# lez-s/Materialist

Hardware: AMD Instinct MI355X
Metric: opt_iterations_per_sec_512x512 (higher is better)
Workload: dtype f32; 1 GPU; BASELINE configs[1] synthetic: 1x512x512/GPU, --model_name pos_mlp --opt_order 'rm a' part rm, spp 64; mode=pos_mlp, height=512, width=512, spp=64, images_per_gpu=1, light=SH25, parallelism=dp1 (independent images, no data-path collective)

## Files before the change

include/matpbr_mlp.h:

```cpp
#ifndef MATPBR_MLP_H
#define MATPBR_MLP_H
#include <stddef.h>
#include <stdint.h>

#ifdef __cplusplus
extern "C" {
#endif

int matpbr_mlp_small_bwd_step(const float* g, int ldg, const float* w, int ldw, const float* c_prev, float* g_prev, int ldo, float* colsum_out,
                              int n_prev, const float* x, int ldx, float* d_w, int ldw_out, int K, const float* colsum_in, int colsum_stride,
                              int groups_in, float* d_bias, long M, int n_red, void* stream);

int matpbr_sin_bwd(const float* d_y, long ld_d, const float* pre, long ld_p, float* out, long M, int n, void* stream);
size_t matpbr_column_sum_workspace_bytes(int N);
int matpbr_column_sum(const float* x, float* out, long M, int N, void* workspace, size_t workspace_bytes, void* stream);

int matpbr_mlp_layer_fwd(const float* x, int ldx, const float* w, int ldw, const float* bias, float* s_out, float* c_out, int ldo, long M,
                         int N, int K, void* stream);
size_t matpbr_mlp_bwd_input_workspace_bytes(long M);
int matpbr_mlp_layer_bwd_input(const float* g, int ldg, const float* wt, int ldwt, const float* c_prev, float* g_prev, int ldo,
                               float* d_bias_prev, void* workspace, size_t workspace_bytes, long M, int n_prev, int n_red, void* stream);
size_t matpbr_mlp_bwd_weight_workspace_bytes(long M);
int matpbr_mlp_layer_bwd_weight(const float* g, int ldg, const float* x, int ldx, float* d_w, int ldw, void* workspace,
                                size_t workspace_bytes, long M, int N, int K, void* stream);

size_t matpbr_mlp_wsplit_bytes(int K);
int matpbr_mlp_split_weights(const float* w, int ldw, int N, int K, void* wsplit, void* stream);
int matpbr_mlp_layer_fwd_bx(const float* x, int ldx, const void* wsplit, const float* bias, float* s_out, float* c_out, int ldo, long M,
                            int N, int K, int nprod, void* stream);
int matpbr_mlp_first_layer_bwd_bx(const float* g, int ldg, const void* wtsplit, const float* c_prev, int ldc, int sgn, const float* x0, int ldx0,
                                  float* d_w0, long ld_j, long ld_c, int d0, float* d_bias0, void* workspace, size_t workspace_bytes, void* workspace2,
                                  size_t workspace2_bytes, long M, int n0, int n_red, int nprod, void* stream);
int matpbr_mlp_layer_bwd_input_bx(const float* g, int ldg, const void* wtsplit, const float* c_prev, float* g_prev, int ldo,
                                  float* d_bias_prev, void* workspace, size_t workspace_bytes, long M, int n_prev, int n_red,
                                  int nprod, void* stream);
int matpbr_mlp_layer_fwd_tail(const float* x, int ldx, const float* w, int ldw, const float* bias, float* s_out, float* c_out, int ldo,
                              const float* tail, int ldt, long M, int N, int K, void* stream);
int matpbr_mlp_layer_fwd_bx_tail(const float* x, int ldx, const void* wsplit, const float* bias, float* s_out, float* c_out, int ldo,
                                 const float* tail, int ldt, long M, int N, int K, int nprod, void* stream);
int matpbr_mlp_layer_fwd_bx_head(const float* x, int ldx, const void* wsplit, const float* bias, float* s_out, float* c_out, int ldo,
                                 const float* w_out, int ldw_out, const float* bias_out, const float* start, int lds, float* th,
                                 float* map_a, float* map_r, float* map_m, long M, int K, int nprod, void* stream);
int matpbr_mlp_layer_fwd_sgn(const float* x, int ldx, const float* w, int ldw, const float* bias, float* s_out, int ldo, const float* tail, int ldt,
                             long M, int N, int K, void* stream);
int matpbr_mlp_layer_bwd_input_sgn(const float* g, int ldg, const float* wt, int ldwt, const float* s_prev, float* g_prev, int ldo,
                                   float* d_bias_prev, void* workspace, size_t workspace_bytes, long M, int n_prev, int n_red, void* stream);
int matpbr_mlp_layer_bwd_input_bx_sgn(const float* g, int ldg, const void* wtsplit, const float* s_prev, float* g_prev, int ldo,
                                      float* d_bias_prev, void* workspace, size_t workspace_bytes, long M, int n_prev, int n_red,
                                      int nprod, void* stream);
int matpbr_mlp_layer_bwd_weight_bx(const float* g, int ldg, const float* x, int ldx, float* d_w, int ldw, void* workspace,
                                   size_t workspace_bytes, long M, int N, int K, int nprod, void* stream);

#define MATPBR_WSPLIT_TRANSPOSED 1
#define MATPBR_WSPLIT_F16X2 2
int matpbr_mlp_split_weights_fmt(const float* w, int ldw, int N, int K, int flags, void* wsplit, void* stream);
size_t matpbr_mlp_chain_images_bytes(void);
int matpbr_mlp_chain_prep(const float* const* w, const int* ldw, const int* n, const float* const* bias, int d0, void* images, void* const* bwd_images,
                          void* zero, long zero_words, void* stream);
int matpbr_mlp_chain_fwd(const float* x0, int ldx0, const void* images, float* const* s_out, int ldo, const int* n, const float* start, int lds, float* th,
                         float* map_a, float* map_r, float* map_m, int n_head, long M, void* stream);
#define MATPBR_REDUCE_NONE (-1)
#define MATPBR_REDUCE_WGRAD 0
#define MATPBR_REDUCE_COLSUM 1
#define MATPBR_REDUCE_SKINNY 2
typedef struct MatpbrReduceJob {
    int kind, groups;
    const float *src, *src_b, *src_g;
    float *dst, *dst_b, *dst_g;
    int n0, n1, n2, n3;
    long ld_j, ld_c;
} MatpbrReduceJob;
int matpbr_mlp_reduce_jobs(const MatpbrReduceJob* jobs, int n_jobs, void* stream);
int matpbr_mlp_out_layer_bwd_tmax(const float* d_x, int ldd, const float* s_prev, const float* c_prev, int lds, const float* w_out, int ldw, float* g_prev,
                                  int ldg, void* g_tile_max, float* d_w, long ld_j, long ld_c, float* d_bias, float* d_bias_prev, void* workspace,
                                  size_t workspace_bytes, long M, int J, int n_prev, MatpbrReduceJob* defer, void* stream);
int matpbr_mlp_layer_bwd_input_blk(const float* g, int ldg, const void* g_tile_max, const void* wtsplit, const float* s_prev, float* g_prev, int ldo,
                                   void* out_tile_max, float* d_bias_prev, void* workspace, size_t workspace_bytes, long M, int n_prev, int n_red,
                                   MatpbrReduceJob* defer, void* stream);
int matpbr_mlp_first_layer_bwd_blk(const float* g, int ldg, const void* g_tile_max, const void* wtsplit, const float* s_prev, int lds, const float* x0,
                                   int ldx0, float* d_w0, long ld_j, long ld_c, int d0, float* d_bias0, void* workspace, size_t workspace_bytes,
                                   void* workspace2, size_t workspace2_bytes, long M, int n0, int n_red, MatpbrReduceJob* defer2, void* stream);
int matpbr_mlp_layer_bwd_weight_blk(const float* g, int ldg, const void* g_tile_max, const float* x, int ldx, float* d_w, int ldw, void* workspace,
                                    size_t workspace_bytes, long M, int N, int K, MatpbrReduceJob* defer, void* stream);
int matpbr_mlp_set_wgrad_kernel(int kernel);
int matpbr_mlp_split_weights_multi(const float* const* w, const int* ldw, const int* N, const int* K, const int* transposed,
                                   void* const* wsplit, int n_jobs, void* stream);
int matpbr_mlp_skinny_fwd(const float* x, int ldx, const float* w, int ldw, const float* bias, float* out, int ldo, long M, int J, int K,
                          void* stream);
int matpbr_mlp_arm_head_fwd(const float* x, int ldx, const float* w, int ldw, const float* bias, const float* start, int lds, float* th,
                            float* map_a, float* map_r, float* map_m, long M, int K, void* stream);
int matpbr_mlp_arm_head_bwd(const float* g_a, const float* g_r, const float* g_m, const float* th, float* d_x, long M, void* stream);
size_t matpbr_mlp_skinny_workspace_bytes(int J);
int matpbr_mlp_out_layer_bwd(const float* d_x, int ldd, const float* s_prev, const float* c_prev, int lds, const float* w_out, int ldw, float* g_prev,
                             int ldg, float* d_w, long ld_j, long ld_c, float* d_bias, float* d_bias_prev, void* workspace, size_t workspace_bytes,
                             long M, int J, int n_prev, void* stream);
int matpbr_mlp_skinny_bwd_weight(const float* s, int lds, const float* b, int ldb, float* d_w, long ld_j, long ld_c, float* d_bias,
                                 void* workspace, size_t workspace_bytes, long M, int J, int C, void* stream);
int matpbr_adamw_step_dev(float* p, const float* g, float* m, float* v, long n, float* hyper, float beta1, float beta2, float eps,
                          float weight_decay, void* stream);
int matpbr_adamw_step_snapshot_dev(float* p, const float* g, float* m, float* v, long n, float* hyper, float beta1, float beta2,
                                   float eps, float weight_decay, float* best, const float* stats, void* stream);

#ifdef __cplusplus
}
#endif
#endif
```

materialist_amd/_lib.py:

```python
from __future__ import annotations

import ctypes
import os
import threading

from . import build as _build

_c_f = ctypes.c_void_p


class MatpbrCamera(ctypes.Structure):
    _fields_ = [("fov_x_deg", ctypes.c_float)]


class MatpbrBrdfPhase(ctypes.Structure):
    _fields_ = ([(k, ctypes.c_void_p) for k in ("pa", "pr", "pm", "n", "light", "gt_srgb", "a0", "r0", "m0", "dcache", "pred", "jac", "d_a",
                                                "d_r", "d_m")] +
                [("adam_m", ctypes.c_void_p * 3), ("adam_v", ctypes.c_void_p * 3)] +
                [(k, ctypes.c_void_p) for k in ("best_a", "best_r", "best_m", "best_img", "stats", "history", "workspace")] +
                [("workspace_bytes", ctypes.c_size_t), ("H", ctypes.c_int), ("W", ctypes.c_int), ("batch", ctypes.c_int), ("spp", ctypes.c_int),
                 ("fov_x_deg", ctypes.c_float), ("scale_delta", ctypes.c_float), ("part_mask", ctypes.c_uint32), ("es_patience", ctypes.c_int),
                 ("es_min_delta", ctypes.c_float), ("hist_len", ctypes.c_int), ("s1cache", ctypes.c_void_p), ("lazy_state", ctypes.c_void_p),
                 ("lazy_tol", ctypes.c_float), ("pred_next", ctypes.c_void_p), ("flags", ctypes.c_uint32), ("lazy_fold", ctypes.c_void_p)])


class MatpbrNormalStep(ctypes.Structure):
    _fields_ = ([(k, ctypes.c_void_p) for k in ("pa", "pr", "pm", "pn", "ca", "cr", "cm", "cn", "d_a", "d_r", "d_m", "d_n", "a0", "r0", "m0", "n0")] +
                [("adam_m", ctypes.c_void_p * 4), ("adam_v", ctypes.c_void_p * 4)] +
                [(k, ctypes.c_void_p) for k in ("best_a", "best_r", "best_m", "best_n", "best_img", "pred", "stats", "ln_part")] +
                [("H", ctypes.c_int), ("W", ctypes.c_int), ("batch", ctypes.c_int), ("part_mask", ctypes.c_uint32), ("scale_delta", ctypes.c_float)])


class MatpbrError(RuntimeError):
    pass


class ReduceJob(ctypes.Structure):
    _fields_ = [("kind", ctypes.c_int), ("groups", ctypes.c_int), ("src", ctypes.c_void_p), ("src_b", ctypes.c_void_p), ("src_g", ctypes.c_void_p),
                ("dst", ctypes.c_void_p), ("dst_b", ctypes.c_void_p), ("dst_g", ctypes.c_void_p), ("n0", ctypes.c_int), ("n1", ctypes.c_int),
                ("n2", ctypes.c_int), ("n3", ctypes.c_int), ("ld_j", ctypes.c_long), ("ld_c", ctypes.c_long)]


SIGNATURES = {
    "matpbr_version": (ctypes.c_int, []),
    "matpbr_strerror": (ctypes.c_char_p, [ctypes.c_int]),
    "matpbr_shade_fwd": (ctypes.c_int, [_c_f] * 5 + [ctypes.c_int, ctypes.c_int, _c_f, ctypes.c_int, ctypes.c_int, ctypes.c_int,
                                       ctypes.c_int, ctypes.POINTER(MatpbrCamera), ctypes.c_uint32, ctypes.c_void_p]),
    "matpbr_shade_bwd": (ctypes.c_int, [_c_f] * 5 + [ctypes.c_int, ctypes.c_int] + [_c_f] * 6 + [ctypes.c_void_p, ctypes.c_size_t,
                                       ctypes.c_int, ctypes.c_int, ctypes.c_int, ctypes.c_int, ctypes.POINTER(MatpbrCamera),
                                       ctypes.c_uint32, ctypes.c_void_p]),
    "matpbr_shade_bwd_workspace_bytes": (ctypes.c_size_t, [ctypes.c_int] * 4),
    "matpbr_plane9_bytes": (ctypes.c_size_t, [ctypes.c_int] * 3),
    "matpbr_shade_fwd_ex": (ctypes.c_int, [_c_f] * 5 + [ctypes.c_int, ctypes.c_int, _c_f, _c_f, _c_f, ctypes.c_int, ctypes.c_int, ctypes.c_int,
                                          ctypes.c_int, ctypes.POINTER(MatpbrCamera), ctypes.c_uint32, ctypes.c_void_p]),
    "matpbr_shade_fwd_keep": (ctypes.c_int, [_c_f] * 5 + [ctypes.c_int, ctypes.c_int, _c_f, _c_f, _c_f, _c_f, ctypes.c_int, ctypes.c_int, ctypes.c_int,
                                            ctypes.c_int, ctypes.POINTER(MatpbrCamera), ctypes.c_uint32, ctypes.c_void_p]),
    "matpbr_shade_fwd_cached": (ctypes.c_int, [_c_f] * 5 + [ctypes.c_int, ctypes.c_int, ctypes.c_int, ctypes.c_uint32, ctypes.c_void_p]),
    "matpbr_diffuse_cache": (ctypes.c_int, [_c_f, _c_f, ctypes.c_int, ctypes.c_int, _c_f, ctypes.c_int, ctypes.c_int, ctypes.c_int, ctypes.c_int,
                                           ctypes.POINTER(MatpbrCamera), ctypes.c_void_p]),
    "matpbr_lazy_state_bytes": (ctypes.c_size_t, [ctypes.c_int] * 3),
    "matpbr_lazy_fold_bytes": (ctypes.c_size_t, [ctypes.c_int] * 3),
    "matpbr_env_texel_phase_step": (ctypes.c_int, [_c_f] * 6 + [ctypes.c_int, ctypes.c_int, ctypes.c_float, ctypes.c_void_p, ctypes.c_size_t, ctypes.c_int,
                                                   ctypes.c_int, _c_f, ctypes.c_int] + [_c_f] * 8 + [ctypes.c_float] * 3 + [ctypes.c_int, ctypes.c_int,
                                                                                                                          ctypes.c_void_p]),
    "matpbr_brdf_loss_dpred": (ctypes.c_int, [_c_f] * 4 + [ctypes.c_int, ctypes.c_int, ctypes.c_int, ctypes.c_void_p]),
    "matpbr_brdf_normal_step": (ctypes.c_int, [ctypes.POINTER(MatpbrNormalStep), ctypes.c_int, ctypes.c_float, ctypes.c_void_p]),
    "matpbr_env_mlp_phase_step": (ctypes.c_int, [_c_f] * 7 + [ctypes.c_int, ctypes.c_int, ctypes.c_float, ctypes.c_void_p, ctypes.c_size_t, ctypes.c_int,
                                                 ctypes.c_int, _c_f, ctypes.c_int] + [_c_f] * 4 + [ctypes.c_int, ctypes.c_int, ctypes.c_void_p]),
    "matpbr_brdf_phase_stages_timed": (ctypes.c_int, [ctypes.POINTER(MatpbrBrdfPhase), ctypes.c_int, ctypes.c_float, ctypes.c_uint32, ctypes.c_void_p,
                                                      ctypes.c_void_p, ctypes.c_void_p]),
    "matpbr_lazy_sums_count": (ctypes.c_int, [ctypes.c_int] * 2),
    "matpbr_shade_fwd_lazy": (ctypes.c_int, [_c_f] * 5 + [ctypes.c_int, ctypes.c_int] + [_c_f] * 6 + [ctypes.c_int, ctypes.c_int, ctypes.c_int, ctypes.c_int,
                                            ctypes.POINTER(MatpbrCamera), ctypes.c_uint32, ctypes.c_float, ctypes.c_float, ctypes.c_void_p]),
    "matpbr_lazy_state_unpack": (ctypes.c_int, [_c_f, _c_f, _c_f, ctypes.c_int, ctypes.c_int, ctypes.c_int, ctypes.c_void_p]),
    "matpbr_jac16_unpack": (ctypes.c_int, [_c_f, _c_f, ctypes.c_int, ctypes.c_int, ctypes.c_int, ctypes.c_void_p]),
    "matpbr_shade_bwd_jac": (ctypes.c_int, [_c_f] * 8 + [ctypes.c_int, ctypes.c_int, ctypes.c_int, ctypes.c_void_p]),
    "matpbr_brdf_loss_workspace_bytes": (ctypes.c_size_t, [ctypes.c_int]),
    "matpbr_brdf_loss_stats": (ctypes.c_int, [_c_f] * 9 + [ctypes.c_float, _c_f, ctypes.c_void_p, ctypes.c_size_t, ctypes.c_int, ctypes.c_int,
                                             ctypes.c_int, ctypes.c_uint32, ctypes.c_void_p]),
    "matpbr_brdf_loss_stats_es": (ctypes.c_int, [_c_f] * 9 + [ctypes.c_float, _c_f, ctypes.c_void_p, ctypes.c_size_t, ctypes.c_int, ctypes.c_int,
                                                ctypes.c_int, ctypes.c_uint32, ctypes.c_int, ctypes.c_float, _c_f, ctypes.c_int, ctypes.c_void_p]),
    "matpbr_brdf_loss_bwd_jac": (ctypes.c_int, [_c_f] * 10 + [ctypes.c_float] + [_c_f] * 7 + [ctypes.c_int, ctypes.c_int, ctypes.c_int,
                                                                                              ctypes.c_uint32, ctypes.c_void_p]),
    "matpbr_brdf_phase_workspace_bytes": (ctypes.c_size_t, [ctypes.c_int] * 3),
    "matpbr_brdf_phase_step": (ctypes.c_int, [ctypes.POINTER(MatpbrBrdfPhase), ctypes.c_int, ctypes.c_float, ctypes.c_void_p]),
    "matpbr_brdf_phase_stages": (ctypes.c_int, [ctypes.POINTER(MatpbrBrdfPhase), ctypes.c_int, ctypes.c_float, ctypes.c_uint32, ctypes.c_void_p]),
    "matpbr_brdf_phase_resolve": (ctypes.c_int, [ctypes.POINTER(MatpbrBrdfPhase), ctypes.c_int, ctypes.c_void_p]),
    "matpbr_env_phase_workspace_bytes": (ctypes.c_size_t, [ctypes.c_int] * 3),
    "matpbr_env_phase_step": (ctypes.c_int, [_c_f] * 7 + [ctypes.c_int, ctypes.c_int, ctypes.c_float, ctypes.c_void_p, ctypes.c_size_t,
                                            ctypes.c_int, ctypes.c_int, ctypes.c_int, ctypes.c_void_p]),
    "matpbr_env_project": (ctypes.c_int, [_c_f, ctypes.c_int, _c_f, _c_f, _c_f, ctypes.c_int, ctypes.c_void_p]),
    "matpbr_env_project_bwd": (ctypes.c_int, [_c_f, ctypes.c_int, _c_f, _c_f, _c_f, ctypes.c_int, ctypes.c_int, ctypes.c_void_p]),
    "matpbr_select_improved": (ctypes.c_int, [_c_f, _c_f, _c_f, ctypes.c_int, ctypes.c_long, ctypes.c_void_p]),
    "matpbr_mlp_wsplit_bytes": (ctypes.c_size_t, [ctypes.c_int]),
    "matpbr_mlp_split_weights": (ctypes.c_int, [_c_f, ctypes.c_int, ctypes.c_int, ctypes.c_int, _c_f, ctypes.c_void_p]),
    "matpbr_mlp_layer_fwd_bx": (ctypes.c_int, [_c_f, ctypes.c_int, _c_f, _c_f, _c_f, _c_f, ctypes.c_int, ctypes.c_long, ctypes.c_int, ctypes.c_int,
                                              ctypes.c_int, ctypes.c_void_p]),
    "matpbr_mlp_layer_bwd_input_bx": (ctypes.c_int, [_c_f, ctypes.c_int, _c_f, _c_f, _c_f, ctypes.c_int, _c_f, ctypes.c_void_p, ctypes.c_size_t,
                                                    ctypes.c_long, ctypes.c_int, ctypes.c_int, ctypes.c_int, ctypes.c_void_p]),
    "matpbr_sin_bwd": (ctypes.c_int, [_c_f, ctypes.c_long, _c_f, ctypes.c_long, _c_f, ctypes.c_long, ctypes.c_int, ctypes.c_void_p]),
    "matpbr_mlp_layer_fwd": (ctypes.c_int, [_c_f, ctypes.c_int, _c_f, ctypes.c_int, _c_f, _c_f, _c_f, ctypes.c_int, ctypes.c_long, ctypes.c_int,
                                           ctypes.c_int, ctypes.c_void_p]),
    "matpbr_mlp_bwd_input_workspace_bytes": (ctypes.c_size_t, [ctypes.c_long]),
    "matpbr_mlp_layer_bwd_input": (ctypes.c_int, [_c_f, ctypes.c_int, _c_f, ctypes.c_int, _c_f, _c_f, ctypes.c_int, _c_f, ctypes.c_void_p,
                                                 ctypes.c_size_t, ctypes.c_long, ctypes.c_int, ctypes.c_int, ctypes.c_void_p]),
    "matpbr_mlp_bwd_weight_workspace_bytes": (ctypes.c_size_t, [ctypes.c_long]),
    "matpbr_mlp_layer_bwd_weight": (ctypes.c_int, [_c_f, ctypes.c_int, _c_f, ctypes.c_int, _c_f, ctypes.c_int, ctypes.c_void_p, ctypes.c_size_t,
                                                  ctypes.c_long, ctypes.c_int, ctypes.c_int, ctypes.c_void_p]),
    "matpbr_mlp_layer_fwd_sgn": (ctypes.c_int, [_c_f, ctypes.c_int, _c_f, ctypes.c_int, _c_f, _c_f, ctypes.c_int, _c_f, ctypes.c_int, ctypes.c_long,
                                               ctypes.c_int, ctypes.c_int, ctypes.c_void_p]),
    "matpbr_mlp_layer_bwd_input_sgn": (ctypes.c_int, [_c_f, ctypes.c_int, _c_f, ctypes.c_int, _c_f, _c_f, ctypes.c_int, _c_f, ctypes.c_void_p,
                                                     ctypes.c_size_t, ctypes.c_long, ctypes.c_int, ctypes.c_int, ctypes.c_void_p]),
    "matpbr_mlp_layer_bwd_input_bx_sgn": (ctypes.c_int, [_c_f, ctypes.c_int, _c_f, _c_f, _c_f, ctypes.c_int, _c_f, ctypes.c_void_p, ctypes.c_size_t,
                                                        ctypes.c_long, ctypes.c_int, ctypes.c_int, ctypes.c_int, ctypes.c_void_p]),
    "matpbr_mlp_layer_bwd_weight_bx": (ctypes.c_int, [_c_f, ctypes.c_int, _c_f, ctypes.c_int, _c_f, ctypes.c_int, ctypes.c_void_p, ctypes.c_size_t,
                                                     ctypes.c_long, ctypes.c_int, ctypes.c_int, ctypes.c_int, ctypes.c_void_p]),
    "matpbr_mlp_out_layer_bwd_tmax": (ctypes.c_int, [_c_f, ctypes.c_int, _c_f, _c_f, ctypes.c_int, _c_f, ctypes.c_int, _c_f, ctypes.c_int, ctypes.c_void_p, _c_f,
                                                     ctypes.c_long, ctypes.c_long, _c_f, _c_f, ctypes.c_void_p, ctypes.c_size_t, ctypes.c_long, ctypes.c_int,
                                                     ctypes.c_int, ctypes.c_void_p, ctypes.c_void_p]),
    "matpbr_mlp_reduce_jobs": (ctypes.c_int, [ctypes.c_void_p, ctypes.c_int, ctypes.c_void_p]),
    "matpbr_mlp_layer_bwd_input_blk": (ctypes.c_int, [_c_f, ctypes.c_int, ctypes.c_void_p, ctypes.c_void_p, _c_f, _c_f, ctypes.c_int, ctypes.c_void_p, _c_f,
                                                      ctypes.c_void_p, ctypes.c_size_t, ctypes.c_long, ctypes.c_int, ctypes.c_int, ctypes.c_void_p, ctypes.c_void_p]),
    "matpbr_mlp_first_layer_bwd_blk": (ctypes.c_int, [_c_f, ctypes.c_int, ctypes.c_void_p, ctypes.c_void_p, _c_f, ctypes.c_int, _c_f, ctypes.c_int, _c_f,
                                                      ctypes.c_long, ctypes.c_long, ctypes.c_int, _c_f, ctypes.c_void_p, ctypes.c_size_t, ctypes.c_void_p,
                                                      ctypes.c_size_t, ctypes.c_long, ctypes.c_int, ctypes.c_int, ctypes.c_void_p, ctypes.c_void_p]),
    "matpbr_mlp_layer_bwd_weight_blk": (ctypes.c_int, [_c_f, ctypes.c_int, ctypes.c_void_p, _c_f, ctypes.c_int, _c_f, ctypes.c_int, ctypes.c_void_p,
                                                       ctypes.c_size_t, ctypes.c_long, ctypes.c_int, ctypes.c_int, ctypes.c_void_p, ctypes.c_void_p]),
    "matpbr_mlp_set_wgrad_kernel": (ctypes.c_int, [ctypes.c_int]),
    "matpbr_mlp_chain_images_bytes": (ctypes.c_size_t, []),
    "matpbr_mlp_chain_prep": (ctypes.c_int, [ctypes.c_void_p, ctypes.c_void_p, ctypes.c_void_p, ctypes.c_void_p, ctypes.c_int, ctypes.c_void_p, ctypes.c_void_p,
                                             ctypes.c_void_p, ctypes.c_long, ctypes.c_void_p]),
    "matpbr_mlp_chain_fwd": (ctypes.c_int, [_c_f, ctypes.c_int, ctypes.c_void_p, ctypes.c_void_p, ctypes.c_int, ctypes.c_void_p, _c_f, ctypes.c_int, _c_f, _c_f, _c_f,
                                            _c_f, ctypes.c_int, ctypes.c_long, ctypes.c_void_p]),
    "matpbr_mlp_split_weights_fmt": (ctypes.c_int, [_c_f, ctypes.c_int, ctypes.c_int, ctypes.c_int, ctypes.c_int, ctypes.c_void_p, ctypes.c_void_p]),
    "matpbr_mlp_skinny_fwd": (ctypes.c_int, [_c_f, ctypes.c_int, _c_f, ctypes.c_int, _c_f, _c_f, ctypes.c_int, ctypes.c_long, ctypes.c_int, ctypes.c_int,
                                            ctypes.c_void_p]),
    "matpbr_mlp_arm_head_fwd": (ctypes.c_int, [_c_f, ctypes.c_int, _c_f, ctypes.c_int, _c_f, _c_f, ctypes.c_int, _c_f, _c_f, _c_f, _c_f, ctypes.c_long,
                                              ctypes.c_int, ctypes.c_void_p]),
    "matpbr_mlp_arm_head_bwd": (ctypes.c_int, [_c_f, _c_f, _c_f, _c_f, _c_f, ctypes.c_long, ctypes.c_void_p]),
    "matpbr_mlp_skinny_workspace_bytes": (ctypes.c_size_t, [ctypes.c_int]),
    "matpbr_mlp_set_lds_dma": (ctypes.c_int, [ctypes.c_int]),
    "matpbr_mlp_skinny_bwd_weight": (ctypes.c_int, [_c_f, ctypes.c_int, _c_f, ctypes.c_int, _c_f, ctypes.c_long, ctypes.c_long, _c_f, ctypes.c_void_p,
                                                   ctypes.c_size_t, ctypes.c_long, ctypes.c_int, ctypes.c_int, ctypes.c_void_p]),
    "matpbr_adamw_step_dev": (ctypes.c_int, [_c_f] * 4 + [ctypes.c_long, _c_f, ctypes.c_float, ctypes.c_float, ctypes.c_float, ctypes.c_float,
                                                         ctypes.c_void_p]),
    "matpbr_light_to_sh25": (ctypes.c_int, [_c_f, ctypes.c_int, ctypes.c_int, _c_f, ctypes.c_int, ctypes.c_void_p]),
    "matpbr_light_to_sh25_bwd": (ctypes.c_int, [_c_f, ctypes.c_int, ctypes.c_int, _c_f, ctypes.c_int, ctypes.c_void_p]),
    "matpbr_mlp_split_weights_multi": (ctypes.c_int, [ctypes.c_void_p] * 6 + [ctypes.c_int, ctypes.c_void_p]),
    "matpbr_adamw_step_snapshot_dev": (ctypes.c_int, [_c_f] * 4 + [ctypes.c_long, _c_f, ctypes.c_float, ctypes.c_float, ctypes.c_float, ctypes.c_float,
                                                                  _c_f, _c_f, ctypes.c_void_p]),
    "matpbr_mlp_layer_fwd_tail": (ctypes.c_int, [_c_f, ctypes.c_int, _c_f, ctypes.c_int, _c_f, _c_f, _c_f, ctypes.c_int, _c_f, ctypes.c_int, ctypes.c_long,
                                                ctypes.c_int, ctypes.c_int, ctypes.c_void_p]),
    "matpbr_mlp_layer_fwd_bx_tail": (ctypes.c_int, [_c_f, ctypes.c_int, _c_f, _c_f, _c_f, _c_f, ctypes.c_int, _c_f, ctypes.c_int, ctypes.c_long,
                                                   ctypes.c_int, ctypes.c_int, ctypes.c_int, ctypes.c_void_p]),
    "matpbr_sample_brdf_dr": (ctypes.c_int, [_c_f] * 10 + [ctypes.c_long, ctypes.c_void_p]),
    "matpbr_mlp_layer_fwd_bx_head": (ctypes.c_int, [_c_f, ctypes.c_int, _c_f, _c_f, _c_f, _c_f, ctypes.c_int, _c_f, ctypes.c_int, _c_f, _c_f, ctypes.c_int,
                                                   _c_f, _c_f, _c_f, _c_f, ctypes.c_long, ctypes.c_int, ctypes.c_int, ctypes.c_void_p]),
    "matpbr_column_sum_workspace_bytes": (ctypes.c_size_t, [ctypes.c_int]),
    "matpbr_column_sum": (ctypes.c_int, [_c_f, _c_f, ctypes.c_long, ctypes.c_int, ctypes.c_void_p, ctypes.c_size_t, ctypes.c_void_p]),
    "matpbr_shade_transfer": (ctypes.c_int, [_c_f] * 5 + [ctypes.c_int, ctypes.c_int, ctypes.c_int, ctypes.c_int, ctypes.POINTER(MatpbrCamera),
                                            ctypes.c_uint32, ctypes.c_void_p]),
    "matpbr_transfer_bytes": (ctypes.c_size_t, [ctypes.c_int] * 3),
    "matpbr_relight": (ctypes.c_int, [_c_f] * 3 + [ctypes.c_int, ctypes.c_int, ctypes.c_int, ctypes.c_void_p]),
    "matpbr_adam_step": (ctypes.c_int, [_c_f] * 4 + [ctypes.c_long, ctypes.c_float, ctypes.c_float, ctypes.c_float, ctypes.c_float, ctypes.c_int,
                                       ctypes.c_void_p]),
    "matpbr_eval_brdf": (ctypes.c_int, [_c_f] * 8 + [ctypes.c_long, ctypes.c_void_p]),
    "matpbr_eval_brdf_bwd": (ctypes.c_int, [_c_f] * 11 + [ctypes.c_long, ctypes.c_void_p]),
    "matpbr_brdf_terms": (ctypes.c_int, [_c_f] * 5 + [ctypes.c_long, ctypes.c_void_p]),
    "matpbr_sample_brdf": (ctypes.c_int, [_c_f] * 10 + [ctypes.c_long, ctypes.c_void_p]),
    "matpbr_sh_eval": (ctypes.c_int, [_c_f] * 3 + [ctypes.c_long, ctypes.c_void_p]),
    "matpbr_depth_to_mesh_host": (ctypes.c_int, [ctypes.c_void_p, ctypes.c_int, ctypes.c_int, ctypes.c_float, ctypes.c_float] + [ctypes.c_void_p] * 6),
    "matpbr_mlp_small_bwd_step": (ctypes.c_int, [_c_f, ctypes.c_int, _c_f, ctypes.c_int, _c_f, _c_f, ctypes.c_int, _c_f, ctypes.c_int, _c_f, ctypes.c_int,
                                                 _c_f, ctypes.c_int, ctypes.c_int, _c_f, ctypes.c_int, ctypes.c_int, _c_f, ctypes.c_long, ctypes.c_int,
                                                 ctypes.c_void_p]),
    "matpbr_mlp_out_layer_bwd": (ctypes.c_int, [_c_f, ctypes.c_int, _c_f, _c_f, ctypes.c_int, _c_f, ctypes.c_int, _c_f, ctypes.c_int, _c_f, ctypes.c_long,
                                                ctypes.c_long, _c_f, _c_f, ctypes.c_void_p, ctypes.c_size_t, ctypes.c_long, ctypes.c_int, ctypes.c_int,
                                                ctypes.c_void_p]),
    "matpbr_mlp_first_layer_bwd_bx": (ctypes.c_int, [_c_f, ctypes.c_int, ctypes.c_void_p, _c_f, ctypes.c_int, ctypes.c_int, _c_f, ctypes.c_int, _c_f, ctypes.c_long,
                                                     ctypes.c_long, ctypes.c_int, _c_f, ctypes.c_void_p, ctypes.c_size_t, ctypes.c_void_p, ctypes.c_size_t,
                                                     ctypes.c_long, ctypes.c_int, ctypes.c_int, ctypes.c_int, ctypes.c_void_p]),
    "matpbr_masked_mean_fill": (ctypes.c_int, [_c_f, ctypes.c_void_p, _c_f, ctypes.c_float, ctypes.c_float, _c_f, ctypes.c_long, ctypes.c_int,
                                               ctypes.c_void_p]),
    "matpbr_normals_from_depth": (ctypes.c_int, [_c_f, _c_f, ctypes.c_int, ctypes.c_int, ctypes.c_int, ctypes.POINTER(MatpbrCamera),
                                                 ctypes.c_void_p]),
}

_lock = threading.Lock()
_lib = None


def library_path() -> str:
    return os.environ.get("MATPBR_LIB") or _build.LIB_PATH


def load(build_if_missing: bool = False) -> ctypes.CDLL:
    global _lib
    with _lock:
        if _lib is not None:
            return _lib
        path = library_path()
        if not os.path.exists(path):
            if build_if_missing:
                _build.build_library()
            else:
                raise MatpbrError(
                    f"{path} is missing: build it with `python -c 'import __graft_entry__ as g; g.build()'` "
                    "(hipcc --offload-arch=gfx950). matpbr has no CPU or PyTorch fallback.")
        try:
            lib = ctypes.CDLL(path)
        except OSError as e:
            raise MatpbrError(f"cannot load {path}: {e}") from e
        for name, (res, args) in SIGNATURES.items():
            try:
                fn = getattr(lib, name)
            except AttributeError as e:
                raise MatpbrError(f"{path} does not export {name}") from e
            fn.restype = res
            fn.argtypes = args
        _lib = lib
        return lib


def check(code: int, what: str) -> None:
    if code != 0:
        msg = load().matpbr_strerror(code)
        raise MatpbrError(f"{what} failed: {msg.decode() if msg else code} ({code})")
```

materialist_amd/csrc/posmlp_kernels.hip:

```cpp
#include <hip/hip_runtime.h>
#include <stdint.h>
#include <atomic>
#include <type_traits>

#include "../../include/matpbr.h"
#include "../../include/matpbr_experimental.h"
#include "posmlp_device.hpp"

namespace {


constexpr int kBM = 128, kBN = 128, kBK = 32;
constexpr int kPersistent = 512;
constexpr int EPI_SINCOS = 0, EPI_MULC = 1, EPI_BIAS = 2;

struct HeadArgs {
  const float* w;
  int ldw;
  const float* bias;
  ArmHead h;
};

__global__ __launch_bounds__(256) void mlp_tail_copy_kernel(float* __restrict__ out, int ldo, const float* __restrict__ tail, int ldt, long M, int N) {
  const int w = 256 - N;
  const long total = M * w;
  for (long i = (long)blockIdx.x * 256 + threadIdx.x; i < total; i += (long)gridDim.x * 256) {
    const long m = i / w;
    const int j = (int)(i - m * w);
    out[m * ldo + N + j] = tail[m * ldt + j];
  }
}
__device__ __forceinline__ void store4_upto(float* dst, float4 v, int valid, bool all) {
  if (all) {
    *reinterpret_cast<float4*>(dst) = v;
    return;
  }
  if (valid >= 4) {
    *reinterpret_cast<float4*>(dst) = v;
  } else {
    if (valid > 0) dst[0] = v.x;
    if (valid > 1) dst[1] = v.y;
    if (valid > 2) dst[2] = v.z;
  }
}

struct NtArgs {
  const float* A;
  const float* B;
  const float* bias;
  const float* cmul;
  float* out0;
  float* out1;
  float* colsum;
  int M;
  int N, K, lda, ldb, ldo;
  const float* tail;
  int ldt;
  int cmul_sin;
  const float* x0;
  int ldx0;
  float* w0_part;
  const unsigned* a_tmax;
  unsigned* o_tmax;
};

constexpr int kLd = 36;
constexpr int kTileFloats = kBM * kLd;

__device__ __forceinline__ void fetch_a(const NtArgs& p, float4 (&ra)[4], int row0, int kslot, int crow, int ck) {
  int k = kslot * kBK + ck;
  const int kmax = ((p.K + 3) & ~3) - 4;
  k = k < kmax ? k : kmax;
#pragma unroll
  for (int q = 0; q < 4; ++q) {
    int m = row0 + crow + 32 * q;
    m = m < p.M ? m : p.M - 1;
    ra[q] = *reinterpret_cast<const float4*>(p.A + (size_t)m * p.lda + k);
  }
}

__device__ __forceinline__ void fetch_b(const NtArgs& p, float4 (&rb)[4], int col0, int kslot, int crow, int ck) {
  int k = kslot * kBK + ck;
  const int kmax = ((p.K + 3) & ~3) - 4;
  k = k < kmax ? k : kmax;
#pragma unroll
  for (int q = 0; q < 4; ++q) {
    int n = col0 + crow + 32 * q;
    n = n < p.N ? n : p.N - 1;
    rb[q] = *reinterpret_cast<const float4*>(p.B + (size_t)n * p.ldb + k);
  }
}

__device__ __forceinline__ float4 kmask(float4 v, int k, int K, bool keep) {
  v.x = (keep && k < K) ? v.x : 0.f;
  v.y = (keep && k + 1 < K) ? v.y : 0.f;
  v.z = (keep && k + 2 < K) ? v.z : 0.f;
  v.w = (keep && k + 3 < K) ? v.w : 0.f;
  return v;
}

template <bool ROWS_FULL>
__device__ __forceinline__ void stash(const NtArgs& p, const float4 (&ra)[4], const float4 (&rb)[4], float* sA, float* sB, int row0, int col0,
                                      int kslot, int crow, int ck) {
  const int k = kslot * kBK + ck;
#pragma unroll
  for (int q = 0; q < 4; ++q) {
    const bool mrow = ROWS_FULL || (row0 + crow + 32 * q < p.M);
    *reinterpret_cast<float4*>(sA + (crow + 32 * q) * kLd + ck) = kmask(ra[q], k, p.K, mrow);
    *reinterpret_cast<float4*>(sB + (crow + 32 * q) * kLd + ck) = kmask(rb[q], k, p.K, col0 + crow + 32 * q < p.N);
  }
}

template <class Mid>
__device__ __forceinline__ void nt_tile_mma(f32x16 (&acc)[2][2], const float* pa, const float* pb, Mid&& mid) {
#pragma unroll
  for (int j = 0; j < 4; ++j) {
    float4 a4[2], b4[2];
#pragma unroll
    for (int mi = 0; mi < 2; ++mi) a4[mi] = *reinterpret_cast<const float4*>(pa + mi * 32 * kLd + 4 * j);
#pragma unroll
    for (int ni = 0; ni < 2; ++ni) b4[ni] = *reinterpret_cast<const float4*>(pb + ni * 32 * kLd + 4 * j);
#pragma unroll
    for (int e = 0; e < 4; ++e)
#pragma unroll
      for (int mi = 0; mi < 2; ++mi)
#pragma unroll
        for (int ni = 0; ni < 2; ++ni) {
          const float av = e == 0 ? a4[mi].x : e == 1 ? a4[mi].y : e == 2 ? a4[mi].z : a4[mi].w;
          const float bv = e == 0 ? b4[ni].x : e == 1 ? b4[ni].y : e == 2 ? b4[ni].z : b4[ni].w;
          acc[mi][ni] = __builtin_amdgcn_mfma_f32_32x32x2f32(av, bv, acc[mi][ni], 0, 0, 0);
        }
    mid(j);
  }
}

struct TileMap {
  int halves, half, col0, my_count;
  __device__ TileMap(int rtiles, int N) {
    halves = (N + kBN - 1) / kBN;
    const int ntiles = (halves == 2) ? ((rtiles + 7) / 8) * 16 : rtiles;
    half = (halves == 2) ? (int)((blockIdx.x >> 3) & 1) : 0;
    col0 = half * kBN;
    my_count = ((int)blockIdx.x < ntiles) ? (ntiles - (int)blockIdx.x + (int)gridDim.x - 1) / (int)gridDim.x : 0;
    while (my_count > 0 && row_of(my_count - 1) >= rtiles * kBM) --my_count;
  }
  __device__ int row_of(int j) const {
    const int id = (int)blockIdx.x + j * (int)gridDim.x;
    return ((halves == 2) ? (id >> 4) * 8 + (id & 7) : id) * kBM;
  }
};

template <int EPI>
__global__ __launch_bounds__(256, 2) void mlp_gemm_nt(NtArgs p) {
  __shared__ __attribute__((aligned(16))) float sA[2][kTileFloats];
  __shared__ __attribute__((aligned(16))) float sB[2][kTileFloats];
  const int tid = threadIdx.x, lane = tid & 63, wave = tid >> 6;
  const int wm = wave >> 1, wn = wave & 1;
  const int li = lane & 31, lh = lane >> 5;
  const int crow = tid >> 3, ck = (tid & 7) * 4;
  const int nk = (p.K + kBK - 1) / kBK;
  const int aoff = (wm * 64 + li) * kLd + 16 * lh, boff = (wn * 64 + li) * kLd + 16 * lh;
  const TileMap tm((p.M + kBM - 1) / kBM, p.N);
  const int col0 = tm.col0;
  float csum[2] = {0.f, 0.f};

  for (int j = 0; j < tm.my_count; ++j) {
    const int row0 = tm.row_of(j);
    f32x16 acc[2][2];
#pragma unroll
    for (int mi = 0; mi < 2; ++mi)
#pragma unroll
      for (int ni = 0; ni < 2; ++ni)
#pragma unroll
        for (int r = 0; r < 16; ++r) acc[mi][ni][r] = 0.f;

    float4 ra[4], rb[4];
    __syncthreads();
    fetch_a(p, ra, row0, 0, crow, ck);
    fetch_b(p, rb, col0, 0, crow, ck);
    stash<false>(p, ra, rb, sA[0], sB[0], row0, col0, 0, crow, ck);
    fetch_a(p, ra, row0, nk > 1 ? 1 : 0, crow, ck);
    fetch_b(p, rb, col0, nk > 1 ? 1 : 0, crow, ck);
    __syncthreads();
    for (int kt = 0; kt < nk; ++kt) {
      const int cur = kt & 1;
      nt_tile_mma(acc, sA[cur] + aoff, sB[cur] + boff, [](int) {});
      const int k1 = kt + 1 < nk ? kt + 1 : kt, k2 = kt + 2 < nk ? kt + 2 : nk - 1;
      stash<false>(p, ra, rb, sA[cur ^ 1], sB[cur ^ 1], row0, col0, k1, crow, ck);
      fetch_a(p, ra, row0, k2, crow, ck);
      fetch_b(p, rb, col0, k2, crow, ck);
      __syncthreads();
    }

    int ncol[2];
    bool nok[2];
    float bn[2];
#pragma unroll
    for (int ni = 0; ni < 2; ++ni) {
      const int n = col0 + wn * 64 + ni * 32 + li;
      nok[ni] = n < p.N;
      ncol[ni] = nok[ni] ? n : p.N - 1;
      bn[ni] = (EPI != EPI_MULC) ? p.bias[ncol[ni]] : 0.f;
    }
    if (row0 + kBM <= p.M && p.ldo >= col0 + kBN) {
      float* scr = sA[0] + wave * (32 * kLd);
      const int t_row = lane >> 3, t_col = (lane & 7) * 4;
      float4 cs4[2] = {make_float4(0.f, 0.f, 0.f, 0.f), make_float4(0.f, 0.f, 0.f, 0.f)};
#pragma unroll
      for (int mi = 0; mi < 2; ++mi) {
        const size_t tile_row = (size_t)(row0 + wm * 64 + mi * 32 + t_row) * p.ldo;
        float4 cv4[2][4];
        if (EPI == EPI_MULC) {
#pragma unroll
          for (int ni = 0; ni < 2; ++ni)
#pragma unroll
            for (int ps = 0; ps < 4; ++ps)
// ... 653 lines not shown
  const int tn = block / tiles_k, tk = block - tn * tiles_k;
  const int n = tn * 32 + li, k = tk * 32 + li;
  const bool nok = n < N, kok = k < K;
  const float* pg = G + (nok ? n : N - 1);
  const float* px = X + (kok ? k : K - 1);
  const int quarter = ((M + 3) / 4 + 1) & ~1;
  const int m_begin = wave * quarter, m_end = min(M, m_begin + quarter);
  f32x16 acc;
#pragma unroll
  for (int r = 0; r < 16; ++r) acc[r] = 0.f;
  for (int m0 = m_begin; m0 < m_end; m0 += 128) {
    float a[64], b[64];
#pragma unroll
    for (int j = 0; j < 64; ++j) {
      const int m = m0 + 2 * j + lh;
      const int mc = m < M ? m : M - 1;
      const float av = pg[(size_t)mc * ldg], bv = px[(size_t)mc * ldx];
      a[j] = (m < m_end && nok) ? av : 0.f;
      b[j] = (m < m_end && kok) ? bv : 0.f;
    }
#pragma unroll
    for (int j = 0; j < 64; ++j)
      if (m0 + 2 * j < m_end) acc = __builtin_amdgcn_mfma_f32_32x32x2f32(a[j], b[j], acc, 0, 0, 0);
  }
  if (wave > 0) {
#pragma unroll
    for (int r = 0; r < 16; ++r) s_part[wave - 1][r * 64 + lane] = acc[r];
  }
  __syncthreads();
  if (wave == 0) {
#pragma unroll
    for (int r = 0; r < 16; ++r) {
      const float v = ((acc[r] + s_part[0][r * 64 + lane]) + s_part[1][r * 64 + lane]) + s_part[2][r * 64 + lane];
      const int nn = tn * 32 + (r & 3) + 8 * (r >> 2) + 4 * lh;
      if (nn < N && kok) dW[(size_t)nn * ldw + k] = v;
    }
  }
}

__global__ __launch_bounds__(256) void mlp_small_tn(const float* __restrict__ G, int ldg, const float* __restrict__ X, int ldx,
                                                    float* __restrict__ dW, int ldw, int M, int N, int K) {
  small_tn_body(G, ldg, X, ldx, dW, ldw, M, N, K, (int)blockIdx.x);
}

struct SmallBwdStep {
  NtArgs d;
  int nD;
  const float* G; int ldg; const float* X; int ldx; float* dW; int ldw; int M, N, K;
  int nW;
  const float* part_in; int part_stride, groups_in; float* d_bias; int n_bias;
};
__global__ __launch_bounds__(256) void mlp_small_bwd_step_kernel(const SmallBwdStep a) {
  int b = (int)blockIdx.x;
  if (b < a.nD) {
    small_nt_body<EPI_MULC, true>(a.d, b);
    return;
  }
  b -= a.nD;
  if (b < a.nW) {
    small_tn_body(a.G, a.ldg, a.X, a.ldx, a.dW, a.ldw, a.M, a.N, a.K, b);
    return;
  }
  if (a.n_bias <= 4 && a.groups_in > 64) {
    __shared__ float s_b[256][4];
    float v[4] = {0.f, 0.f, 0.f, 0.f};
    for (int g = (int)threadIdx.x; g < a.groups_in; g += 256) {
#pragma unroll
      for (int c = 0; c < 4; ++c)
        if (c < a.n_bias) v[c] += a.part_in[(long)g * a.part_stride + c];
    }
#pragma unroll
    for (int c = 0; c < 4; ++c) s_b[threadIdx.x][c] = v[c];
    __syncthreads();
    for (int half = 128; half > 0; half >>= 1) {
      if ((int)threadIdx.x < half) {
#pragma unroll
        for (int c = 0; c < 4; ++c) s_b[threadIdx.x][c] += s_b[threadIdx.x + half][c];
      }
      __syncthreads();
    }
    if ((int)threadIdx.x < a.n_bias) a.d_bias[threadIdx.x] = s_b[0][threadIdx.x];
    return;
  }
  const int c = (b - a.nW) * 256 + (int)threadIdx.x;
  if (c < a.n_bias) {
    float s = 0.f;
    int g = 0;
    for (; g + 8 <= a.groups_in; g += 8) {
      float t[8];
#pragma unroll
      for (int j = 0; j < 8; ++j) t[j] = a.part_in[(long)(g + j) * a.part_stride + c];
#pragma unroll
      for (int j = 0; j < 8; ++j) s += t[j];
    }
    for (; g < a.groups_in; ++g) s += a.part_in[(long)g * a.part_stride + c];
    a.d_bias[c] = s;
  }
}

template <int EPI, bool BKN = false>
int launch_small_nt(NtArgs p, long M, hipStream_t stream) {
  p.M = (int)M;
  const int tiles = (int)((M + 31) / 32) * ((p.N + 31) / 32);
  hipLaunchKernelGGL((mlp_small_nt<EPI, BKN>), dim3((unsigned)tiles), dim3(256), 0, stream, p);
  return (int)((M + 31) / 32);
}


constexpr int kBxStage = 2 * 3 * 2 * 256;
__host__ __device__ inline size_t wsplit_index(int ks, int s, int piece, int n, int g) {
  return ((((size_t)ks * 2 + s) * 3 + piece) * 2 + g) * 256 + n;
}
__device__ __forceinline__ void split_weights_item(const float* __restrict__ B, int ldb, int N, int K, bool tr, bool f16, uint4* __restrict__ out, int idx) {
  const int nks = (K + 31) / 32;
  if (idx >= nks * 2 * 256 * 2) return;
  const int g = idx & 1, n = (idx >> 1) & 255, s = (idx >> 9) & 1, ks = idx >> 10;
  float v[8];
#pragma unroll
  for (int q = 0; q < 8; ++q) {
    const int k = 32 * ks + 16 * g + 8 * s + q;
    v[q] = (n < N && k < K) ? (tr ? B[(size_t)k * ldb + n] : B[(size_t)n * ldb + k]) : 0.f;
  }
  if (f16) {
    unsigned p[2][4];
#pragma unroll
    for (int q = 0; q < 4; ++q) split2h(v[2 * q] * kF16WScale, v[2 * q + 1] * kF16WScale, p[0][q], p[1][q]);
#pragma unroll
    for (int piece = 0; piece < 2; ++piece)
      out[((((size_t)ks * 2 + s) * 2 + piece) * 2 + g) * 256 + n] = make_uint4(p[piece][0], p[piece][1], p[piece][2], p[piece][3]);
    return;
  }
  unsigned p[3][4];
#pragma unroll
  for (int q = 0; q < 4; ++q) split3(v[2 * q], v[2 * q + 1], p[0][q], p[1][q], p[2][q]);
#pragma unroll
  for (int piece = 0; piece < 3; ++piece) out[wsplit_index(ks, s, piece, n, g)] = make_uint4(p[piece][0], p[piece][1], p[piece][2], p[piece][3]);
}
__global__ __launch_bounds__(256) void mlp_split_weights_kernel(const float* __restrict__ B, int ldb, int N, int K, int flags, uint4* __restrict__ out) {
  split_weights_item(B, ldb, N, K, (flags & 1) != 0, (flags & 2) != 0, out, blockIdx.x * 256 + threadIdx.x);
}

struct SplitJobs {
  const float* w[8];
  uint4* out[8];
  int ldw[8], N[8], K[8], transposed[8];
};
__global__ __launch_bounds__(256) void mlp_split_weights_multi_kernel(const SplitJobs jobs) {
  const int j = blockIdx.y;
  split_weights_item(jobs.w[j], jobs.ldw[j], jobs.N[j], jobs.K[j], (jobs.transposed[j] & 1) != 0, (jobs.transposed[j] & 2) != 0, jobs.out[j],
                     blockIdx.x * 256 + threadIdx.x);
}

constexpr int kBxThreads = 512;
typedef float f32x4v __attribute__((ext_vector_type(4)));
constexpr int kGlRows = 128 * 32 * 4;
constexpr size_t kGlSmem = 2 * kBxStage * sizeof(uint4) + 3 * kGlRows;
template <int EPI, int NPROD, bool FULL, bool HEAD = false, bool W0 = false, bool GL = false>
__global__ __launch_bounds__(kBxThreads, 1) void mlp_nt_bx(const NtArgs p, const uint4* __restrict__ wsplit, const HeadArgs hd) {
  extern __shared__ __align__(16) unsigned char bx_smem[];
  uint4* sB = reinterpret_cast<uint4*>(bx_smem);
  float* sScr = reinterpret_cast<float*>(bx_smem + 2 * kBxStage * sizeof(uint4));
  float* sRed = reinterpret_cast<float*>(bx_smem);
  float* sExtra = GL ? reinterpret_cast<float*>(bx_smem + kGlSmem) : sScr + 8 * 32 * kLd;
  float* sW4 = sExtra;
  float* sComb = sW4 + 5 * 256;
  float* sX0 = sExtra;
  const int tid = threadIdx.x, lane = tid & 63, wave = tid >> 6;
  const int wm = wave >> 1, wn = wave & 1, li = lane & 31, lh = lane >> 5;
  const int nks = (p.K + 31) / 32;
  const int tiles = p.M / kBM;
  constexpr int kCopy = kBxStage / kBxThreads;
  float bn[4];
  float4 csum4[4];
  f32x4v acc0[4][2];
  if (W0) {
#pragma unroll
    for (int ni = 0; ni < 4; ++ni)
#pragma unroll
      for (int ct = 0; ct < 2; ++ct) acc0[ni][ct] = f32x4v{0.f, 0.f, 0.f, 0.f};
  }
#pragma unroll
  for (int ni = 0; ni < 4; ++ni) {
    const int n = wn * 128 + ni * 32 + li;
    bn[ni] = (EPI != EPI_MULC) ? p.bias[n < p.N ? n : p.N - 1] : 0.f;
    csum4[ni] = make_float4(0.f, 0.f, 0.f, 0.f);
  }
  const int b_lane = lh * 256 + wn * 128 + li;
  uint4 bnext[kCopy];
  if (!GL) {
#pragma unroll
    for (int q = 0; q < kCopy; ++q) sB[tid + kBxThreads * q] = wsplit[tid + kBxThreads * q];
  }
  if (HEAD) {
    for (int i = tid; i < 5 * 256; i += kBxThreads) sW4[i] = hd.w[(size_t)(i >> 8) * hd.ldw + (i & 255)];
  }
  __syncthreads();
  int buf = 0;
  const int wave_u = __builtin_amdgcn_readfirstlane(wave);
  const unsigned lds0 = GL ? lds_byte_address(bx_smem) : 0u;
  const bool issuer = wave_u >= 4;
  const unsigned gl_w_dst = lds0, gl_a_dst = lds0 + 2u * kBxStage * 16u;
  unsigned gl_w_voff[2], gl_a_voff[2][2], gl_rd[4];
#pragma unroll
  for (int v = 0; v < 2; ++v) {
    const int vw = (wave & 3) + 4 * v;
    gl_w_voff[v] = (unsigned)(384 * vw + lane) * 16u;
#pragma unroll
    for (int j = 0; j < 2; ++j) {
      const int row = 16 * vw + 8 * j + (lane >> 3);
      gl_a_voff[v][j] = (unsigned)(row * p.lda + 4 * ((lane & 7) ^ ((row >> 1) & 7))) * 4u;
    }
  }
#pragma unroll
  for (int q = 0; q < 4; ++q) {
    const int row = wm * 32 + li;
    gl_rd[q] = (unsigned)(2 * kBxStage * 16 + row * 128 + (((4 * lh + q) ^ ((row >> 1) & 7)) * 16));
  }
  int a_slot = 0;
  auto gl_issue_w = [&](int ks_w, int wb) {
    const char* src = reinterpret_cast<const char*>(wsplit) + (size_t)ks_w * (kBxStage * 16);
#pragma unroll
    for (int v = 0; v < 2; ++v)
#pragma unroll
      for (int j = 0; j < 6; ++j)
        glds16(src + 1024 * j, gl_w_voff[v], gl_w_dst + (unsigned)wb * (kBxStage * 16u) + (unsigned)((wave_u & 3) + 4 * v) * 6144u + 1024u * j);
  };
  auto gl_issue_a = [&](int tile_a, int ks_a, int slot) {
    const float* src = p.A + (size_t)tile_a * kBM * p.lda + 32 * ks_a;
#pragma unroll
    for (int v = 0; v < 2; ++v)
#pragma unroll
      for (int j = 0; j < 2; ++j)
        glds16(src, gl_a_voff[v][j], gl_a_dst + (unsigned)slot * (unsigned)kGlRows + (unsigned)((wave_u & 3) + 4 * v) * 2048u + 1024u * j);
  };
  if (GL) {
    const int t0 = blockIdx.x;
    if (issuer) {
      gl_issue_w(0, 0);
      gl_issue_a(t0, 0, 0);
      gl_issue_a(nks > 1 ? t0 : (t0 + (int)gridDim.x < tiles ? t0 + (int)gridDim.x : t0), nks > 1 ? 1 : 0, 1);
      asm volatile("s_waitcnt vmcnt(4)" ::: "memory");
    }
    asm volatile("s_barrier" ::: "memory");
  }

  for (int tile = blockIdx.x; tile < tiles; tile += gridDim.x) {
    const int row0 = tile * kBM;
    const float* pa0 = p.A + (size_t)(row0 + wm * 32 + li) * p.lda + 16 * lh;
    f32x16 acc[4];
#pragma unroll
    for (int ni = 0; ni < 4; ++ni)
#pragma unroll
      for (int r = 0; r < 16; ++r) acc[ni][r] = 0.f;

    float4 raw[4];
    if (!GL) {
#pragma unroll
      for (int q = 0; q < 4; ++q) raw[q] = *reinterpret_cast<const float4*>(pa0 + 4 * q);
    }
    for (int ks = 0; ks < nks; ++ks) {
      const int ksn = ks + 1 < nks ? ks + 1 : 0;
      float4 cur[4];
      const int ks_stamp = ks & 7; (void)ks_stamp;
      if (GL) {
        int t2 = tile, k2 = ks + 2;
        if (k2 >= nks) { k2 -= nks; t2 = tile + (int)gridDim.x < tiles ? tile + (int)gridDim.x : tile; }
        if (k2 >= nks) k2 = 0;
        if (issuer) {
          gl_issue_w(ksn, buf ^ 1);
          gl_issue_a(t2, k2, a_slot >= 1 ? a_slot - 1 : 2);
        }
#pragma unroll
        for (int q = 0; q < 4; ++q) cur[q] = *reinterpret_cast<const float4*>(bx_smem + gl_rd[q] + a_slot * kGlRows);
      } else {
#pragma unroll
      for (int q = 0; q < 4; ++q) cur[q] = raw[q];
      const uint4* wsrc = wsplit + (size_t)ksn * kBxStage + tid;
#pragma unroll
      for (int q = 0; q < kCopy; ++q) bnext[q] = wsrc[kBxThreads * q];
      if (ks + 1 < nks) {
#pragma unroll
        for (int q = 0; q < 4; ++q) raw[q] = *reinterpret_cast<const float4*>(pa0 + 32 * (ks + 1) + 4 * q);
      }
      }
      if (32 * (ks + 1) > p.K) {
#pragma unroll
        for (int q = 0; q < 4; ++q) {
          const int k = 32 * ks + 16 * lh + 4 * q;
          cur[q].x = k < p.K ? cur[q].x : 0.f;
          cur[q].y = k + 1 < p.K ? cur[q].y : 0.f;
          cur[q].z = k + 2 < p.K ? cur[q].z : 0.f;
          cur[q].w = k + 3 < p.K ? cur[q].w : 0.f;
        }
      }
      const uint4* sb = sB + buf * kBxStage + b_lane;
#pragma unroll
      for (int s = 0; s < 2; ++s) {
        uint4 bq[3][4];
#pragma unroll
        for (int piece = 0; piece < 3; ++piece)
#pragma unroll
          for (int ni = 0; ni < 4; ++ni) bq[piece][ni] = sb[((s * 3 + piece) * 2) * 256 + ni * 32];
        uint4 aq[3];
        {
          const float4 u = cur[2 * s], v = cur[2 * s + 1];
          split3(u.x, u.y, aq[0].x, aq[1].x, aq[2].x);
          split3(u.z, u.w, aq[0].y, aq[1].y, aq[2].y);
// ... 7 lines not shown
#pragma unroll
          for (int ni = 0; ni < 4; ++ni)
            acc[ni] = __builtin_amdgcn_mfma_f32_32x32x16_bf16(__builtin_bit_cast(bf16x8, aq[ia[t]]), __builtin_bit_cast(bf16x8, bq[ib[t]][ni]),
                                                              acc[ni], 0, 0, 0);
        }
      }
      if (GL) {
        if (issuer) asm volatile("s_waitcnt vmcnt(4)" ::: "memory");
        asm volatile("s_waitcnt lgkmcnt(0)\n\ts_barrier" ::: "memory");
        a_slot = a_slot == 2 ? 0 : a_slot + 1;
      } else {
      uint4* sdst = sB + (buf ^ 1) * kBxStage + tid;
#pragma unroll
      for (int q = 0; q < kCopy; ++q) sdst[kBxThreads * q] = bnext[q];
      __syncthreads();
      }
      buf ^= 1;
    }
    float* scr = GL ? reinterpret_cast<float*>(bx_smem + (size_t)(buf ^ 1) * (kBxStage * 16) + wave * 6144) : sScr + wave * (32 * kLd);
    const int t_row = lane >> 3, t_col = (lane & 7) * 4;
    const size_t tile_row = (size_t)(row0 + wm * 32 + t_row) * p.ldo;
    float* sx = sX0 + wave * (32 * 16);
    if (W0) {
      const float* xs = p.x0 + (size_t)(row0 + wm * 32 + (lane >> 1)) * p.ldx0 + 8 * (lane & 1);
      const float4 xa = *reinterpret_cast<const float4*>(xs), xb = *reinterpret_cast<const float4*>(xs + 4);
      *reinterpret_cast<float4*>(sx + (lane >> 1) * 16 + 8 * (lane & 1)) = xa;
      *reinterpret_cast<float4*>(sx + (lane >> 1) * 16 + 8 * (lane & 1) + 4) = xb;
    }
    float hacc[4][5];
    if (HEAD) {
#pragma unroll
      for (int ps = 0; ps < 4; ++ps)
#pragma unroll
        for (int j = 0; j < 5; ++j) hacc[ps][j] = 0.f;
    }
#pragma unroll
    for (int nh = 0; nh < 2; ++nh) {
      float4 cv[2][4];
      if (EPI == EPI_MULC) {
#pragma unroll
        for (int n2 = 0; n2 < 2; ++n2)
#pragma unroll
          for (int ps = 0; ps < 4; ++ps)
            cv[n2][ps] = *reinterpret_cast<const float4*>(p.cmul + tile_row + (size_t)(8 * ps) * p.ldo + wn * 128 + (nh * 2 + n2) * 32 + t_col);
      }
#pragma unroll
      for (int n2 = 0; n2 < 2; ++n2) {
        const int ni = nh * 2 + n2;
        const size_t o0 = tile_row + wn * 128 + ni * 32 + t_col;
        float second[16];
#pragma unroll
        for (int r = 0; r < 16; ++r) {
          float v = acc[ni][r];
          if (EPI == EPI_SINCOS) {
            if (p.out1 == nullptr) v = sin_packed(v + bn[ni]);
            else sincos_cw(v + bn[ni], v, second[r]);
          } else if (EPI == EPI_BIAS) {
            v += bn[ni];
          }
          scr[((r & 3) + 8 * (r >> 2) + 4 * lh) * kLd + li] = v;
        }
#pragma unroll
        for (int ps = 0; ps < 4; ++ps) {
          float4 v = *reinterpret_cast<const float4*>(scr + (t_row + 8 * ps) * kLd + t_col);
          if (EPI == EPI_MULC) {
            if (p.cmul_sin) cv[n2][ps] = cos_from_packed_sin(cv[n2][ps]);
            v.x *= cv[n2][ps].x; v.y *= cv[n2][ps].y; v.z *= cv[n2][ps].z; v.w *= cv[n2][ps].w;
            csum4[ni].x += v.x; csum4[ni].y += v.y; csum4[ni].z += v.z; csum4[ni].w += v.w;
          }
          if (W0) *reinterpret_cast<float4*>(scr + (t_row + 8 * ps) * kLd + t_col) = v;
          if (HEAD) {
#pragma unroll
            for (int j = 0; j < 5; ++j) {
              const float4 w4 = *reinterpret_cast<const float4*>(sW4 + j * 256 + wn * 128 + ni * 32 + t_col);
              hacc[ps][j] = __builtin_fmaf(v.x, w4.x, __builtin_fmaf(v.y, w4.y, __builtin_fmaf(v.z, w4.z, __builtin_fmaf(v.w, w4.w, hacc[ps][j]))));
            }
          }
          if (!W0) store4_upto(p.out0 + o0 + (size_t)(8 * ps) * p.ldo, v, p.N - (wn * 128 + ni * 32 + t_col), FULL || wn * 128 + ni * 32 + 32 <= p.N);
        }
        if (W0) {
#pragma unroll
          for (int ct = 0; ct < 2; ++ct)
#pragma unroll
            for (int kk = 0; kk < 8; ++kk)
              acc0[ni][ct] = __builtin_amdgcn_mfma_f32_16x16x4f32(scr[(4 * kk + (lane >> 4)) * kLd + 16 * ct + (lane & 15)],
                                                                  sx[(4 * kk + (lane >> 4)) * 16 + (lane & 15)], acc0[ni][ct], 0, 0, 0);
        }
        if (EPI == EPI_SINCOS && p.out1 != nullptr) {
#pragma unroll
          for (int r = 0; r < 16; ++r) scr[((r & 3) + 8 * (r >> 2) + 4 * lh) * kLd + li] = second[r];
#pragma unroll
          for (int ps = 0; ps < 4; ++ps)
            store4_upto(p.out1 + o0 + (size_t)(8 * ps) * p.ldo, *reinterpret_cast<const float4*>(scr + (t_row + 8 * ps) * kLd + t_col),
                        p.N - (wn * 128 + ni * 32 + t_col), FULL || wn * 128 + ni * 32 + 32 <= p.N);
        }
      }
    }
    if (HEAD) {
#pragma unroll
      for (int ps = 0; ps < 4; ++ps)
#pragma unroll
        for (int j = 0; j < 5; ++j) {
          float v = hacc[ps][j];
          v = dpp_add_f<0x111>(v);
          v = dpp_add_f<0x112>(v);
          v = dpp_add_f<0x114>(v);
          if ((lane & 7) == 7) sComb[((wm * 32 + t_row + 8 * ps) * 2 + wn) * 8 + j] = v;
        }
      __syncthreads();
      if (tid < kBM) {
        float v5[5];
#pragma unroll
        for (int j = 0; j < 5; ++j) v5[j] = (sComb[(tid * 2) * 8 + j] + sComb[(tid * 2 + 1) * 8 + j]) + hd.bias[j];
        arm_head_store(hd.h, (long)row0 + tid, v5);
      }
    }
    if (GL) asm volatile("s_waitcnt lgkmcnt(0)\n\ts_barrier" ::: "memory");
  }
  if (GL) asm volatile("s_waitcnt vmcnt(0)" ::: "memory");
  if (W0) {
    const size_t slab = (size_t)blockIdx.x * 4 + wm;
#pragma unroll
    for (int ni = 0; ni < 4; ++ni)
#pragma unroll
      for (int ct = 0; ct < 2; ++ct)
#pragma unroll
        for (int r = 0; r < 4; ++r)
          p.w0_part[(slab * 16 + (lane & 15)) * 256 + wn * 128 + ni * 32 + 16 * ct + 4 * (lane >> 4) + r] = acc0[ni][ct][r];
  }
  if (EPI == EPI_MULC && p.colsum != nullptr) {
    const int t_row = lane >> 3, t_col = (lane & 7) * 4;
    __syncthreads();
#pragma unroll
    for (int ni = 0; ni < 4; ++ni)
      *reinterpret_cast<float4*>(sRed + (wm * 8 + t_row) * 256 + wn * 128 + ni * 32 + t_col) = csum4[ni];
    __syncthreads();
    if (tid < 256) {
      float t = 0.f;
#pragma unroll
      for (int sl = 0; sl < 32; ++sl) t += sRed[sl * 256 + tid];
      p.colsum[(size_t)blockIdx.x * 256 + tid] = t;
    }
  }
}

constexpr int kGxThreads = 256;
constexpr int kGxW = kBxStage / 2 * 16;
constexpr size_t kGxSmem = 2 * kGxW + 2 * kGlRows;
template <int EPI, int NPROD, bool HEAD, bool PK, bool W0 = false>
__global__ __launch_bounds__(kGxThreads, 2) void mlp_nt_gx(const NtArgs p, const uint4* __restrict__ wsplit, const HeadArgs hd) {
  extern __shared__ __align__(16) unsigned char gx_smem[];
  constexpr bool F16 = NPROD == 3;
  constexpr bool BLK = F16 && EPI == EPI_MULC;
  static_assert(!F16 || EPI != EPI_BIAS, "the two-piece f16 form: sine layers forward (sines in, unit scale) and input gradients (block-scaled rows)");
  constexpr int kSlicePitch = F16 ? 384 : 256;
  constexpr size_t kStepBytes = F16 ? 16384 : (size_t)kGxW;
  const int tid = threadIdx.x, lane = tid & 63, wave = tid >> 6;
  const int wm = wave >> 1, wn = wave & 1, li = lane & 31, lh = lane >> 5;
  const int ng = (p.K + 31) / 32;
  const int tiles = p.M / kBM;
  const int wave_u = __builtin_amdgcn_readfirstlane(wave);
  const unsigned lds0 = lds_byte_address(gx_smem);
  const unsigned w_dst = lds0 + (unsigned)wave_u * 6144u, a_dst = lds0 + 2u * kGxW + (unsigned)wave_u * 4096u;
  const unsigned w_voff = (unsigned)((F16 ? 256 : 384) * wave + lane) * 16u;
  unsigned a_voff[4], a_rd[4];
#pragma unroll
  for (int j = 0; j < 4; ++j) {
    const int row = 32 * wave + 8 * j + (lane >> 3);
    a_voff[j] = (unsigned)(row * p.lda + 4 * ((lane & 7) ^ ((row >> 1) & 7))) * 4u;
  }
#pragma unroll
  for (int q = 0; q < 4; ++q) a_rd[q] = (unsigned)(2 * kGxW + (wm * 64 + li) * 128 + (((4 * lh + q) ^ ((li >> 1) & 7)) * 16));
  float bn[4];
  float4 csum4[4];
#pragma unroll
  for (int ni = 0; ni < 4; ++ni) {
    bn[ni] = (EPI != EPI_MULC) ? p.bias[wn * 128 + ni * 32 + li] : 0.f;
    csum4[ni] = make_float4(0.f, 0.f, 0.f, 0.f);
  }
  f32x4v acc0[4][2];
  if (W0) {
#pragma unroll
    for (int ni = 0; ni < 4; ++ni)
#pragma unroll
      for (int ct = 0; ct < 2; ++ct) acc0[ni][ct] = f32x4v{0.f, 0.f, 0.f, 0.f};
  }
  const int b_lane = lh * kSlicePitch + wn * 128 + li;
  auto issue_w = [&](int step_w, int wb) {
    const char* src = reinterpret_cast<const char*>(wsplit) + (size_t)step_w * kStepBytes;
    if (F16) {
      glds16_x4(src, w_voff, w_dst + (unsigned)wb * (unsigned)kGxW);
    } else {
      glds16_x3(src, w_voff, w_dst + (unsigned)wb * (unsigned)kGxW);
      glds16_x3(src + 3072, w_voff, w_dst + (unsigned)wb * (unsigned)kGxW + 3072u);
    }
  };
  auto issue_a = [&](int tile_a, int g_a, int ab) {
    const float* src = p.A + (size_t)tile_a * kBM * p.lda + 32 * g_a;
    glds16_x4v(src, a_voff[0], a_voff[1] - 1024u, a_voff[2] - 2048u, a_voff[3] - 3072u, a_dst + (unsigned)ab * (unsigned)kGlRows);
  };
  issue_w(0, 0);
  issue_a(blockIdx.x, 0, 0);
  asm volatile("s_waitcnt vmcnt(0)\n\ts_barrier" ::: "memory");
  int wb = 0, ab = 0;

  for (int tile = blockIdx.x; tile < tiles; tile += gridDim.x) {
    const int row0 = tile * kBM;
    float a_scale = 1.0f, a_unscale = kF16WUnscale, omax = 0.f;
    if (BLK) {
      block_scale(p.a_tmax[tile], a_scale, a_unscale);
      a_unscale *= kF16WUnscale;
    }
    f32x16 acc[2][4];
#pragma unroll
    for (int mi = 0; mi < 2; ++mi)
#pragma unroll
      for (int ni = 0; ni < 4; ++ni)
#pragma unroll
        for (int r = 0; r < 16; ++r) acc[mi][ni][r] = 0.f;
    for (int g = 0; g < ng; ++g) {
      int t2 = tile, g2 = g + 1;
      if (g2 >= ng) { g2 = 0; t2 = tile + (int)gridDim.x < tiles ? tile + (int)gridDim.x : tile; }
#pragma unroll
      for (int s = 0; s < 2; ++s) {
        const int step_n = s == 0 ? 2 * g + 1 : (g + 1 < ng ? 2 * g + 2 : 0);
        issue_w(step_n, wb ^ 1);
        if (s == 0) issue_a(t2, g2, ab ^ 1);
        uint4 aq[2][3];
#pragma unroll
        for (int mi = 0; mi < 2; ++mi) {
          float4 u = *reinterpret_cast<const float4*>(gx_smem + a_rd[2 * s] + ab * kGlRows + mi * 4096);
          float4 v = *reinterpret_cast<const float4*>(gx_smem + a_rd[2 * s + 1] + ab * kGlRows + mi * 4096);
          if (32 * (g + 1) > p.K) {
            const int k = 32 * g + 16 * lh + 8 * s;
            u.x = k < p.K ? u.x : 0.f; u.y = k + 1 < p.K ? u.y : 0.f; u.z = k + 2 < p.K ? u.z : 0.f; u.w = k + 3 < p.K ? u.w : 0.f;
            v.x = k + 4 < p.K ? v.x : 0.f; v.y = k + 5 < p.K ? v.y : 0.f; v.z = k + 6 < p.K ? v.z : 0.f; v.w = k + 7 < p.K ? v.w : 0.f;
          }
          if (BLK) {
            u.x *= a_scale; u.y *= a_scale; u.z *= a_scale; u.w *= a_scale;
            v.x *= a_scale; v.y *= a_scale; v.z *= a_scale; v.w *= a_scale;
          }
          if (F16) {
            split2h(u.x, u.y, aq[mi][0].x, aq[mi][1].x);
            split2h(u.z, u.w, aq[mi][0].y, aq[mi][1].y);
            split2h(v.x, v.y, aq[mi][0].z, aq[mi][1].z);
            split2h(v.z, v.w, aq[mi][0].w, aq[mi][1].w);
          } else {
            split3(u.x, u.y, aq[mi][0].x, aq[mi][1].x, aq[mi][2].x);
            split3(u.z, u.w, aq[mi][0].y, aq[mi][1].y, aq[mi][2].y);
            split3(v.x, v.y, aq[mi][0].z, aq[mi][1].z, aq[mi][2].z);
            split3(v.z, v.w, aq[mi][0].w, aq[mi][1].w, aq[mi][2].w);
          }
        }
        const uint4* sb = reinterpret_cast<const uint4*>(gx_smem + wb * kGxW) + b_lane;
#pragma unroll
        for (int ni = 0; ni < 4; ++ni) {
          uint4 bq[3];
#pragma unroll
          for (int piece = 0; piece < (F16 ? 2 : 3); ++piece) bq[piece] = sb[(piece * 2) * kSlicePitch + ni * 32];
          if constexpr (F16) {
#pragma unroll
            for (int t = 0; t < 3; ++t) {
              constexpr int ia[3] = {1, 0, 0}, ib[3] = {0, 1, 0};
#pragma unroll
              for (int mi = 0; mi < 2; ++mi)
                acc[mi][ni] = __builtin_amdgcn_mfma_f32_32x32x16_f16(__builtin_bit_cast(f16x8, aq[mi][ia[t]]), __builtin_bit_cast(f16x8, bq[ib[t]]),
                                                                     acc[mi][ni], 0, 0, 0);
            }
          }
#pragma unroll
          for (int t = 0; t < (F16 ? 0 : 9); ++t) {
            constexpr int ia[9] = {2, 1, 2, 2, 0, 1, 1, 0, 0}, ib[9] = {2, 2, 1, 0, 2, 1, 0, 1, 0};
            if (NPROD == 6 && t < 3) continue;
#pragma unroll
            for (int mi = 0; mi < 2; ++mi)
              acc[mi][ni] = __builtin_amdgcn_mfma_f32_32x32x16_bf16(__builtin_bit_cast(bf16x8, aq[mi][ia[t]]), __builtin_bit_cast(bf16x8, bq[ib[t]]),
                                                                    acc[mi][ni], 0, 0, 0);
          }
        }
        if (s == 0) asm volatile("s_waitcnt vmcnt(4) lgkmcnt(0)\n\ts_barrier" ::: "memory");
        else asm volatile("s_waitcnt vmcnt(0) lgkmcnt(0)\n\ts_barrier" ::: "memory");
        wb ^= 1;
      }
      ab ^= 1;
    }
    float* scr = reinterpret_cast<float*>(gx_smem + (size_t)(wb ^ 1) * kGxW + wave * 6144);
    float* sW4 = reinterpret_cast<float*>(gx_smem + 2 * kGxW + (size_t)(ab ^ 1) * kGlRows);
    float* sComb = sW4 + 5 * 256;
    const int t_row = lane >> 3, t_col = (lane & 7) * 4;
    if (HEAD) {
      for (int i = tid; i < 5 * 256; i += kGxThreads) sW4[i] = hd.w[(size_t)(i >> 8) * hd.ldw + (i & 255)];
      __syncthreads();
    }
    float* sx = reinterpret_cast<float*>(gx_smem + 2 * kGxW + (size_t)(ab ^ 1) * kGlRows + wave * 4096);
    if (W0) {
      const float* xs = p.x0 + (size_t)(row0 + wm * 64 + lane) * p.ldx0;
#pragma unroll
      for (int q = 0; q < 4; ++q) *reinterpret_cast<float4*>(sx + lane * 16 + 4 * ((q + lane) & 3)) = *reinterpret_cast<const float4*>(xs + 4 * ((q + lane) & 3));
    }
    constexpr int kCvSets = W0 ? 1 : 2;
    float4 cvb[kCvSets][4];
    auto cv_load = [&](int b, float4 (&dst)[4]) {
      const float* src = p.cmul + (size_t)(row0 + wm * 64 + (b >> 2) * 32 + t_row) * p.ldo + wn * 128 + (b & 3) * 32 + t_col;
#pragma unroll
      for (int ps = 0; ps < 4; ++ps) dst[ps] = *reinterpret_cast<const float4*>(src + (size_t)(8 * ps) * p.ldo);
    };
    if (EPI == EPI_MULC) cv_load(0, cvb[0]);
    float hacc[4][5];
#pragma unroll
    for (int b = 0; b < 8; ++b) {
      const int mi = b >> 2, ni = b & 3;
      const size_t o0 = (size_t)(row0 + wm * 64 + mi * 32 + t_row) * p.ldo + wn * 128 + ni * 32 + t_col;
      if (EPI == EPI_MULC && !W0 && b + 1 < 8) cv_load(b + 1, cvb[(b + 1) & (kCvSets - 1)]);
      if (HEAD && ni == 0) {
#pragma unroll
        for (int ps = 0; ps < 4; ++ps)
#pragma unroll
          for (int j = 0; j < 5; ++j) hacc[ps][j] = 0.f;
      }
      float second[16];
#pragma unroll
      for (int r = 0; r < 16; ++r) {
        float v = acc[mi][ni][r];
        if (BLK) v *= a_unscale;
        if (EPI == EPI_SINCOS) {
          const float pre = F16 ? __builtin_fmaf(v, kF16WUnscale, bn[ni]) : v + bn[ni];
          if (PK) v = sin_packed(pre);
          else sincos_cw(pre, v, second[r]);
        }
        scr[((r & 3) + 8 * (r >> 2) + 4 * lh) * kLd + li] = v;
      }
      float4 vrow[4];
#pragma unroll
      for (int ps = 0; ps < 4; ++ps) {
        float4 v = *reinterpret_cast<const float4*>(scr + (t_row + 8 * ps) * kLd + t_col);
        if (EPI == EPI_MULC) {
          float4 c4 = cvb[b & (kCvSets - 1)][ps];
          if (p.cmul_sin) c4 = cos_from_packed_sin(c4);
          v.x *= c4.x; v.y *= c4.y; v.z *= c4.z; v.w *= c4.w;
          csum4[ni].x += v.x; csum4[ni].y += v.y; csum4[ni].z += v.z; csum4[ni].w += v.w;
          if (BLK && !W0) omax = __builtin_fmaxf(__builtin_fmaxf(omax, __builtin_fmaxf(__builtin_fabsf(v.x), __builtin_fabsf(v.y))),
                                                   __builtin_fmaxf(__builtin_fabsf(v.z), __builtin_fabsf(v.w)));
        }
        if (EPI == EPI_SINCOS && !HEAD && ni == 3 && p.tail != nullptr && wn == 1) {
            const int col = 224 + t_col;
            const float* tl = p.tail + (size_t)(row0 + wm * 64 + mi * 32 + t_row + 8 * ps) * p.ldt - p.N;
            if (col >= p.N) v.x = tl[col];
            if (col + 1 >= p.N) v.y = tl[col + 1];
            if (col + 2 >= p.N) v.z = tl[col + 2];
            if (col + 3 >= p.N) v.w = tl[col + 3];
        }
        if (W0) *reinterpret_cast<float4*>(scr + (t_row + 8 * ps) * kLd + t_col) = v;
        else *reinterpret_cast<float4*>(p.out0 + o0 + (size_t)(8 * ps) * p.ldo) = v;
        vrow[ps] = v;
      }
      if (W0) {
        if (EPI == EPI_MULC && b + 1 < 8) cv_load(b + 1, cvb[0]);
#pragma unroll
        for (int ct = 0; ct < 2; ++ct) {
#pragma unroll
          for (int kk = 0; kk < 8; ++kk)
            acc0[ni][ct] = __builtin_amdgcn_mfma_f32_16x16x4f32(scr[(4 * kk + (lane >> 4)) * kLd + 16 * ct + (lane & 15)],
                                                                sx[(mi * 32 + 4 * kk + (lane >> 4)) * 16 + (lane & 15)], acc0[ni][ct], 0, 0, 0);
          __builtin_amdgcn_sched_barrier(0);
        }
      }
      if (HEAD) {
#pragma unroll
        for (int j = 0; j < 5; ++j) {
          const float4 w4 = *reinterpret_cast<const float4*>(sW4 + j * 256 + wn * 128 + ni * 32 + t_col);
#pragma unroll
          for (int ps = 0; ps < 4; ++ps)
            hacc[ps][j] = __builtin_fmaf(vrow[ps].x, w4.x, __builtin_fmaf(vrow[ps].y, w4.y, __builtin_fmaf(vrow[ps].z, w4.z, __builtin_fmaf(vrow[ps].w, w4.w, hacc[ps][j]))));
        }
      }
      if (EPI == EPI_SINCOS && !PK) {
#pragma unroll
        for (int r = 0; r < 16; ++r) scr[((r & 3) + 8 * (r >> 2) + 4 * lh) * kLd + li] = second[r];
#pragma unroll
        for (int ps = 0; ps < 4; ++ps)
          *reinterpret_cast<float4*>(p.out1 + o0 + (size_t)(8 * ps) * p.ldo) = *reinterpret_cast<const float4*>(scr + (t_row + 8 * ps) * kLd + t_col);
      }
      if (HEAD && ni == 3) {
#pragma unroll
        for (int ps = 0; ps < 4; ++ps)
#pragma unroll
          for (int j = 0; j < 5; ++j) {
            float v = hacc[ps][j];
            v = dpp_add_f<0x111>(v);
            v = dpp_add_f<0x112>(v);
            v = dpp_add_f<0x114>(v);
            if ((lane & 7) == 7) sComb[((wm * 64 + mi * 32 + t_row + 8 * ps) * 2 + wn) * 8 + j] = v;
          }
      }
    }
    if (HEAD) {
      __syncthreads();
      if (tid < kBM) {
        float v5[5];
#pragma unroll
        for (int j = 0; j < 5; ++j) v5[j] = (sComb[(tid * 2) * 8 + j] + sComb[(tid * 2 + 1) * 8 + j]) + hd.bias[j];
        arm_head_store(hd.h, (long)row0 + tid, v5);
      }
      __syncthreads();
    }
    if (BLK && !W0 && p.o_tmax != nullptr) {
      const float wmx = wave_max_lane63(omax);
      if (lane == 63) atomicMax(p.o_tmax + tile, __float_as_uint(wmx));
    }
    asm volatile("s_waitcnt lgkmcnt(0)" ::: "memory");
  }
  asm volatile("s_waitcnt vmcnt(0)" ::: "memory");
  if (W0) {
    const size_t slab = (size_t)blockIdx.x * 2 + wm;
#pragma unroll
    for (int ni = 0; ni < 4; ++ni)
#pragma unroll
      for (int ct = 0; ct < 2; ++ct)
#pragma unroll
        for (int r = 0; r < 4; ++r)
          p.w0_part[(slab * 16 + (lane & 15)) * 256 + wn * 128 + ni * 32 + 16 * ct + 4 * (lane >> 4) + r] = acc0[ni][ct][r];
  }
  if (EPI == EPI_MULC && p.colsum != nullptr) {
    float* sRed = reinterpret_cast<float*>(gx_smem);
    const int t_row = lane >> 3, t_col = (lane & 7) * 4;
    __syncthreads();
#pragma unroll
    for (int ni = 0; ni < 4; ++ni)
      *reinterpret_cast<float4*>(sRed + (wm * 8 + t_row) * 256 + wn * 128 + ni * 32 + t_col) = csum4[ni];
    __syncthreads();
    float t = 0.f;
#pragma unroll
    for (int sl = 0; sl < 16; ++sl) t += sRed[sl * 256 + tid];
    p.colsum[(size_t)blockIdx.x * 256 + tid] = t;
  }
}

constexpr int kWgStage = 2 * 3 * 2 * 256;
constexpr size_t kWgSmem = 2 * kWgStage * sizeof(uint4);
#ifndef MATPBR_WG_DEPTH
#define MATPBR_WG_DEPTH 2
#endif
constexpr int kWgDepth = MATPBR_WG_DEPTH;
constexpr int kWgThreads = 512;
__device__ __forceinline__ int wg_perm(int i) { return (i & 16) + 2 * (i & 7) + ((i >> 3) & 1); }
template <int NPROD, bool EARLY>
__device__ __forceinline__ void wgrad_bx_body(const float* __restrict__ G, int ldg, const float* __restrict__ X, int ldx,
                                              float* __restrict__ partial, long M, long rows_per_slab, uint4* sW, const unsigned* __restrict__ g_tmax) {
  constexpr bool F16 = NPROD == 3;
  constexpr int NP = F16 ? 2 : 3;
  const int tid = threadIdx.x, lane = tid & 63, wave = tid >> 6;
  const int nq = wave >> 1, kq = wave & 1, li = lane & 31, lh = lane >> 5;
  const long m_begin = (long)blockIdx.x * rows_per_slab;
  const long m_end = (m_begin + rows_per_slab < M) ? m_begin + rows_per_slab : M;
  const int t_first = F16 ? (int)(M / kBM) - 1 - (int)blockIdx.x : 0;
  const int steps = F16 ? (t_first >= 0 ? (t_first / (int)gridDim.x + 1) * (kBM / 16) : 0) : (m_begin < m_end ? (int)((m_end - m_begin) / 16) : 0);
  auto step_row = [&](int step) -> long {
    return F16 ? ((long)t_first - (long)(step >> 3) * gridDim.x) * kBM + 16 * (7 - (step & 7)) : m_begin + 16L * step;
  };
  float g_scale = 1.0f, g_unscale = 1.0f;
  if (F16 && steps > 0) {
    unsigned mb = 0;
    for (int t = t_first; t >= 0; t -= (int)gridDim.x) mb = g_tmax[t] > mb ? g_tmax[t] : mb;
    block_scale(mb, g_scale, g_unscale);
  }

  f32x16 acc[2][4];
#pragma unroll
  for (int ni = 0; ni < 2; ++ni)
#pragma unroll
    for (int ki = 0; ki < 4; ++ki)
#pragma unroll
      for (int r = 0; r < 16; ++r) acc[ni][ki][r] = 0.f;

  const int cp = tid & 255, sh = tid >> 8;
  const float* src = (cp >> 7) ? X + (8 * sh) * (long)ldx + 2 * (cp & 127) : G + (8 * sh) * (long)ldg + 2 * (cp & 127);
  const long ld = (cp >> 7) ? ldx : ldg;
  const float my_scale = (F16 && !(cp >> 7)) ? g_scale : 1.0f;
  uint4* sdst = sW + (((cp >> 7) * NP) * 2 + sh) * 256 + ((cp & 127) >> 3) * 16 + (cp & 7);
  float2 raw[kWgDepth][8];
  auto load_stage = [&](int slot, int step) {
#pragma unroll
    for (int j = 0; j < 8; ++j) raw[slot][j] = *reinterpret_cast<const float2*>(src + (step_row(step) + j) * ld);
  };
  auto split_store = [&](int slot, int buf) {
#pragma unroll
    for (int c = 0; c < 2; ++c) {
      uint4 pc[3];
      const float2* r = raw[slot];
#define MATPBR_COMP(v) (c == 0 ? (v).x : (v).y)
      if (F16) {
        split2h(MATPBR_COMP(r[0]) * my_scale, MATPBR_COMP(r[1]) * my_scale, pc[0].x, pc[1].x);
        split2h(MATPBR_COMP(r[2]) * my_scale, MATPBR_COMP(r[3]) * my_scale, pc[0].y, pc[1].y);
        split2h(MATPBR_COMP(r[4]) * my_scale, MATPBR_COMP(r[5]) * my_scale, pc[0].z, pc[1].z);
        split2h(MATPBR_COMP(r[6]) * my_scale, MATPBR_COMP(r[7]) * my_scale, pc[0].w, pc[1].w);
      } else {
        split3(MATPBR_COMP(r[0]), MATPBR_COMP(r[1]), pc[0].x, pc[1].x, pc[2].x);
        split3(MATPBR_COMP(r[2]), MATPBR_COMP(r[3]), pc[0].y, pc[1].y, pc[2].y);
        split3(MATPBR_COMP(r[4]), MATPBR_COMP(r[5]), pc[0].z, pc[1].z, pc[2].z);
        split3(MATPBR_COMP(r[6]), MATPBR_COMP(r[7]), pc[0].w, pc[1].w, pc[2].w);
      }
#undef MATPBR_COMP
#pragma unroll
      for (int piece = 0; piece < NP; ++piece) sdst[buf * kWgStage + (piece * 2) * 256 + 8 * c] = pc[piece];
    }
  };
  auto stage = [&](int slot, int buf, int next_stage) {
    __builtin_amdgcn_sched_barrier(0);
    split_store(slot, buf);
    __builtin_amdgcn_sched_barrier(0);
    load_stage(slot, next_stage < steps ? next_stage : steps - 1);
    __builtin_amdgcn_sched_barrier(0);
  };

  if (steps > 0) {
    load_stage(0, 0);
    split_store(0, 0);
#pragma unroll
    for (int d = 0; d < kWgDepth; ++d) {
      __builtin_amdgcn_sched_barrier(0);
      load_stage((1 + d) % kWgDepth, 1 + d < steps ? 1 + d : steps - 1);
    }
    __builtin_amdgcn_sched_barrier(0);
    __syncthreads();
    auto step = [&](auto u_tag, int st) {
        constexpr int u = decltype(u_tag)::value;
        const int cur = st & 1;
        if (EARLY) stage((u + 1) % kWgDepth, cur ^ 1, st + 1 + kWgDepth);
        const uint4* sa = sW + cur * kWgStage + lh * 256 + nq * 64 + li;
        const uint4* sb = sW + cur * kWgStage + (NP * 2 + lh) * 256 + kq * 128 + li;
        uint4 a[3][2];
#pragma unroll
        for (int piece = 0; piece < NP; ++piece)
#pragma unroll
          for (int ni = 0; ni < 2; ++ni) a[piece][ni] = sa[(piece * 2) * 256 + ni * 32];
#pragma unroll
        for (int kh = 0; kh < 2; ++kh) {
          uint4 b[3][2];
#pragma unroll
          for (int piece = 0; piece < NP; ++piece)
#pragma unroll
            for (int k2 = 0; k2 < 2; ++k2) b[piece][k2] = sb[(piece * 2) * 256 + (kh * 2 + k2) * 32];
          if constexpr (F16) {
#pragma unroll
            for (int t = 0; t < 3; ++t) {
              constexpr int ia[3] = {1, 0, 0}, ib[3] = {0, 1, 0};
#pragma unroll
              for (int k2 = 0; k2 < 2; ++k2)
#pragma unroll
                for (int ni = 0; ni < 2; ++ni)
                  acc[ni][kh * 2 + k2] = __builtin_amdgcn_mfma_f32_32x32x16_f16(__builtin_bit_cast(f16x8, a[ia[t]][ni]),
                                                                               __builtin_bit_cast(f16x8, b[ib[t]][k2]), acc[ni][kh * 2 + k2], 0, 0, 0);
            }
          }
#pragma unroll
          for (int t = 0; t < (F16 ? 0 : 9); ++t) {
            constexpr int ia[9] = {2, 1, 2, 2, 0, 1, 1, 0, 0}, ib[9] = {2, 2, 1, 0, 2, 1, 0, 1, 0};
            if (NPROD == 6 && t < 3) continue;
#pragma unroll
            for (int k2 = 0; k2 < 2; ++k2)
#pragma unroll
              for (int ni = 0; ni < 2; ++ni)
                acc[ni][kh * 2 + k2] = __builtin_amdgcn_mfma_f32_32x32x16_bf16(__builtin_bit_cast(bf16x8, a[ia[t]][ni]),
                                                                              __builtin_bit_cast(bf16x8, b[ib[t]][k2]), acc[ni][kh * 2 + k2], 0, 0, 0);
          }
        }
        if (!EARLY) stage((u + 1) % kWgDepth, cur ^ 1, st + 1 + kWgDepth);
        __syncthreads();
    };
    int st0 = 0;
    for (; st0 + kWgDepth <= steps; st0 += kWgDepth) {
      step(std::integral_constant<int, 0>{}, st0);
      if constexpr (kWgDepth > 1) step(std::integral_constant<int, 1>{}, st0 + 1);
      if constexpr (kWgDepth > 2) step(std::integral_constant<int, 2>{}, st0 + 2);
      if constexpr (kWgDepth > 3) step(std::integral_constant<int, 3>{}, st0 + 3);
    }
    if (st0 < steps) step(std::integral_constant<int, 0>{}, st0);
    if constexpr (kWgDepth > 2) if (st0 + 1 < steps) step(std::integral_constant<int, 1>{}, st0 + 1);
    if constexpr (kWgDepth > 3) if (st0 + 2 < steps) step(std::integral_constant<int, 2>{}, st0 + 2);
  }
  float* out = partial + (long)blockIdx.x * 256 * 256;
#pragma unroll
  for (int ni = 0; ni < 2; ++ni)
#pragma unroll
    for (int ki = 0; ki < 4; ++ki)
#pragma unroll
      for (int r = 0; r < 16; ++r) {
        const int n = nq * 64 + ni * 32 + wg_perm((r & 3) + 8 * (r >> 2) + 4 * lh);
        const int k = kq * 128 + ki * 32 + wg_perm(li);
        out[n * 256 + k] = F16 ? acc[ni][ki][r] * g_unscale : acc[ni][ki][r];
      }
}

template <int NPROD>
__global__ __launch_bounds__(kWgThreads, 1) void mlp_wgrad_bx(const float* __restrict__ G, int ldg, const float* __restrict__ X, int ldx,
                                                              float* __restrict__ partial, long M, long rows_per_slab, const unsigned* __restrict__ g_tmax) {
  extern __shared__ __align__(16) unsigned char wg_smem[];
  uint4* sW = reinterpret_cast<uint4*>(wg_smem);
  if (threadIdx.x >> 8)
    wgrad_bx_body<NPROD, true>(G, ldg, X, ldx, partial, M, rows_per_slab, sW, g_tmax);
  else
    wgrad_bx_body<NPROD, false>(G, ldg, X, ldx, partial, M, rows_per_slab, sW, g_tmax);
}

#ifndef MATPBR_WG_HX
#define MATPBR_WG_HX 1
#endif
constexpr int kHxRaw = 16 * 2 * 1024;
constexpr int kHxPieces = 2 * 2 * 2 * 256;
constexpr size_t kHxSmem = 3 * kHxRaw + 2 * kHxPieces * sizeof(uint4);
static_assert(kHxSmem <= 160 * 1024, "mlp_wgrad_hx: the LDS of a CU");
__global__ __launch_bounds__(kWgThreads, 1) void mlp_wgrad_hx(const float* __restrict__ G, int ldg, const float* __restrict__ X, int ldx,
                                                              float* __restrict__ partial, long M, long rows_per_slab, const unsigned* __restrict__ g_tmax) {
  extern __shared__ __align__(16) unsigned char hx_smem[];
  uint4* sP = reinterpret_cast<uint4*>(hx_smem + 3 * kHxRaw);
  const int tid = threadIdx.x, lane = tid & 63, wave = tid >> 6;
  const int nq = wave >> 1, kq = wave & 1, li = lane & 31, lh = lane >> 5;
  (void)rows_per_slab;
  const int tiles = (int)(M / kBM);
  const int t_first = tiles - 1 - (int)blockIdx.x;
  const int my_tiles = t_first >= 0 ? t_first / (int)gridDim.x + 1 : 0;
  const int steps = my_tiles * (kBM / 16);
  float g_scale = 1.0f, g_unscale = 1.0f;
  if (steps > 0) {
    unsigned mb = 0;
    for (int t = t_first; t >= 0; t -= (int)gridDim.x) mb = g_tmax[t] > mb ? g_tmax[t] : mb;
    block_scale(mb, g_scale, g_unscale);
  }
  f32x16 acc[2][4];
#pragma unroll
  for (int ni = 0; ni < 2; ++ni)
#pragma unroll
    for (int ki = 0; ki < 4; ++ki)
#pragma unroll
      for (int r = 0; r < 16; ++r) acc[ni][ki][r] = 0.f;
  if (steps > 0) {
    const int wave_u = __builtin_amdgcn_readfirstlane(wave);
    const bool loader = wave_u < 4;
    const unsigned lds0 = lds_byte_address(hx_smem);
    unsigned vg[4], vx[4];
#pragma unroll
    for (int j = 0; j < 4; ++j) {
      vg[j] = (unsigned)(j * ldg) * 4u + (unsigned)lane * 16u - 1024u * j;
      vx[j] = (unsigned)(j * ldx) * 4u + (unsigned)lane * 16u - 1024u * j;
    }
    auto issue = [&](int step, int buf) {
      const int sc = step < steps ? step : steps - 1;
      const long row = ((long)t_first - (long)(sc >> 3) * gridDim.x) * kBM + 16 * (7 - (sc & 7)) + 4 * wave_u;
      const unsigned dst = lds0 + (unsigned)buf * (unsigned)kHxRaw + (unsigned)wave_u * 4096u;
      glds16_x4v(G + row * ldg, vg[0], vg[1], vg[2], vg[3], dst);
      glds16_x4v(X + row * ldx, vx[0], vx[1], vx[2], vx[3], dst + 16u * 1024u);
    };
    const int cp = tid & 255, sh = tid >> 8;
    const float my_scale = (cp >> 7) ? 1.0f : g_scale;
    const unsigned raw_off = (unsigned)((cp >> 7) * 16 * 1024 + (8 * sh) * 1024 + (cp & 127) * 8);
    uint4* sdst = sP + (((cp >> 7) * 2) * 2 + sh) * 256 + ((cp & 127) >> 3) * 16 + (cp & 7);
    float2 raw[8];
    auto read_raw = [&](int buf) {
#pragma unroll
      for (int j = 0; j < 8; ++j) raw[j] = *reinterpret_cast<const float2*>(hx_smem + buf * kHxRaw + raw_off + j * 1024);
    };
    auto cut_store = [&](int pb) {
#pragma unroll
      for (int c = 0; c < 2; ++c) {
        uint4 pc[2];
#define MATPBR_COMP(v) (c == 0 ? (v).x : (v).y)
        split2h(MATPBR_COMP(raw[0]) * my_scale, MATPBR_COMP(raw[1]) * my_scale, pc[0].x, pc[1].x);
        split2h(MATPBR_COMP(raw[2]) * my_scale, MATPBR_COMP(raw[3]) * my_scale, pc[0].y, pc[1].y);
        split2h(MATPBR_COMP(raw[4]) * my_scale, MATPBR_COMP(raw[5]) * my_scale, pc[0].z, pc[1].z);
        split2h(MATPBR_COMP(raw[6]) * my_scale, MATPBR_COMP(raw[7]) * my_scale, pc[0].w, pc[1].w);
#undef MATPBR_COMP
#pragma unroll
        for (int piece = 0; piece < 2; ++piece) sdst[pb * kHxPieces + (piece * 2) * 256 + 8 * c] = pc[piece];
      }
    };
    const uint4* sa = sP + lh * 256 + nq * 64 + li;
    const uint4* sb = sP + (2 * 2 + lh) * 256 + kq * 128 + li;
    auto read_frags = [&](int pb, uint4 (&a)[2][2], uint4 (&b)[2][4]) {
#pragma unroll
      for (int piece = 0; piece < 2; ++piece) {
#pragma unroll
        for (int ni = 0; ni < 2; ++ni) a[piece][ni] = sa[pb * kHxPieces + (piece * 2) * 256 + ni * 32];
#pragma unroll
        for (int ki = 0; ki < 4; ++ki) b[piece][ki] = sb[pb * kHxPieces + (piece * 2) * 256 + ki * 32];
      }
    };
    auto products = [&](const uint4 (&a)[2][2], const uint4 (&b)[2][4]) {
#pragma unroll
      for (int ki = 0; ki < 4; ++ki)
#pragma unroll
        for (int t = 0; t < 3; ++t) {
          constexpr int ia[3] = {1, 0, 0}, ib[3] = {0, 1, 0};
#pragma unroll
          for (int ni = 0; ni < 2; ++ni)
            acc[ni][ki] = __builtin_amdgcn_mfma_f32_32x32x16_f16(__builtin_bit_cast(f16x8, a[ia[t]][ni]), __builtin_bit_cast(f16x8, b[ib[t]][ki]), acc[ni][ki], 0, 0, 0);
        }
    };
#define MATPBR_HX_BARRIER() do { __builtin_amdgcn_sched_barrier(0); asm volatile("s_waitcnt lgkmcnt(0)\n\ts_barrier" ::: "memory"); __builtin_amdgcn_sched_barrier(0); } while (0)
    if (loader) { issue(0, 0); issue(1, 1); issue(2, 2); }
    if (loader) asm volatile("s_waitcnt vmcnt(16)" ::: "memory");
    asm volatile("s_barrier" ::: "memory");
    read_raw(0);
    cut_store(0);
    uint4 a[2][2], b[2][4];
    int nxt = 1;
    if (loader) {
      for (int st = 0; st < steps; ++st) {
        asm volatile("s_waitcnt vmcnt(8)" ::: "memory");
        MATPBR_HX_BARRIER();
        issue(st + 3, nxt == 0 ? 2 : nxt - 1);
        __builtin_amdgcn_sched_barrier(0);
        read_frags(st & 1, a, b);
        read_raw(nxt);
        cut_store((st + 1) & 1);
        MATPBR_HX_BARRIER();
        products(a, b);
        nxt = nxt == 2 ? 0 : nxt + 1;
      }
    } else {
      MATPBR_HX_BARRIER();
      MATPBR_HX_BARRIER();
      read_frags(0, a, b);
      read_raw(1);
      cut_store(1);
      nxt = 2;
      for (int st = 1; st < steps; ++st) {
        MATPBR_HX_BARRIER();
        products(a, b);
        MATPBR_HX_BARRIER();
        read_frags(st & 1, a, b);
        read_raw(nxt);
        cut_store((st + 1) & 1);
        nxt = nxt == 2 ? 0 : nxt + 1;
      }
      products(a, b);
    }
#undef MATPBR_HX_BARRIER
    asm volatile("s_waitcnt vmcnt(0)" ::: "memory");
  }
  float* out = partial + (long)blockIdx.x * 256 * 256;
#pragma unroll
  for (int ni = 0; ni < 2; ++ni)
#pragma unroll
    for (int ki = 0; ki < 4; ++ki)
#pragma unroll
      for (int r = 0; r < 16; ++r) {
        const int n = nq * 64 + ni * 32 + wg_perm((r & 3) + 8 * (r >> 2) + 4 * lh);
        const int k = kq * 128 + ki * 32 + wg_perm(li);
        out[n * 256 + k] = acc[ni][ki][r] * g_unscale;
      }
}

constexpr size_t kBxSmem = 2 * kBxStage * sizeof(uint4) + 8 * 32 * kLd * sizeof(float);
constexpr size_t kBxSmemHead = kBxSmem + (5 * 256 + 128 * 2 * 8) * sizeof(float);
std::atomic<int> g_nt_gl{2};
std::atomic<int> g_nt_w0_gx{0};
std::atomic<int> g_wg_hx{MATPBR_WG_HX};
inline bool gl_ok(const NtArgs& p) {
  return g_nt_gl.load(std::memory_order_relaxed) != 0 && p.K > 32 && (long)kBM * p.lda * 4 < (1l << 31);
}
template <auto Kernel>
bool lds_opt_in(size_t bytes) {
  static std::atomic<unsigned long long> done{0};
  int dev = 0;
  if (hipGetDevice(&dev) != hipSuccess) return false;
  const unsigned long long bit = 1ull << (dev & 63);
  if (done.load(std::memory_order_acquire) & bit) return true;
  if (hipFuncSetAttribute(reinterpret_cast<const void*>(Kernel), hipFuncAttributeMaxDynamicSharedMemorySize, (int)bytes) != hipSuccess) return false;
  done.fetch_or(bit, std::memory_order_release);
  return true;
}
template <int EPI, int NPROD, bool FULL>
bool launch_nt_bx_full(const NtArgs& p, const uint4* wsplit, unsigned grid, hipStream_t stream) {
  if constexpr (FULL) if (gl_ok(p)) {
    if (!lds_opt_in<&mlp_nt_bx<EPI, NPROD, true, false, false, true>>(kGlSmem)) return false;
    hipLaunchKernelGGL((mlp_nt_bx<EPI, NPROD, true, false, false, true>), dim3(grid), dim3(kBxThreads), kGlSmem, stream, p, wsplit, HeadArgs{});
    return true;
  }
  if (!lds_opt_in<&mlp_nt_bx<EPI, NPROD, FULL>>(kBxSmem)) return false;
  hipLaunchKernelGGL((mlp_nt_bx<EPI, NPROD, FULL>), dim3(grid), dim3(kBxThreads), kBxSmem, stream, p, wsplit, HeadArgs{});
  return true;
}
constexpr size_t kBxSmemW0 = kBxSmem + 8 * 32 * 16 * sizeof(float);
template <int NPROD>
bool launch_nt_bx_w0(const NtArgs& p, const uint4* wsplit, unsigned grid, hipStream_t stream) {
  if (gl_ok(p)) {
    constexpr size_t bytes = kGlSmem + 8 * 32 * 16 * sizeof(float);
    if (!lds_opt_in<&mlp_nt_bx<EPI_MULC, NPROD, true, false, true, true>>(bytes)) return false;
    hipLaunchKernelGGL((mlp_nt_bx<EPI_MULC, NPROD, true, false, true, true>), dim3(grid), dim3(kBxThreads), bytes, stream, p, wsplit, HeadArgs{});
    return true;
  }
  if (!lds_opt_in<&mlp_nt_bx<EPI_MULC, NPROD, true, false, true>>(kBxSmemW0)) return false;
  hipLaunchKernelGGL((mlp_nt_bx<EPI_MULC, NPROD, true, false, true>), dim3(grid), dim3(kBxThreads), kBxSmemW0, stream, p, wsplit, HeadArgs{});
  return true;
}
template <int NPROD>
bool launch_nt_bx_head(const NtArgs& p, const uint4* wsplit, const HeadArgs& hd, unsigned grid, hipStream_t stream) {
  if (gl_ok(p)) {
    constexpr size_t bytes = kGlSmem + (5 * 256 + 128 * 2 * 8) * sizeof(float);
    if (!lds_opt_in<&mlp_nt_bx<EPI_SINCOS, NPROD, true, true, false, true>>(bytes)) return false;
    hipLaunchKernelGGL((mlp_nt_bx<EPI_SINCOS, NPROD, true, true, false, true>), dim3(grid), dim3(kBxThreads), bytes, stream, p, wsplit, hd);
    return true;
  }
  if (!lds_opt_in<&mlp_nt_bx<EPI_SINCOS, NPROD, true, true>>(kBxSmemHead)) return false;
  hipLaunchKernelGGL((mlp_nt_bx<EPI_SINCOS, NPROD, true, true>), dim3(grid), dim3(kBxThreads), kBxSmemHead, stream, p, wsplit, hd);
  return true;
}
template <int EPI, int NPROD>
bool launch_nt_bx_one(const NtArgs& p, const uint4* wsplit, unsigned grid, hipStream_t stream) {
  if (p.N >= 256 || EPI == EPI_MULC || p.tail != nullptr) return launch_nt_bx_full<EPI, NPROD, true>(p, wsplit, grid, stream);
  return launch_nt_bx_full<EPI, NPROD, false>(p, wsplit, grid, stream);
}
template <int EPI, int NPROD, bool HEAD, bool PK>
bool launch_nt_gx_pk(const NtArgs& p, const uint4* wsplit, const HeadArgs& hd, unsigned grid, hipStream_t stream) {
  if (!lds_opt_in<&mlp_nt_gx<EPI, NPROD, HEAD, PK>>(kGxSmem)) return false;
  hipLaunchKernelGGL((mlp_nt_gx<EPI, NPROD, HEAD, PK>), dim3(grid), dim3(kGxThreads), kGxSmem, stream, p, wsplit, hd);
  return true;
}
template <int EPI, int NPROD, bool HEAD>
bool launch_nt_gx(const NtArgs& p, const uint4* wsplit, const HeadArgs& hd, unsigned grid, hipStream_t stream) {
  if constexpr (EPI == EPI_SINCOS) {
    if (p.out1 == nullptr) return launch_nt_gx_pk<EPI, NPROD, HEAD, true>(p, wsplit, hd, grid, stream);
  }
  return launch_nt_gx_pk<EPI, NPROD, HEAD, false>(p, wsplit, hd, grid, stream);
}
inline bool gx_ok(const NtArgs& p) { return g_nt_gl.load(std::memory_order_relaxed) == 2 && gl_ok(p); }
template <int EPI>
int launch_nt_bx(NtArgs p, const uint4* wsplit, int nprod, hipStream_t stream) {
  const int tiles = p.M / kBM;
  if (nprod == 3) {
    if constexpr (EPI != EPI_BIAS) {
      if (p.K > 32 && (long)kBM * p.lda * 4 < (1l << 31) && (p.N >= 256 || EPI == EPI_MULC || p.tail != nullptr) && (EPI != EPI_MULC || p.a_tmax != nullptr)) {
        const unsigned grid2 = (unsigned)(tiles < 512 ? tiles : 512);
        return launch_nt_gx<EPI, 3, false>(p, wsplit, HeadArgs{}, grid2, stream) ? (int)grid2 : -1;
      }
    }
    return -1;
  }
  if constexpr (EPI != EPI_BIAS) {
    if (gx_ok(p) && (p.N >= 256 || EPI == EPI_MULC || p.tail != nullptr)) {
      const unsigned grid2 = (unsigned)(tiles < 512 ? tiles : 512);
      const bool ok2 = nprod == 9 ? launch_nt_gx<EPI, 9, false>(p, wsplit, HeadArgs{}, grid2, stream) : launch_nt_gx<EPI, 6, false>(p, wsplit, HeadArgs{}, grid2, stream);
      return ok2 ? (int)grid2 : -1;
    }
  }
  const unsigned grid = (unsigned)(tiles < 256 ? tiles : 256);
  const bool ok = nprod == 9 ? launch_nt_bx_one<EPI, 9>(p, wsplit, grid, stream) : launch_nt_bx_one<EPI, 6>(p, wsplit, grid, stream);
  return ok ? (int)grid : -1;
}

inline unsigned nt_grid(long M, int N) {
  const long rt = (M + kBM - 1) / kBM;
  const long items = N > kBN ? ((rt + 7) / 8) * 16 : rt;
  return (unsigned)(items < kPersistent ? items : kPersistent);
}

inline bool aligned16(const void* p) { return (reinterpret_cast<uintptr_t>(p) & 15u) == 0; }

template <int EPI>
int launch_nt(NtArgs p, long M, hipStream_t stream) {
  const int halves = (p.N + kBN - 1) / kBN;
  const bool pipe = p.K > 224 && p.ldo >= halves * kBN && p.lda >= 256 && p.ldb >= 256 && M >= kBM;
  int groups = 0;
  long done = 0;
  if (pipe && halves == 2) {
    done = M / kBM * kBM;
    p.M = (int)done;
    const long rt = done / kBM;
    const unsigned grid = (unsigned)(rt < kPersistent ? rt : kPersistent);
    hipLaunchKernelGGL(mlp_gemm_nt_wide<EPI>, dim3(grid), dim3(256), 0, stream, p);
    groups += (int)grid;
  } else if (pipe) {
    done = M / kBM * kBM;
    p.M = (int)done;
    const unsigned grid = nt_grid(done, p.N);
    hipLaunchKernelGGL(mlp_gemm_nt_pipe<EPI>, dim3(grid), dim3(256), 0, stream, p);
    groups += (int)grid;
  }
  if (done < M) {
    NtArgs q = p;
    q.A = p.A + (size_t)done * p.lda;
    q.out0 = p.out0 + (size_t)done * p.ldo;
    if (p.out1) q.out1 = p.out1 + (size_t)done * p.ldo;
    if (p.cmul) q.cmul = p.cmul + (size_t)done * p.ldo;
    if (p.tail) q.tail = p.tail + (size_t)done * p.ldt;
    if (p.colsum) q.colsum = p.colsum + (size_t)groups * 256;
    q.M = (int)(M - done);
    const unsigned grid = nt_grid(M - done, p.N);
    hipLaunchKernelGGL(mlp_gemm_nt<EPI>, dim3(grid), dim3(256), 0, stream, q);
    groups += (int)grid;
  }
  return groups;
}

template <int EPI, int KP>
__global__ __launch_bounds__(256) void mlp_thin_k_kernel(const NtArgs p, int tiles) {
  __shared__ __align__(16) float scr_all[4][32 * kLd];
  __shared__ __align__(16) float sWt[256 * KP];
  const int lane = threadIdx.x & 63, wave = threadIdx.x >> 6, li = lane & 31, lh = lane >> 5;
  float* scr = scr_all[wave];
  constexpr int KS = KP / 2;
  for (int i = threadIdx.x; i < 256 * KP; i += 256) {
    const int nn = i / KP, k = i - nn * KP;
    sWt[i] = (nn < p.N && k < p.K) ? p.B[(size_t)nn * p.ldb + k] : 0.f;
  }
  float bn[8];
#pragma unroll
  for (int ni = 0; ni < 8; ++ni) bn[ni] = (EPI != EPI_MULC && ni * 32 + li < p.N) ? p.bias[ni * 32 + li] : 0.f;
  __syncthreads();
  const int t_row = lane >> 3, t_col = (lane & 7) * 4;
// ... 40 lines not shown
      float second[16];
#pragma unroll
      for (int r = 0; r < 16; ++r) {
        float v = acc[r];
        if (EPI == EPI_SINCOS) {
          if (p.out1 == nullptr) v = sin_packed<true>(v + bn[ni]);
          else sincos_cw(v + bn[ni], v, second[r]);
        } else if (EPI == EPI_BIAS) v += bn[ni];
        scr[((r & 3) + 8 * (r >> 2) + 4 * lh) * kLd + li] = v;
      }
      const bool all_cols = ni * 32 + 32 <= p.N || p.tail != nullptr;
#pragma unroll
      for (int ps = 0; ps < 4; ++ps) {
        float4 v = *reinterpret_cast<const float4*>(scr + (t_row + 8 * ps) * kLd + t_col);
        const bool row_ok = full_rows || row0 + t_row + 8 * ps < p.M;
        if (EPI == EPI_MULC) {
          if (p.cmul_sin) cv[ps] = cos_from_packed_sin(cv[ps]);
          v.x *= cv[ps].x; v.y *= cv[ps].y; v.z *= cv[ps].z; v.w *= cv[ps].w;
          if (!row_ok) v = make_float4(0.f, 0.f, 0.f, 0.f);
          csum[ni].x += v.x; csum[ni].y += v.y; csum[ni].z += v.z; csum[ni].w += v.w;
        }
        if (row_ok)
          store4_upto(p.out0 + o0 + (size_t)(8 * ps) * p.ldo, v, p.N - (ni * 32 + t_col), all_cols);
      }
      if (EPI == EPI_SINCOS && p.out1 != nullptr) {
#pragma unroll
        for (int r = 0; r < 16; ++r) scr[((r & 3) + 8 * (r >> 2) + 4 * lh) * kLd + li] = second[r];
#pragma unroll
        for (int ps = 0; ps < 4; ++ps)
          if (full_rows || row0 + t_row + 8 * ps < p.M)
            store4_upto(p.out1 + o0 + (size_t)(8 * ps) * p.ldo, *reinterpret_cast<const float4*>(scr + (t_row + 8 * ps) * kLd + t_col),
                        p.N - (ni * 32 + t_col), all_cols);
      }
    }
  }
  if (EPI == EPI_MULC && p.colsum != nullptr) {
    __shared__ float red[32][256];
    __syncthreads();
#pragma unroll
    for (int ni = 0; ni < 8; ++ni) *reinterpret_cast<float4*>(&red[wave * 8 + t_row][ni * 32 + t_col]) = csum[ni];
    __syncthreads();
    float t = 0.f;
#pragma unroll
    for (int sl = 0; sl < 32; ++sl) t += red[sl][threadIdx.x];
    p.colsum[(size_t)blockIdx.x * 256 + threadIdx.x] = t;
  }
}
constexpr int kThinBlocks = 1024;
inline int thin_pad(int K) { return K <= 8 ? 8 : 16; }
template <int EPI>
int launch_thin_k(const NtArgs& p, hipStream_t stream) {
  const int tiles = (p.M + 31) / 32;
  const int grid = (tiles + 3) / 4 < kThinBlocks ? (tiles + 3) / 4 : kThinBlocks;
  if (p.K <= 8) hipLaunchKernelGGL((mlp_thin_k_kernel<EPI, 8>), dim3(grid), dim3(256), 0, stream, p, tiles);
  else hipLaunchKernelGGL((mlp_thin_k_kernel<EPI, 16>), dim3(grid), dim3(256), 0, stream, p, tiles);
  return grid;
}

template <int J, bool HEAD>
__global__ __launch_bounds__(256) void mlp_skinny_nt_kernel(const float* __restrict__ X, int ldx, const float* __restrict__ W, int ldw,
                                                            const float* __restrict__ bias, float* __restrict__ out, int ldo, long M, int K,
                                                            const ArmHead h) {
  const int lane = threadIdx.x & 63;
  const long wave = (long)blockIdx.x * 4 + (threadIdx.x >> 6), waves = (long)gridDim.x * 4;
  const int k0 = 4 * lane;
  const bool in = k0 < K;
  float4 w[J];
#pragma unroll
  for (int j = 0; j < J; ++j) w[j] = in ? *reinterpret_cast<const float4*>(W + (size_t)j * ldw + k0) : make_float4(0.f, 0.f, 0.f, 0.f);
  const long tiles = (M + 63) / 64;
  constexpr int R = 4;
  for (long tile = wave; tile < tiles; tile += waves) {
    const long row0 = tile * 64;
    float mine[J];
#pragma unroll
    for (int j = 0; j < J; ++j) mine[j] = 0.f;
    float4 x[R];
    auto load_rows = [&](int g) {
#pragma unroll
      for (int r = 0; r < R; ++r) {
        long m = row0 + g * R + r;
        m = m < M ? m : M - 1;
        x[r] = in ? *reinterpret_cast<const float4*>(X + m * ldx + k0) : make_float4(0.f, 0.f, 0.f, 0.f);
      }
    };
    load_rows(0);
    for (int g = 0; g < 64 / R; ++g) {
      float4 cur[R];
#pragma unroll
      for (int r = 0; r < R; ++r) cur[r] = x[r];
      if (g + 1 < 64 / R) load_rows(g + 1);
#pragma unroll
      for (int r = 0; r < R; ++r) {
        const int row = g * R + r;
#pragma unroll
        for (int j = 0; j < J; ++j) {
          const float t = wave_sum_lane63(fmaf(cur[r].x, w[j].x, fmaf(cur[r].y, w[j].y, fmaf(cur[r].z, w[j].z, cur[r].w * w[j].w))));
          const float total = __builtin_bit_cast(float, __builtin_amdgcn_readlane(__builtin_bit_cast(int, t), 63));
          mine[j] = lane == row ? total : mine[j];
        }
      }
    }
    const long m = row0 + lane;
    if (m < M) {
      float v[J];
#pragma unroll
      for (int j = 0; j < J; ++j) v[j] = mine[j] + bias[j];
      if (out != nullptr) {
#pragma unroll
        for (int j = 0; j < J; ++j) out[m * ldo + j] = v[j];
      }
      if (HEAD) arm_head_store(h, m, v);
    }
  }
}

template <int J, bool HEAD>
void launch_skinny_nt(const float* x, int ldx, const float* w, int ldw, const float* bias, float* out, int ldo, long M, int K, const ArmHead& h,
                      hipStream_t stream) {
  const long tiles = (M + 63) / 64;
  const unsigned grid = (unsigned)((tiles + 3) / 4 < 2048 ? (tiles + 3) / 4 : 2048);
  hipLaunchKernelGGL((mlp_skinny_nt_kernel<J, HEAD>), dim3(grid), dim3(256), 0, stream, x, ldx, w, ldw, bias, out, ldo, M, K, h);
}

__global__ __launch_bounds__(256) void arm_head_bwd_kernel(const float* __restrict__ g_a, const float* __restrict__ g_r, const float* __restrict__ g_m,
                                                           const float* __restrict__ th, float* __restrict__ d_x, long M) {
  for (long m = (long)blockIdx.x * 256 + threadIdx.x; m < M; m += (long)gridDim.x * 256) {
    const float4 t0 = *reinterpret_cast<const float4*>(th + m * 8);
    const float t4 = th[m * 8 + 4];
    float4 o = make_float4(0.f, 0.f, 0.f, 0.f);
    float o4 = 0.f;
    if (g_a) {
      o.x = (g_a[m * 3 + 0] * 1.3f) * (1.f - t0.x * t0.x);
      o.y = (g_a[m * 3 + 1] * 1.3f) * (1.f - t0.y * t0.y);
      o.z = (g_a[m * 3 + 2] * 1.3f) * (1.f - t0.z * t0.z);
    }
    if (g_r) o.w = ((g_r[m] * 0.93f) * 1.3f) * (1.f - t0.w * t0.w);
    if (g_m) o4 = (g_m[m] * 1.3f) * (1.f - t4 * t4);
    *reinterpret_cast<float4*>(d_x + m * 8) = o;
    *reinterpret_cast<float4*>(d_x + m * 8 + 4) = make_float4(o4, 0.f, 0.f, 0.f);
  }
}

constexpr int kSkinnySlabs = 1024;
constexpr int kOutJ = 5;
struct SkinnyDgrad {
  const float* W;
  int ldw, Jv;
  const float* cmul;
  float* G;
  int ldg;
  float* gsum_part;
  unsigned* tmax;
};
template <int J, bool DGRAD = false, int JV = kOutJ>
__global__ __launch_bounds__(256) void mlp_skinny_tn_kernel(const float* __restrict__ S, int lds, const float* __restrict__ B, int ldb,
                                                            float* __restrict__ partial, float* __restrict__ bpart, long M, long rows_per_slab,
                                                            const SkinnyDgrad dg) {
  __shared__ float red[3][8][256];
  __shared__ float bred[4][J];
  const int cq = threadIdx.x & 63, rs = __builtin_amdgcn_readfirstlane(threadIdx.x >> 6);
  const long m_begin = (long)blockIdx.x * rows_per_slab;
  const long m_end = (m_begin + rows_per_slab < M) ? m_begin + rows_per_slab : M;
  float4 acc[J];
  float bs[J];
#pragma unroll
  for (int j = 0; j < J; ++j) { acc[j] = make_float4(0.f, 0.f, 0.f, 0.f); bs[j] = 0.f; }
  float4 wv[DGRAD ? JV : 1], gsum = make_float4(0.f, 0.f, 0.f, 0.f);
  if (DGRAD) {
#pragma unroll
    for (int j = 0; j < JV; ++j) wv[j] = j < dg.Jv ? *reinterpret_cast<const float4*>(dg.W + (size_t)j * dg.ldw + 4 * cq) : make_float4(0.f, 0.f, 0.f, 0.f);
  }
  constexpr int U = 4;
  float tmx = 0.f;
  long tmx_tile = m_begin / kBM;
  auto tmx_flush = [&]() {
    if (DGRAD && dg.tmax != nullptr) {
      const float wmx = wave_max_lane63(tmx);
      if (cq == 63) atomicMax(dg.tmax + tmx_tile, __float_as_uint(wmx));
    }
    tmx = 0.f;
  };
  for (long m0 = m_begin + rs; m0 < m_end; m0 += 4 * U) {
    float4 b[U];
#pragma unroll
    for (int u = 0; u < U; ++u) {
      const long m = m0 + 4 * u;
      b[u] = m < m_end ? *reinterpret_cast<const float4*>(B + m * ldb + 4 * cq) : make_float4(0.f, 0.f, 0.f, 0.f);
    }
#pragma unroll
    for (int u = 0; u < U; ++u) {
      const long m = m0 + 4 * u < m_end ? m0 + 4 * u : m_end - 1;
      const float* srow = S + m * lds;
      const bool live = m0 + 4 * u < m_end;
      float4 dot = make_float4(0.f, 0.f, 0.f, 0.f);
      constexpr int JA = DGRAD ? JV : J;
#pragma unroll
      for (int j = 0; j < JA; ++j) {
        const float sv = srow[j];
        acc[j].x = fmaf(sv, b[u].x, acc[j].x);
        acc[j].y = fmaf(sv, b[u].y, acc[j].y);
        acc[j].z = fmaf(sv, b[u].z, acc[j].z);
        acc[j].w = fmaf(sv, b[u].w, acc[j].w);
        bs[j] += live ? sv : 0.f;
        if (DGRAD && j < JV) {
          dot.x = fmaf(sv, wv[j].x, dot.x); dot.y = fmaf(sv, wv[j].y, dot.y); dot.z = fmaf(sv, wv[j].z, dot.z); dot.w = fmaf(sv, wv[j].w, dot.w);
        }
      }
      if (DGRAD && live) {
        const float4 c = dg.cmul ? *reinterpret_cast<const float4*>(dg.cmul + m * ldb + 4 * cq) : cos_from_packed_sin(b[u]);
        const float4 gv = make_float4(dot.x * c.x, dot.y * c.y, dot.z * c.z, dot.w * c.w);
        *reinterpret_cast<float4*>(dg.G + m * dg.ldg + 4 * cq) = gv;
        gsum.x += gv.x; gsum.y += gv.y; gsum.z += gv.z; gsum.w += gv.w;
        if (m / kBM != tmx_tile) {
          tmx_flush();
          tmx_tile = m / kBM;
        }
        tmx = __builtin_fmaxf(__builtin_fmaxf(tmx, __builtin_fmaxf(__builtin_fabsf(gv.x), __builtin_fabsf(gv.y))), __builtin_fmaxf(__builtin_fabsf(gv.z), __builtin_fabsf(gv.w)));
      }
    }
  }
  if (DGRAD) tmx_flush();
  if (DGRAD) {
    if (rs > 0) *reinterpret_cast<float4*>(&red[rs - 1][0][4 * cq]) = gsum;
    __syncthreads();
    if (rs == 0) {
#pragma unroll
      for (int q = 0; q < 3; ++q) {
        const float4 o = *reinterpret_cast<const float4*>(&red[q][0][4 * cq]);
        gsum.x += o.x; gsum.y += o.y; gsum.z += o.z; gsum.w += o.w;
      }
      *reinterpret_cast<float4*>(dg.gsum_part + (size_t)blockIdx.x * 256 + 4 * cq) = gsum;
    }
    __syncthreads();
  }
  if (cq == 0) {
#pragma unroll
    for (int j = 0; j < J; ++j) bred[rs][j] = bs[j];
  }
#pragma unroll
  for (int j0 = 0; j0 < J; j0 += 8) {
    if (j0 > 0) __syncthreads();
    if (rs > 0) {
#pragma unroll
      for (int j = 0; j < 8; ++j) *reinterpret_cast<float4*>(&red[rs - 1][j][4 * cq]) = acc[j0 + j];
    }
    __syncthreads();
    if (rs == 0) {
#pragma unroll
      for (int j = 0; j < 8; ++j) {
        float4 t = acc[j0 + j];
#pragma unroll
        for (int q = 0; q < 3; ++q) {
          const float4 o = *reinterpret_cast<const float4*>(&red[q][j][4 * cq]);
          t.x += o.x; t.y += o.y; t.z += o.z; t.w += o.w;
        }
        *reinterpret_cast<float4*>(partial + ((size_t)blockIdx.x * J + j0 + j) * 256 + 4 * cq) = t;
      }
    }
  }
  if (rs == 0 && bpart != nullptr && threadIdx.x < J)
    bpart[(size_t)blockIdx.x * J + threadIdx.x] = (bred[0][threadIdx.x] + bred[1][threadIdx.x]) + (bred[2][threadIdx.x] + bred[3][threadIdx.x]);
}

__device__ __forceinline__ void skinny_reduce_body(float* red_, int block, const float* __restrict__ partial, const float* __restrict__ bpart, int slabs, int J, int Jv,
                                                             int C, float* __restrict__ out, long ld_j, long ld_c, float* __restrict__ d_b,
                                                             const float* __restrict__ gsum_part, int C2, float* __restrict__ d_b2) {
  float (*red)[64] = reinterpret_cast<float (*)[64]>(red_);
  int j = block >> 2;
  const int cl = threadIdx.x & 63, c = (block & 3) * 64 + cl, sl = threadIdx.x >> 6;
  if (j == J) {
    partial = gsum_part; J = 1; j = 0; Jv = 1; C = C2; out = d_b2; ld_j = 0; ld_c = 1; d_b = nullptr;
  }
  if (j >= Jv) return;
  float a0 = 0.f, a1 = 0.f, a2 = 0.f, a3 = 0.f;
  int q = sl;
  for (; q + 48 < slabs; q += 64) {
    a0 += partial[((size_t)q * J + j) * 256 + c];
    a1 += partial[((size_t)(q + 16) * J + j) * 256 + c];
    a2 += partial[((size_t)(q + 32) * J + j) * 256 + c];
    a3 += partial[((size_t)(q + 48) * J + j) * 256 + c];
  }
  for (; q < slabs; q += 16) a0 += partial[((size_t)q * J + j) * 256 + c];
  red[sl][cl] = (a0 + a1) + (a2 + a3);
  __syncthreads();
  if (sl == 0 && c < C) {
    float t = 0.f;
#pragma unroll
    for (int u = 0; u < 16; ++u) t += red[u][cl];
    out[j * ld_j + c * ld_c] = t;
  }
  if (d_b != nullptr && bpart != nullptr && (block & 3) == 0) {
    __syncthreads();
    float t = 0.f;
    for (int q2 = threadIdx.x; q2 < slabs; q2 += 1024) t += bpart[(size_t)q2 * J + j];
    red[sl][cl] = t;
    __syncthreads();
    if (sl == 0) {
      float u = 0.f;
#pragma unroll
      for (int r = 0; r < 16; ++r) u += red[r][cl];
      red[0][cl] = u;
    }
    __syncthreads();
    if (threadIdx.x == 0) {
      float u = 0.f;
      for (int r = 0; r < 64; ++r) u += red[0][r];
      d_b[j] = u;
    }
  }
}
__global__ __launch_bounds__(1024) void mlp_skinny_tn_reduce(const float* __restrict__ partial, const float* __restrict__ bpart, int slabs, int J, int Jv,
                                                             int C, float* __restrict__ out, long ld_j, long ld_c, float* __restrict__ d_b,
                                                             const float* __restrict__ gsum_part, int C2, float* __restrict__ d_b2) {
  __shared__ float red[1024];
  skinny_reduce_body(red, (int)blockIdx.x, partial, bpart, slabs, J, Jv, C, out, ld_j, ld_c, d_b, gsum_part, C2, d_b2);
}

constexpr int kMaxReduceJobs = 16;
struct ReduceJobs {
  MatpbrReduceJob j[kMaxReduceJobs];
  int first[kMaxReduceJobs + 1];
  int n;
};
__global__ __launch_bounds__(1024) void mlp_reduce_jobs_kernel(const ReduceJobs js) {
  __shared__ float red[1024];
  int k = 0;
  while (k + 1 < js.n && (int)blockIdx.x >= js.first[k + 1]) ++k;
  const MatpbrReduceJob& q = js.j[k];
  const int block = (int)blockIdx.x - js.first[k];
  if (q.kind == MATPBR_REDUCE_WGRAD) wgrad_reduce_body(red, q.src, q.groups, q.dst, q.n0, q.n1, q.n2, block);
  else if (q.kind == MATPBR_REDUCE_COLSUM) colsum_reduce_body(red, q.src, q.groups, q.dst, block);
  else skinny_reduce_body(red, block, q.src, q.src_b, q.groups, q.n0, q.n1, q.n2, q.dst, q.ld_j, q.ld_c, q.dst_b, q.src_g, q.n3, q.dst_g);
}
inline int reduce_job_blocks(const MatpbrReduceJob& q) {
  if (q.kind == MATPBR_REDUCE_WGRAD) return 256;
  if (q.kind == MATPBR_REDUCE_COLSUM) return q.n0;
  return q.n0 * 4 + (q.dst_g ? 4 : 0);
}
inline void launch_reduce_job(const MatpbrReduceJob& q, hipStream_t st) {
  if (q.kind == MATPBR_REDUCE_WGRAD) hipLaunchKernelGGL(mlp_wgrad_reduce, dim3(256), dim3(1024), 0, st, q.src, q.groups, q.dst, q.n0, q.n1, q.n2);
  else if (q.kind == MATPBR_REDUCE_COLSUM) hipLaunchKernelGGL(mlp_colsum_reduce, dim3(q.n0), dim3(256), 0, st, q.src, q.groups, q.dst);
  else hipLaunchKernelGGL(mlp_skinny_tn_reduce, dim3(reduce_job_blocks(q)), dim3(1024), 0, st, q.src, q.src_b, q.groups, q.n0, q.n1, q.n2, q.dst, q.ld_j, q.ld_c,
                          q.dst_b, q.src_g, q.n3, q.dst_g);
}
inline void reduce_or_defer(const MatpbrReduceJob& q, MatpbrReduceJob* defer, hipStream_t st) {
  if (defer) *defer = q;
  else launch_reduce_job(q, st);
}

}

extern "C" {

int matpbr_mlp_set_wgrad_kernel(int kernel) { return g_wg_hx.exchange(kernel != 0 ? 1 : 0, std::memory_order_relaxed); }

int matpbr_mlp_set_lds_dma(int mode) {
  g_nt_w0_gx.store(mode == 3 ? 1 : 0, std::memory_order_relaxed);
  const int was = g_nt_gl.exchange(mode < 0 ? 0 : (mode > 2 ? 2 : mode), std::memory_order_relaxed);
  return was;
}

int matpbr_mlp_layer_fwd_tail(const float* x, int ldx, const float* w, int ldw, const float* bias, float* s_out, float* c_out, int ldo,
                              const float* tail, int ldt, long M, int N, int K, void* stream) {
  if (!x || !w || !bias || !s_out || M <= 0 || M > 0x7fffff00L || N <= 0 || N > 256 || K <= 0 || K > 256) return MATPBR_ERR_INVALID_ARG;
  if ((ldx & 3) || (ldw & 3) || ldx < ((K + 3) & ~3) || ldw < ((K + 3) & ~3) || ldo < N || !aligned16(x) || !aligned16(w))
    return MATPBR_ERR_INVALID_ARG;
  if (tail && (ldo < 256 || ldt < 256 - N || !c_out)) return MATPBR_ERR_INVALID_ARG;
  NtArgs p{x, w, bias, nullptr, s_out, c_out, nullptr, 0, N, K, ldx, ldw, ldo};
  p.tail = tail; p.ldt = ldt;
  const bool thin = M > kSmallM && K <= 16 && ldx >= thin_pad(K) && ldw >= ((K + 3) & ~3) && ldo >= 256 && !(ldo & 3) && aligned16(s_out) &&
                    (!c_out || aligned16(c_out));
  if (M <= kSmallM) {
    if (c_out) launch_small_nt<EPI_SINCOS>(p, M, (hipStream_t)stream);
    else launch_small_nt<EPI_BIAS>(p, M, (hipStream_t)stream);
  } else if (thin) {
    p.M = (int)M;
    if (c_out) launch_thin_k<EPI_SINCOS>(p, (hipStream_t)stream);
    else launch_thin_k<EPI_BIAS>(p, (hipStream_t)stream);
  } else if (c_out)
    launch_nt<EPI_SINCOS>(p, M, (hipStream_t)stream);
  else
    launch_nt<EPI_BIAS>(p, M, (hipStream_t)stream);
  if (tail && N < 256)
    hipLaunchKernelGGL(mlp_tail_copy_kernel, dim3((unsigned)((M * (256 - N) + 255) / 256 < 2048 ? (M * (256 - N) + 255) / 256 : 2048)), dim3(256), 0,
                       (hipStream_t)stream, s_out, ldo, tail, ldt, M, N);
  return hipGetLastError() == hipSuccess ? MATPBR_OK : MATPBR_ERR_LAUNCH;
}

int matpbr_mlp_layer_fwd_sgn(const float* x, int ldx, const float* w, int ldw, const float* bias, float* s_out, int ldo, const float* tail, int ldt,
                             long M, int N, int K, void* stream) {
  if (!x || !w || !bias || !s_out || M <= 0 || M > 0x7fffff00L || N <= 0 || N > 256 || K <= 0 || K > 16) return MATPBR_ERR_INVALID_ARG;
  if (M <= kSmallM || (ldx & 3) || (ldw & 3) || ldx < thin_pad(K) || ldw < ((K + 3) & ~3) || ldo < 256 || (ldo & 3) || !aligned16(x) || !aligned16(w) ||
      !aligned16(s_out))
    return MATPBR_ERR_UNSUPPORTED;
  if (tail && ldt < 256 - N) return MATPBR_ERR_INVALID_ARG;
  NtArgs p{x, w, bias, nullptr, s_out, nullptr, nullptr, (int)M, N, K, ldx, ldw, ldo};
  p.tail = tail; p.ldt = ldt;
  launch_thin_k<EPI_SINCOS>(p, (hipStream_t)stream);
  if (tail && N < 256)
    hipLaunchKernelGGL(mlp_tail_copy_kernel, dim3((unsigned)((M * (256 - N) + 255) / 256 < 2048 ? (M * (256 - N) + 255) / 256 : 2048)), dim3(256), 0,
                       (hipStream_t)stream, s_out, ldo, tail, ldt, M, N);
  return hipGetLastError() == hipSuccess ? MATPBR_OK : MATPBR_ERR_LAUNCH;
}

int matpbr_mlp_layer_fwd(const float* x, int ldx, const float* w, int ldw, const float* bias, float* s_out, float* c_out, int ldo, long M,
                         int N, int K, void* stream) {
  return matpbr_mlp_layer_fwd_tail(x, ldx, w, ldw, bias, s_out, c_out, ldo, nullptr, 0, M, N, K, stream);
}

size_t matpbr_mlp_bwd_input_workspace_bytes(long M) {
  (void)M;
  return (size_t)((kPersistent + 16) > kThinBlocks ? (kPersistent + 16) : kThinBlocks) * 256 * sizeof(float);
}

static int mlp_layer_bwd_input_impl(const float* g, int ldg, const float* wt, int ldwt, const float* c_prev, float* g_prev, int ldo,
                                    float* d_bias_prev, void* workspace, size_t workspace_bytes, long M, int n_prev, int n_red, int sgn, void* stream) {
  if (!g || !wt || !c_prev || !g_prev || M <= 0 || M > 0x7fffff00L || n_prev <= 0 || n_prev > 256 || n_red <= 0 || n_red > 256)
    return MATPBR_ERR_INVALID_ARG;
  if ((ldg & 3) || (ldwt & 3) || ldg < ((n_red + 3) & ~3) || ldwt < ((n_red + 3) & ~3) || ldo < n_prev || !aligned16(g) || !aligned16(wt))
    return MATPBR_ERR_INVALID_ARG;
  if (d_bias_prev && (!workspace || workspace_bytes < matpbr_mlp_bwd_input_workspace_bytes(M))) return MATPBR_ERR_WORKSPACE;
  NtArgs p{g, wt, nullptr, c_prev, g_prev, nullptr, d_bias_prev ? (float*)workspace : nullptr, 0, n_prev, n_red, ldg, ldwt, ldo};
  p.cmul_sin = sgn;
  const bool thin = M > kSmallM && n_red <= 16 && ldg >= (n_red <= 8 ? 8 : 16) && ldo >= 256 && !(ldo & 3) && aligned16(c_prev) && aligned16(g_prev);
  if (sgn && !thin) return MATPBR_ERR_UNSUPPORTED;
  int groups;
  if (thin) {
    p.M = (int)M;
    groups = launch_thin_k<EPI_MULC>(p, (hipStream_t)stream);
  } else {
    groups = M <= kSmallM ? launch_small_nt<EPI_MULC>(p, M, (hipStream_t)stream) : launch_nt<EPI_MULC>(p, M, (hipStream_t)stream);
  }
  if (d_bias_prev)
    hipLaunchKernelGGL(mlp_colsum_reduce, dim3(n_prev), dim3(256), 0, (hipStream_t)stream, (const float*)workspace, groups, d_bias_prev);
  return hipGetLastError() == hipSuccess ? MATPBR_OK : MATPBR_ERR_LAUNCH;
}

int matpbr_mlp_layer_bwd_input(const float* g, int ldg, const float* wt, int ldwt, const float* c_prev, float* g_prev, int ldo,
                               float* d_bias_prev, void* workspace, size_t workspace_bytes, long M, int n_prev, int n_red, void* stream) {
  return mlp_layer_bwd_input_impl(g, ldg, wt, ldwt, c_prev, g_prev, ldo, d_bias_prev, workspace, workspace_bytes, M, n_prev, n_red, 0, stream);
}
int matpbr_mlp_layer_bwd_input_sgn(const float* g, int ldg, const float* wt, int ldwt, const float* s_prev, float* g_prev, int ldo,
                                   float* d_bias_prev, void* workspace, size_t workspace_bytes, long M, int n_prev, int n_red, void* stream) {
  return mlp_layer_bwd_input_impl(g, ldg, wt, ldwt, s_prev, g_prev, ldo, d_bias_prev, workspace, workspace_bytes, M, n_prev, n_red, 1, stream);
}

int matpbr_mlp_small_bwd_step(const float* g, int ldg, const float* w, int ldw, const float* c_prev, float* g_prev, int ldo, float* colsum_out,
                              int n_prev, const float* x, int ldx, float* d_w, int ldw_out, int K, const float* colsum_in, int colsum_stride,
                              int groups_in, float* d_bias, long M, int n_red, void* stream) {
  if (!g || !x || !d_w || M <= 0 || M > kSmallM || n_red <= 0 || n_red > 256 || K <= 0 || K > 256) return MATPBR_ERR_INVALID_ARG;
  if ((ldg & 3) || (ldx & 3) || ldg < ((n_red + 3) & ~3) || ldx < ((K + 3) & ~3) || ldw_out < K || !aligned16(g) || !aligned16(x)) return MATPBR_ERR_INVALID_ARG;
  SmallBwdStep a{};
  if (w) {
    if (!c_prev || !g_prev || n_prev <= 0 || n_prev > 256 || ldw < n_prev || ldo < n_prev) return MATPBR_ERR_INVALID_ARG;
    a.d = NtArgs{g, w, nullptr, c_prev, g_prev, nullptr, colsum_out, (int)M, n_prev, n_red, ldg, ldw, ldo};
    a.nD = (int)((M + 31) / 32) * ((n_prev + 31) / 32);
  }
  a.G = g; a.ldg = ldg; a.X = x; a.ldx = ldx; a.dW = d_w; a.ldw = ldw_out; a.M = (int)M; a.N = n_red; a.K = K;
  a.nW = ((n_red + 31) / 32) * ((K + 31) / 32);
  int nB = 0;
  if (d_bias) {
    if (!colsum_in || groups_in <= 0 || colsum_stride < n_red) return MATPBR_ERR_INVALID_ARG;
    a.part_in = colsum_in; a.part_stride = colsum_stride; a.groups_in = groups_in; a.d_bias = d_bias; a.n_bias = n_red;
    nB = (n_red + 255) / 256;
  }
  hipLaunchKernelGGL(mlp_small_bwd_step_kernel, dim3((unsigned)(a.nD + a.nW + nB)), dim3(256), 0, (hipStream_t)stream, a);
  return hipGetLastError() == hipSuccess ? MATPBR_OK : MATPBR_ERR_LAUNCH;
}

size_t matpbr_mlp_wsplit_bytes(int K) { return K > 0 ? (size_t)((K + 31) / 32) * 2 * 3 * 256 * 2 * sizeof(uint4) : 0; }

static int split_weights_one(const float* w, int ldw, int N, int K, int flags, void* wsplit, void* stream) {
  if (!w || !wsplit || N <= 0 || N > 256 || K <= 0 || K > 256 || ldw < ((flags & 1) ? N : K)) return MATPBR_ERR_INVALID_ARG;
  const int n = ((K + 31) / 32) * 2 * 256 * 2;
  hipLaunchKernelGGL(mlp_split_weights_kernel, dim3((unsigned)((n + 255) / 256)), dim3(256), 0, (hipStream_t)stream, w, ldw, N, K, flags, (uint4*)wsplit);
  return hipGetLastError() == hipSuccess ? MATPBR_OK : MATPBR_ERR_LAUNCH;
}
int matpbr_mlp_split_weights(const float* w, int ldw, int N, int K, void* wsplit, void* stream) { return split_weights_one(w, ldw, N, K, 0, wsplit, stream); }
int matpbr_mlp_split_weights_fmt(const float* w, int ldw, int N, int K, int flags, void* wsplit, void* stream) {
  if (flags & ~(MATPBR_WSPLIT_TRANSPOSED | MATPBR_WSPLIT_F16X2)) return MATPBR_ERR_INVALID_ARG;
  return split_weights_one(w, ldw, N, K, flags, wsplit, stream);
}

int matpbr_mlp_split_weights_multi(const float* const* w, const int* ldw, const int* N, const int* K, const int* transposed, void* const* wsplit,
                                   int n_jobs, void* stream) {
  if (!w || !ldw || !N || !K || !transposed || !wsplit || n_jobs <= 0 || n_jobs > 8) return MATPBR_ERR_INVALID_ARG;
  SplitJobs jobs{};
  int kmax = 0;
  for (int j = 0; j < n_jobs; ++j) {
    if (!w[j] || !wsplit[j] || N[j] <= 0 || N[j] > 256 || K[j] <= 0 || K[j] > 256 || (transposed[j] & ~3) || ldw[j] < ((transposed[j] & 1) ? N[j] : K[j])) return MATPBR_ERR_INVALID_ARG;
    jobs.w[j] = w[j]; jobs.out[j] = (uint4*)wsplit[j]; jobs.ldw[j] = ldw[j]; jobs.N[j] = N[j]; jobs.K[j] = K[j]; jobs.transposed[j] = transposed[j];
    kmax = K[j] > kmax ? K[j] : kmax;
  }
  const int n = ((kmax + 31) / 32) * 2 * 256 * 2;
  hipLaunchKernelGGL(mlp_split_weights_multi_kernel, dim3((unsigned)((n + 255) / 256), (unsigned)n_jobs), dim3(256), 0, (hipStream_t)stream, jobs);
  return hipGetLastError() == hipSuccess ? MATPBR_OK : MATPBR_ERR_LAUNCH;
}

int matpbr_mlp_layer_fwd_bx_tail(const float* x, int ldx, const void* wsplit, const float* bias, float* s_out, float* c_out, int ldo,
                                 const float* tail, int ldt, long M, int N, int K, int nprod, void* stream) {
  if (!x || !wsplit || !bias || !s_out || M <= 0 || N <= 0 || N > 256 || K <= 0 || K > 256) return MATPBR_ERR_INVALID_ARG;
  if ((nprod != 3 && nprod != 6 && nprod != 9) || (M % kBM) || M > 0x7fffff00L || ldo < 256 || (ldo & 3) || (ldx & 3) || ldx < ((K + 31) & ~31) || !aligned16(x) ||
      !aligned16(s_out) || (c_out && !aligned16(c_out)))
    return MATPBR_ERR_UNSUPPORTED;
  if (nprod == 3 && (K <= 32 || (N < 256 && !tail))) return MATPBR_ERR_UNSUPPORTED;
  if (tail && ldt < 256 - N) return MATPBR_ERR_INVALID_ARG;
  NtArgs p{x, nullptr, bias, nullptr, s_out, c_out, nullptr, (int)M, N, K, ldx, 0, ldo};
  p.tail = tail; p.ldt = ldt;
  if (launch_nt_bx<EPI_SINCOS>(p, (const uint4*)wsplit, nprod, (hipStream_t)stream) < 0) return MATPBR_ERR_LAUNCH;
  if (tail && N < 256 && !((nprod == 3 || gx_ok(p)) && N > 224))
    hipLaunchKernelGGL(mlp_tail_copy_kernel, dim3((unsigned)((M * (256 - N) + 255) / 256 < 2048 ? (M * (256 - N) + 255) / 256 : 2048)), dim3(256), 0,
                       (hipStream_t)stream, s_out, ldo, tail, ldt, M, N);
  return hipGetLastError() == hipSuccess ? MATPBR_OK : MATPBR_ERR_LAUNCH;
}

int matpbr_mlp_layer_fwd_bx_head(const float* x, int ldx, const void* wsplit, const float* bias, float* s_out, float* c_out, int ldo,
                                 const float* w_out, int ldw_out, const float* bias_out, const float* start, int lds, float* th, float* map_a,
                                 float* map_r, float* map_m, long M, int K, int nprod, void* stream) {
  if (!x || !wsplit || !bias || !s_out || !w_out || !bias_out || !start || !th || M <= 0 || K <= 0 || K > 256 || lds < 5 || ldw_out < 256)
    return MATPBR_ERR_INVALID_ARG;
  if ((nprod != 3 && nprod != 6 && nprod != 9) || (M % kBM) || M > 0x7fffff00L || ldo < 256 || (ldo & 3) || (ldx & 3) || ldx < ((K + 31) & ~31) || !aligned16(x) ||
      !aligned16(s_out) || (c_out && !aligned16(c_out)))
    return MATPBR_ERR_UNSUPPORTED;
  NtArgs p{x, nullptr, bias, nullptr, s_out, c_out, nullptr, (int)M, 256, K, ldx, 0, ldo};
  const HeadArgs hd{w_out, ldw_out, bias_out, ArmHead{start, lds, th, map_a, map_r, map_m}};
  const int tiles = (int)(M / kBM);
  const unsigned grid = (unsigned)(tiles < 256 ? tiles : 256);
  if (nprod == 3) {
    if (c_out != nullptr || K <= 32 || (long)kBM * ldx * 4 >= (1l << 31)) return MATPBR_ERR_UNSUPPORTED;
    const unsigned grid2 = (unsigned)(tiles < 512 ? tiles : 512);
    const bool ok3 = launch_nt_gx<EPI_SINCOS, 3, true>(p, (const uint4*)wsplit, hd, grid2, (hipStream_t)stream);
    return ok3 && hipGetLastError() == hipSuccess ? MATPBR_OK : MATPBR_ERR_LAUNCH;
  }
  if (gx_ok(p) && c_out == nullptr) {
    const unsigned grid2 = (unsigned)(tiles < 512 ? tiles : 512);
    const bool ok2 = nprod == 9 ? launch_nt_gx<EPI_SINCOS, 9, true>(p, (const uint4*)wsplit, hd, grid2, (hipStream_t)stream)
                                : launch_nt_gx<EPI_SINCOS, 6, true>(p, (const uint4*)wsplit, hd, grid2, (hipStream_t)stream);
    return ok2 && hipGetLastError() == hipSuccess ? MATPBR_OK : MATPBR_ERR_LAUNCH;
  }
  const bool ok = nprod == 9 ? launch_nt_bx_head<9>(p, (const uint4*)wsplit, hd, grid, (hipStream_t)stream)
                             : launch_nt_bx_head<6>(p, (const uint4*)wsplit, hd, grid, (hipStream_t)stream);
  return ok && hipGetLastError() == hipSuccess ? MATPBR_OK : MATPBR_ERR_LAUNCH;
}

int matpbr_mlp_layer_fwd_bx(const float* x, int ldx, const void* wsplit, const float* bias, float* s_out, float* c_out, int ldo, long M, int N,
                            int K, int nprod, void* stream) {
  return matpbr_mlp_layer_fwd_bx_tail(x, ldx, wsplit, bias, s_out, c_out, ldo, nullptr, 0, M, N, K, nprod, stream);
}

static int mlp_layer_bwd_input_bx_impl(const float* g, int ldg, const void* wtsplit, const float* c_prev, float* g_prev, int ldo, float* d_bias_prev,
                                       void* workspace, size_t workspace_bytes, long M, int n_prev, int n_red, int nprod, int sgn, void* stream,
                                       const unsigned* g_tile_max = nullptr, unsigned* out_tile_max = nullptr, MatpbrReduceJob* defer = nullptr) {
  if (!g || !wtsplit || !c_prev || !g_prev || M <= 0 || n_prev <= 0 || n_prev > 256 || n_red <= 0 || n_red > 256) return MATPBR_ERR_INVALID_ARG;
  if (nprod == 3 && (!g_tile_max || n_red <= 32)) return MATPBR_ERR_INVALID_ARG;
  if ((nprod != 3 && nprod != 6 && nprod != 9) || (M % kBM) || M > 0x7fffff00L || ldo < 256 || (ldo & 3) || (ldg & 3) || ldg < ((n_red + 31) & ~31) || !aligned16(g) ||
      !aligned16(g_prev) || !aligned16(c_prev))
    return MATPBR_ERR_UNSUPPORTED;
  if (d_bias_prev && (!workspace || workspace_bytes < matpbr_mlp_bwd_input_workspace_bytes(M))) return MATPBR_ERR_WORKSPACE;
  NtArgs p{g, nullptr, nullptr, c_prev, g_prev, nullptr, d_bias_prev ? (float*)workspace : nullptr, (int)M, n_prev, n_red, ldg, 0, ldo};
  p.cmul_sin = sgn;
  p.a_tmax = g_tile_max; p.o_tmax = out_tile_max;
  const int groups = launch_nt_bx<EPI_MULC>(p, (const uint4*)wtsplit, nprod, (hipStream_t)stream);
  if (groups < 0) return MATPBR_ERR_LAUNCH;
  if (defer) defer->kind = MATPBR_REDUCE_NONE;
  if (d_bias_prev) {
    MatpbrReduceJob q{};
    q.kind = MATPBR_REDUCE_COLSUM; q.groups = groups; q.src = (const float*)workspace; q.dst = d_bias_prev; q.n0 = n_prev;
    reduce_or_defer(q, defer, (hipStream_t)stream);
  }
  return hipGetLastError() == hipSuccess ? MATPBR_OK : MATPBR_ERR_LAUNCH;
}

static int mlp_first_layer_bwd_impl(const float* g, int ldg, const void* wtsplit, const float* c_prev, int ldc, int sgn, const float* x0, int ldx0,
                                    float* d_w0, long ld_j, long ld_c, int d0, float* d_bias0, void* workspace, size_t workspace_bytes, void* workspace2,
                                    size_t workspace2_bytes, long M, int n0, int n_red, int nprod, const unsigned* g_tile_max, void* stream,
                                    MatpbrReduceJob* defer = nullptr) {
  if (!g || !wtsplit || !c_prev || !x0 || !d_w0 || M <= 0 || n0 <= 0 || n0 > 256 || n_red <= 0 || n_red > 256 || d0 <= 0 || d0 > 16) return MATPBR_ERR_INVALID_ARG;
  if (nprod == 3 && (!g_tile_max || n_red <= 32)) return MATPBR_ERR_INVALID_ARG;
  if ((nprod != 3 && nprod != 6 && nprod != 9) || (M % kBM) || M > 0x7fffff00L || ldc < 256 || (ldc & 3) || (ldg & 3) || ldg < ((n_red + 31) & ~31) || ldx0 < 16 || (ldx0 & 3) ||
      !aligned16(g) || !aligned16(c_prev) || !aligned16(x0))
    return MATPBR_ERR_UNSUPPORTED;
  if (d_bias0 && (!workspace || workspace_bytes < matpbr_mlp_bwd_input_workspace_bytes(M))) return MATPBR_ERR_WORKSPACE;
  if (!workspace2 || workspace2_bytes < matpbr_mlp_skinny_workspace_bytes(16)) return MATPBR_ERR_WORKSPACE;
  NtArgs p{g, nullptr, nullptr, c_prev, nullptr, nullptr, d_bias0 ? (float*)workspace : nullptr, (int)M, n0, n_red, ldg, 0, ldc};
  p.cmul_sin = sgn;
  p.x0 = x0; p.ldx0 = ldx0; p.w0_part = (float*)workspace2;
  p.a_tmax = g_tile_max;
  const int tiles = (int)(M / kBM);
  unsigned grid = (unsigned)(tiles < 256 ? tiles : 256);
  int slabs = (int)grid * 4;
  bool ok;
  if (nprod == 3) {
    if ((long)kBM * ldg * 4 >= (1l << 31)) return MATPBR_ERR_UNSUPPORTED;
    grid = (unsigned)(tiles < 512 ? tiles : 512);
    slabs = (int)grid * 2;
    ok = lds_opt_in<&mlp_nt_gx<EPI_MULC, 3, false, false, true>>(kGxSmem);
    if (ok) hipLaunchKernelGGL((mlp_nt_gx<EPI_MULC, 3, false, false, true>), dim3(grid), dim3(kGxThreads), kGxSmem, (hipStream_t)stream, p, (const uint4*)wtsplit, HeadArgs{});
  } else if (gx_ok(p) && g_nt_w0_gx.load(std::memory_order_relaxed) != 0) {
    grid = (unsigned)(tiles < 512 ? tiles : 512);
    slabs = (int)grid * 2;
    if (nprod == 9) {
      ok = lds_opt_in<&mlp_nt_gx<EPI_MULC, 9, false, false, true>>(kGxSmem);
      if (ok) hipLaunchKernelGGL((mlp_nt_gx<EPI_MULC, 9, false, false, true>), dim3(grid), dim3(kGxThreads), kGxSmem, (hipStream_t)stream, p, (const uint4*)wtsplit, HeadArgs{});
    } else {
      ok = lds_opt_in<&mlp_nt_gx<EPI_MULC, 6, false, false, true>>(kGxSmem);
      if (ok) hipLaunchKernelGGL((mlp_nt_gx<EPI_MULC, 6, false, false, true>), dim3(grid), dim3(kGxThreads), kGxSmem, (hipStream_t)stream, p, (const uint4*)wtsplit, HeadArgs{});
    }
  } else {
    ok = nprod == 9 ? launch_nt_bx_w0<9>(p, (const uint4*)wtsplit, grid, (hipStream_t)stream) : launch_nt_bx_w0<6>(p, (const uint4*)wtsplit, grid, (hipStream_t)stream);
  }
  if (!ok) return MATPBR_ERR_LAUNCH;
  if (defer) defer[0].kind = MATPBR_REDUCE_NONE;
  if (d_bias0) {
    MatpbrReduceJob q{};
    q.kind = MATPBR_REDUCE_COLSUM; q.groups = (int)grid; q.src = (const float*)workspace; q.dst = d_bias0; q.n0 = n0;
    reduce_or_defer(q, defer, (hipStream_t)stream);
  }
  MatpbrReduceJob q2{};
  q2.kind = MATPBR_REDUCE_SKINNY; q2.groups = slabs; q2.src = (const float*)workspace2; q2.dst = d_w0; q2.n0 = 16; q2.n1 = d0; q2.n2 = n0; q2.ld_j = ld_j; q2.ld_c = ld_c;
  reduce_or_defer(q2, defer ? defer + 1 : nullptr, (hipStream_t)stream);
  return hipGetLastError() == hipSuccess ? MATPBR_OK : MATPBR_ERR_LAUNCH;
}

int matpbr_mlp_first_layer_bwd_bx(const float* g, int ldg, const void* wtsplit, const float* c_prev, int ldc, int sgn, const float* x0, int ldx0,
                                  float* d_w0, long ld_j, long ld_c, int d0, float* d_bias0, void* workspace, size_t workspace_bytes, void* workspace2,
                                  size_t workspace2_bytes, long M, int n0, int n_red, int nprod, void* stream) {
  if (nprod == 3) return MATPBR_ERR_INVALID_ARG;
  return mlp_first_layer_bwd_impl(g, ldg, wtsplit, c_prev, ldc, sgn, x0, ldx0, d_w0, ld_j, ld_c, d0, d_bias0, workspace, workspace_bytes, workspace2,
                                  workspace2_bytes, M, n0, n_red, nprod, nullptr, stream);
}
int matpbr_mlp_first_layer_bwd_blk(const float* g, int ldg, const void* g_tile_max, const void* wtsplit, const float* s_prev, int lds, const float* x0, int ldx0,
                                   float* d_w0, long ld_j, long ld_c, int d0, float* d_bias0, void* workspace, size_t workspace_bytes, void* workspace2,
                                   size_t workspace2_bytes, long M, int n0, int n_red, MatpbrReduceJob* defer2, void* stream) {
  return mlp_first_layer_bwd_impl(g, ldg, wtsplit, s_prev, lds, 1, x0, ldx0, d_w0, ld_j, ld_c, d0, d_bias0, workspace, workspace_bytes, workspace2,
                                  workspace2_bytes, M, n0, n_red, 3, (const unsigned*)g_tile_max, stream, defer2);
}
int matpbr_mlp_layer_bwd_input_blk(const float* g, int ldg, const void* g_tile_max, const void* wtsplit, const float* s_prev, float* g_prev, int ldo,
                                   void* out_tile_max, float* d_bias_prev, void* workspace, size_t workspace_bytes, long M, int n_prev, int n_red,
                                   MatpbrReduceJob* defer, void* stream) {
  return mlp_layer_bwd_input_bx_impl(g, ldg, wtsplit, s_prev, g_prev, ldo, d_bias_prev, workspace, workspace_bytes, M, n_prev, n_red, 3, 1, stream,
                                     (const unsigned*)g_tile_max, (unsigned*)out_tile_max, defer);
}

int matpbr_mlp_layer_bwd_input_bx(const float* g, int ldg, const void* wtsplit, const float* c_prev, float* g_prev, int ldo, float* d_bias_prev,
                                  void* workspace, size_t workspace_bytes, long M, int n_prev, int n_red, int nprod, void* stream) {
  if (nprod == 3) return MATPBR_ERR_INVALID_ARG;
  return mlp_layer_bwd_input_bx_impl(g, ldg, wtsplit, c_prev, g_prev, ldo, d_bias_prev, workspace, workspace_bytes, M, n_prev, n_red, nprod, 0, stream);
}
int matpbr_mlp_layer_bwd_input_bx_sgn(const float* g, int ldg, const void* wtsplit, const float* s_prev, float* g_prev, int ldo, float* d_bias_prev,
                                      void* workspace, size_t workspace_bytes, long M, int n_prev, int n_red, int nprod, void* stream) {
  if (nprod == 3) return MATPBR_ERR_INVALID_ARG;
  return mlp_layer_bwd_input_bx_impl(g, ldg, wtsplit, s_prev, g_prev, ldo, d_bias_prev, workspace, workspace_bytes, M, n_prev, n_red, nprod, 1, stream);
}

static int wgrad_slabs(long M) {
  long s = (M + 255) / 256;
  if (s > 256) s = 256;
  if (s < 1) s = 1;
  return (int)s;
}

size_t matpbr_mlp_bwd_weight_workspace_bytes(long M) { return (size_t)wgrad_slabs(M) * 256 * 256 * sizeof(float); }

int matpbr_mlp_layer_bwd_weight(const float* g, int ldg, const float* x, int ldx, float* d_w, int ldw, void* workspace,
                                size_t workspace_bytes, long M, int N, int K, void* stream) {
  if (!g || !x || !d_w || M <= 0 || N <= 0 || N > 256 || K <= 0 || K > 256) return MATPBR_ERR_INVALID_ARG;
  if ((ldg & 3) || (ldx & 3) || ldg < N || ldx < ((K + 3) & ~3) || ldw < K || !aligned16(g) || !aligned16(x)) return MATPBR_ERR_INVALID_ARG;
  if (M <= kSmallM) {
    const int tiles = ((N + 31) / 32) * ((K + 31) / 32);
    hipLaunchKernelGGL(mlp_small_tn, dim3((unsigned)tiles), dim3(256), 0, (hipStream_t)stream, g, ldg, x, ldx, d_w, ldw, (int)M, N, K);
    return hipGetLastError() == hipSuccess ? MATPBR_OK : MATPBR_ERR_LAUNCH;
  }
  if (!workspace || workspace_bytes < matpbr_mlp_bwd_weight_workspace_bytes(M)) return MATPBR_ERR_WORKSPACE;
  const int slabs = wgrad_slabs(M);
  long rows = (M + slabs - 1) / slabs;
  rows = (rows + kWM - 1) / kWM * kWM;
  hipLaunchKernelGGL(mlp_wgrad_tn, dim3(slabs, (N + 127) / 128), dim3(256), 0, (hipStream_t)stream, g, ldg, x, ldx, (float*)workspace, M, rows, K);
  hipLaunchKernelGGL(mlp_wgrad_reduce, dim3(256), dim3(1024), 0, (hipStream_t)stream, (const float*)workspace, slabs, d_w, N, K, ldw);
  return hipGetLastError() == hipSuccess ? MATPBR_OK : MATPBR_ERR_LAUNCH;
}

static int mlp_layer_bwd_weight_bx_impl(const float* g, int ldg, const float* x, int ldx, float* d_w, int ldw, void* workspace,
                                        size_t workspace_bytes, long M, int N, int K, int nprod, const unsigned* g_tile_max, void* stream,
                                        MatpbrReduceJob* defer = nullptr) {
  if (!g || !x || !d_w || M <= 0 || N <= 0 || N > 256 || K <= 0 || K > 256) return MATPBR_ERR_INVALID_ARG;
  if (nprod == 3 && (!g_tile_max || (M % kBM))) return MATPBR_ERR_INVALID_ARG;
  if ((nprod != 3 && nprod != 6 && nprod != 9) || (M & 15) || ldg < 256 || ldx < 256 || (ldg & 3) || (ldx & 3) || ldw < K || !aligned16(g) || !aligned16(x))
    return MATPBR_ERR_UNSUPPORTED;
  if (!workspace || workspace_bytes < matpbr_mlp_bwd_weight_workspace_bytes(M)) return MATPBR_ERR_WORKSPACE;
  int slabs = wgrad_slabs(M);
  long rows = ((M + slabs - 1) / slabs + 15) / 16 * 16;
  slabs = (int)((M + rows - 1) / rows);
  if (nprod == 3 && g_wg_hx.load(std::memory_order_relaxed) != 0 && (long)ldg * 4 >= 1024 && (long)ldx * 4 >= 1024 && (long)3 * ldg * 4 + 1024 < (1l << 31) && (long)3 * ldx * 4 + 1024 < (1l << 31)) {
    if (!lds_opt_in<&mlp_wgrad_hx>(kHxSmem)) return MATPBR_ERR_LAUNCH;
    hipLaunchKernelGGL(mlp_wgrad_hx, dim3(slabs), dim3(kWgThreads), kHxSmem, (hipStream_t)stream, g, ldg, x, ldx, (float*)workspace, M, rows, g_tile_max);
  } else if (nprod == 3) {
    if (!lds_opt_in<&mlp_wgrad_bx<3>>(kWgSmem)) return MATPBR_ERR_LAUNCH;
    hipLaunchKernelGGL(mlp_wgrad_bx<3>, dim3(slabs), dim3(kWgThreads), kWgSmem, (hipStream_t)stream, g, ldg, x, ldx, (float*)workspace, M, rows, g_tile_max);
  } else if (nprod == 6) {
    if (!lds_opt_in<&mlp_wgrad_bx<6>>(kWgSmem)) return MATPBR_ERR_LAUNCH;
    hipLaunchKernelGGL(mlp_wgrad_bx<6>, dim3(slabs), dim3(kWgThreads), kWgSmem, (hipStream_t)stream, g, ldg, x, ldx, (float*)workspace, M, rows, (const unsigned*)nullptr);
  } else {
    if (!lds_opt_in<&mlp_wgrad_bx<9>>(kWgSmem)) return MATPBR_ERR_LAUNCH;
    hipLaunchKernelGGL(mlp_wgrad_bx<9>, dim3(slabs), dim3(kWgThreads), kWgSmem, (hipStream_t)stream, g, ldg, x, ldx, (float*)workspace, M, rows, (const unsigned*)nullptr);
  }
  MatpbrReduceJob q{};
  q.kind = MATPBR_REDUCE_WGRAD; q.groups = slabs; q.src = (const float*)workspace; q.dst = d_w; q.n0 = N; q.n1 = K; q.n2 = ldw;
  reduce_or_defer(q, defer, (hipStream_t)stream);
  return hipGetLastError() == hipSuccess ? MATPBR_OK : MATPBR_ERR_LAUNCH;
}
int matpbr_mlp_layer_bwd_weight_bx(const float* g, int ldg, const float* x, int ldx, float* d_w, int ldw, void* workspace,
                                   size_t workspace_bytes, long M, int N, int K, int nprod, void* stream) {
  if (nprod == 3) return MATPBR_ERR_INVALID_ARG;
  return mlp_layer_bwd_weight_bx_impl(g, ldg, x, ldx, d_w, ldw, workspace, workspace_bytes, M, N, K, nprod, nullptr, stream);
}
int matpbr_mlp_layer_bwd_weight_blk(const float* g, int ldg, const void* g_tile_max, const float* x, int ldx, float* d_w, int ldw, void* workspace,
                                    size_t workspace_bytes, long M, int N, int K, MatpbrReduceJob* defer, void* stream) {
  return mlp_layer_bwd_weight_bx_impl(g, ldg, x, ldx, d_w, ldw, workspace, workspace_bytes, M, N, K, 3, (const unsigned*)g_tile_max, stream, defer);
}

int matpbr_mlp_skinny_fwd(const float* x, int ldx, const float* w, int ldw, const float* bias, float* out, int ldo, long M, int J, int K,
                          void* stream) {
  if (!x || !w || !bias || !out || M <= 0 || (J != 3 && J != 5 && J != 8) || K <= 0 || K > 256 || (K & 3)) return MATPBR_ERR_INVALID_ARG;
  if ((ldx & 3) || ldx < K || (ldw & 3) || ldw < K || ldo < J || !aligned16(x) || !aligned16(w)) return MATPBR_ERR_INVALID_ARG;
  const ArmHead none{nullptr, 0, nullptr, nullptr, nullptr, nullptr};
  if (J == 3) launch_skinny_nt<3, false>(x, ldx, w, ldw, bias, out, ldo, M, K, none, (hipStream_t)stream);
  else if (J == 5) launch_skinny_nt<5, false>(x, ldx, w, ldw, bias, out, ldo, M, K, none, (hipStream_t)stream);
  else launch_skinny_nt<8, false>(x, ldx, w, ldw, bias, out, ldo, M, K, none, (hipStream_t)stream);
  return hipGetLastError() == hipSuccess ? MATPBR_OK : MATPBR_ERR_LAUNCH;
}

int matpbr_mlp_arm_head_fwd(const float* x, int ldx, const float* w, int ldw, const float* bias, const float* start, int lds, float* th,
                            float* map_a, float* map_r, float* map_m, long M, int K, void* stream) {
  if (!x || !w || !bias || !start || !th || M <= 0 || K <= 0 || K > 256 || (K & 3) || lds < 5) return MATPBR_ERR_INVALID_ARG;
  if ((ldx & 3) || ldx < K || (ldw & 3) || ldw < K || !aligned16(x) || !aligned16(w) || !aligned16(th)) return MATPBR_ERR_INVALID_ARG;
  const ArmHead h{start, lds, th, map_a, map_r, map_m};
  launch_skinny_nt<5, true>(x, ldx, w, ldw, bias, nullptr, 0, M, K, h, (hipStream_t)stream);
  return hipGetLastError() == hipSuccess ? MATPBR_OK : MATPBR_ERR_LAUNCH;
}

int matpbr_mlp_arm_head_bwd(const float* g_a, const float* g_r, const float* g_m, const float* th, float* d_x, long M, void* stream) {
  if (!th || !d_x || M <= 0 || !aligned16(th) || !aligned16(d_x)) return MATPBR_ERR_INVALID_ARG;
  const unsigned grid = (unsigned)((M + 255) / 256 < 4096 ? (M + 255) / 256 : 4096);
  hipLaunchKernelGGL(arm_head_bwd_kernel, dim3(grid), dim3(256), 0, (hipStream_t)stream, g_a, g_r, g_m, th, d_x, M);
  return hipGetLastError() == hipSuccess ? MATPBR_OK : MATPBR_ERR_LAUNCH;
}

size_t matpbr_mlp_skinny_workspace_bytes(int J) {
  return J > 0 && J <= 16 ? (size_t)kSkinnySlabs * (((J + 7) / 8 * 8) * 257 + 256) * sizeof(float) : 0;
}

int matpbr_mlp_skinny_bwd_weight(const float* s, int lds, const float* b, int ldb, float* d_w, long ld_j, long ld_c, float* d_bias, void* workspace,
                                 size_t workspace_bytes, long M, int J, int C, void* stream) {
  if (!s || !b || !d_w || M <= 0 || J <= 0 || J > 16 || C <= 0 || C > 256) return MATPBR_ERR_INVALID_ARG;
  const int JP = (J + 7) / 8 * 8;
  if (lds < JP || ldb < 256 || (ldb & 3) || !aligned16(b)) return MATPBR_ERR_INVALID_ARG;
  if (!workspace || workspace_bytes < matpbr_mlp_skinny_workspace_bytes(J)) return MATPBR_ERR_WORKSPACE;
  long rows = (M + kSkinnySlabs - 1) / kSkinnySlabs;
  rows = (rows + 3) / 4 * 4;
  const int slabs = (int)((M + rows - 1) / rows);
  float* partial = (float*)workspace;
  float* bpart = partial + (size_t)kSkinnySlabs * JP * 256;
  if (JP == 8) hipLaunchKernelGGL((mlp_skinny_tn_kernel<8>), dim3(slabs), dim3(256), 0, (hipStream_t)stream, s, lds, b, ldb, partial, bpart, M, rows, SkinnyDgrad{});
  else hipLaunchKernelGGL((mlp_skinny_tn_kernel<16>), dim3(slabs), dim3(256), 0, (hipStream_t)stream, s, lds, b, ldb, partial, bpart, M, rows, SkinnyDgrad{});
  hipLaunchKernelGGL(mlp_skinny_tn_reduce, dim3(JP * 4), dim3(1024), 0, (hipStream_t)stream, (const float*)partial, (const float*)bpart, slabs, JP, J, C, d_w,
                     ld_j, ld_c, d_bias, (const float*)nullptr, 0, (float*)nullptr);
  return hipGetLastError() == hipSuccess ? MATPBR_OK : MATPBR_ERR_LAUNCH;
}

static int mlp_out_layer_bwd_impl(const float* d_x, int ldd, const float* s_prev, const float* c_prev, int lds, const float* w_out, int ldw, float* g_prev,
                                  int ldg, float* d_w, long ld_j, long ld_c, float* d_bias, float* d_bias_prev, void* workspace, size_t workspace_bytes,
                                  long M, int J, int n_prev, unsigned* g_tile_max, void* stream, MatpbrReduceJob* defer = nullptr) {
  if (!d_x || !s_prev || !w_out || !g_prev || !d_w || M <= 0 || J <= 0 || J > 8 || n_prev <= 0 || n_prev > 256) return MATPBR_ERR_INVALID_ARG;
  if (ldd < 8 || lds < 256 || (lds & 3) || ldg < 256 || (ldg & 3) || ldw < 256 || (ldw & 3) || !aligned16(s_prev) || !aligned16(g_prev) || !aligned16(w_out) ||
      (c_prev && !aligned16(c_prev)))
    return MATPBR_ERR_INVALID_ARG;
  if (!workspace || workspace_bytes < matpbr_mlp_skinny_workspace_bytes(J)) return MATPBR_ERR_WORKSPACE;
  long rows = (M + kSkinnySlabs - 1) / kSkinnySlabs;
  rows = (rows + 3) / 4 * 4;
  const int slabs = (int)((M + rows - 1) / rows);
  float* partial = (float*)workspace;
  float* bpart = partial + (size_t)kSkinnySlabs * 8 * 256;
  float* gsum_part = bpart + (size_t)kSkinnySlabs * 8;
  SkinnyDgrad dg{w_out, ldw, J, c_prev, g_prev, ldg, gsum_part, g_tile_max};
  if (J <= kOutJ) hipLaunchKernelGGL((mlp_skinny_tn_kernel<8, true>), dim3(slabs), dim3(256), 0, (hipStream_t)stream, d_x, ldd, s_prev, lds, partial, bpart, M, rows, dg);
  else hipLaunchKernelGGL((mlp_skinny_tn_kernel<8, true, 8>), dim3(slabs), dim3(256), 0, (hipStream_t)stream, d_x, ldd, s_prev, lds, partial, bpart, M, rows, dg);
  MatpbrReduceJob q{};
  q.kind = MATPBR_REDUCE_SKINNY; q.groups = slabs; q.src = partial; q.src_b = bpart; q.src_g = gsum_part; q.dst = d_w; q.dst_b = d_bias; q.dst_g = d_bias_prev;
  q.n0 = 8; q.n1 = J; q.n2 = 256; q.n3 = n_prev; q.ld_j = ld_j; q.ld_c = ld_c;
  reduce_or_defer(q, defer, (hipStream_t)stream);
  return hipGetLastError() == hipSuccess ? MATPBR_OK : MATPBR_ERR_LAUNCH;
}

int matpbr_mlp_out_layer_bwd(const float* d_x, int ldd, const float* s_prev, const float* c_prev, int lds, const float* w_out, int ldw, float* g_prev,
                             int ldg, float* d_w, long ld_j, long ld_c, float* d_bias, float* d_bias_prev, void* workspace, size_t workspace_bytes,
                             long M, int J, int n_prev, void* stream) {
  return mlp_out_layer_bwd_impl(d_x, ldd, s_prev, c_prev, lds, w_out, ldw, g_prev, ldg, d_w, ld_j, ld_c, d_bias, d_bias_prev, workspace, workspace_bytes, M, J,
                                n_prev, nullptr, stream);
}
int matpbr_mlp_out_layer_bwd_tmax(const float* d_x, int ldd, const float* s_prev, const float* c_prev, int lds, const float* w_out, int ldw, float* g_prev,
                                  int ldg, void* g_tile_max, float* d_w, long ld_j, long ld_c, float* d_bias, float* d_bias_prev, void* workspace,
                                  size_t workspace_bytes, long M, int J, int n_prev, MatpbrReduceJob* defer, void* stream) {
  if (!g_tile_max) return MATPBR_ERR_INVALID_ARG;
  return mlp_out_layer_bwd_impl(d_x, ldd, s_prev, c_prev, lds, w_out, ldw, g_prev, ldg, d_w, ld_j, ld_c, d_bias, d_bias_prev, workspace, workspace_bytes, M, J,
                                n_prev, (unsigned*)g_tile_max, stream, defer);
}

int matpbr_mlp_reduce_jobs(const MatpbrReduceJob* jobs, int n_jobs, void* stream) {
  if (!jobs || n_jobs <= 0 || n_jobs > kMaxReduceJobs) return MATPBR_ERR_INVALID_ARG;
  ReduceJobs js{};
  int blocks = 0;
  for (int i = 0; i < n_jobs; ++i) {
    const MatpbrReduceJob& q = jobs[i];
    if (q.kind == MATPBR_REDUCE_NONE) continue;
    if ((q.kind != MATPBR_REDUCE_WGRAD && q.kind != MATPBR_REDUCE_COLSUM && q.kind != MATPBR_REDUCE_SKINNY) || !q.src || !q.dst || q.groups <= 0 || q.n0 <= 0)
      return MATPBR_ERR_INVALID_ARG;
    js.j[js.n] = q;
    js.first[js.n] = blocks;
    blocks += reduce_job_blocks(q);
    ++js.n;
  }
  if (js.n == 0) return MATPBR_OK;
  js.first[js.n] = blocks;
  hipLaunchKernelGGL(mlp_reduce_jobs_kernel, dim3((unsigned)blocks), dim3(1024), 0, (hipStream_t)stream, js);
  return hipGetLastError() == hipSuccess ? MATPBR_OK : MATPBR_ERR_LAUNCH;
}

}
```

materialist_amd/ops.py:

```python
from __future__ import annotations

import ctypes
from typing import Dict, Optional

import torch

from . import _lib
from ._lib import MatpbrCamera, MatpbrError

LIGHT_SH25 = 0
NSH = 25
MAX_SPP = 128
FLAG_CLAMP_PARAMS = 1
FLAG_ATTACHED_SAMPLING = 2
FLAG_LAZY_FORCE = 16
FLAG_JAC16 = 32
FLAG_MODELS_READY = 64
FLAG_ROTATE_BEST = 128
FLAG_GENERIC_STEP = 256
FLAG_JAC32 = 512
FLAG_SHARE_GPU = 2048
LAZY_NSTATE = 28
LAZY_PLANES = 30
STATS_STRIDE = 16
# ... 661 lines not shown
                                                 M, int(n0), int(n_red), int(nprod), _stream(g))
    _lib.check(code, "matpbr_mlp_first_layer_bwd_bx")


def mlp_layer_bwd_weight(g: torch.Tensor, x: torch.Tensor, N: int, K: int) -> torch.Tensor:
    lib = _lib.load()
    g, x = _mat2(g, "g"), _mat2(x, "x")
    M = g.shape[0]
    ws = _mlp_workspace("bwd_weight", M, g.device, lib.matpbr_mlp_bwd_weight_workspace_bytes(M))
    d_w = torch.empty((N, K), dtype=torch.float32, device=g.device)
    with torch.cuda.device(g.device):
        code = lib.matpbr_mlp_layer_bwd_weight(_ptr(g), g.stride(0), _ptr(x), x.stride(0), _ptr(d_w), K, _ptr(ws), ws.numel() * 4, M, N, K,
                                               _stream(g))
    _lib.check(code, "matpbr_mlp_layer_bwd_weight")
    return d_w


def mlp_layer_bwd_weight_bx(g: torch.Tensor, x: torch.Tensor, N: int, K: int, nprod: int = 6, out: Optional[torch.Tensor] = None) -> torch.Tensor:
    lib = _lib.load()
    g, x = _mat2(g, "g"), _mat2(x, "x")
    M = g.shape[0]
    ws = _mlp_workspace("bwd_weight", M, g.device, lib.matpbr_mlp_bwd_weight_workspace_bytes(M))
    d_w = out if out is not None else torch.empty((N, K), dtype=torch.float32, device=g.device)
    with torch.cuda.device(g.device):
        code = lib.matpbr_mlp_layer_bwd_weight_bx(_ptr(g), g.stride(0), _ptr(x), x.stride(0), _ptr(d_w), d_w.stride(0), _ptr(ws), ws.numel() * 4,
                                                  M, N, K, nprod, _stream(g))
    _lib.check(code, "matpbr_mlp_layer_bwd_weight_bx")
    return d_w


def mlp_skinny_fwd(x: torch.Tensor, w: torch.Tensor, bias: torch.Tensor, out: torch.Tensor, K: int) -> None:
    lib = _lib.load()
    x, w = _mat2(x, "x"), _mat2(w, "w")
    with torch.cuda.device(x.device):
        code = lib.matpbr_mlp_skinny_fwd(_ptr(x), x.stride(0), _ptr(w), w.stride(0), _ptr(bias), _ptr(out), out.stride(0), x.shape[0], w.shape[0], K,
                                         _stream(x))
    _lib.check(code, "matpbr_mlp_skinny_fwd")


def mlp_arm_head_fwd(x: torch.Tensor, w: torch.Tensor, bias: torch.Tensor, start: torch.Tensor, th: torch.Tensor, map_a: Optional[torch.Tensor],
                     map_r: Optional[torch.Tensor], map_m: Optional[torch.Tensor], K: int) -> None:
    lib = _lib.load()
    x, w = _mat2(x, "x"), _mat2(w, "w")
    with torch.cuda.device(x.device):
        code = lib.matpbr_mlp_arm_head_fwd(_ptr(x), x.stride(0), _ptr(w), w.stride(0), _ptr(bias), _ptr(start), start.stride(0), _ptr(th),
                                           _ptr(map_a) if map_a is not None else None, _ptr(map_r) if map_r is not None else None,
                                           _ptr(map_m) if map_m is not None else None, x.shape[0], K, _stream(x))
    _lib.check(code, "matpbr_mlp_arm_head_fwd")


def mlp_arm_head_bwd(g_a: Optional[torch.Tensor], g_r: Optional[torch.Tensor], g_m: Optional[torch.Tensor], th: torch.Tensor, d_x: torch.Tensor) -> None:
    lib = _lib.load()
    with torch.cuda.device(th.device):
        code = lib.matpbr_mlp_arm_head_bwd(_ptr(g_a) if g_a is not None else None, _ptr(g_r) if g_r is not None else None,
                                           _ptr(g_m) if g_m is not None else None, _ptr(th), _ptr(d_x), th.shape[0], _stream(th))
    _lib.check(code, "matpbr_mlp_arm_head_bwd")


def mlp_skinny_bwd_weight(s: torch.Tensor, b: torch.Tensor, d_w: torch.Tensor, J: int, C: int, d_bias: Optional[torch.Tensor] = None,
                          transposed_out: bool = False) -> None:
    lib = _lib.load()
    b = _mat2(b, "b")
    M = b.shape[0]
    ws = _mlp_workspace("skinny%d" % ((J + 7) // 8), 0, b.device, lib.matpbr_mlp_skinny_workspace_bytes(J))
    ld_j, ld_c = (1, d_w.stride(0)) if transposed_out else (d_w.stride(0), 1)
    with torch.cuda.device(b.device):
        code = lib.matpbr_mlp_skinny_bwd_weight(_ptr(s), s.stride(0), _ptr(b), b.stride(0), _ptr(d_w), ld_j, ld_c,
                                                _ptr(d_bias) if d_bias is not None else None, _ptr(ws), ws.numel() * 4, M, J, C, _stream(b))
    _lib.check(code, "matpbr_mlp_skinny_bwd_weight")


def mlp_out_layer_bwd(d_x: torch.Tensor, s_prev: torch.Tensor, c_prev: Optional[torch.Tensor], w_out: torch.Tensor, g_prev: torch.Tensor,
                      d_w: torch.Tensor, d_bias: Optional[torch.Tensor], d_bias_prev: Optional[torch.Tensor], J: int, n_prev: int) -> None:
    lib = _lib.load()
    s_prev, g_prev = _mat2(s_prev, "s_prev"), _mat2(g_prev, "g_prev")
    M = s_prev.shape[0]
    if c_prev is not None and _mat2(c_prev, "c_prev").stride(0) != s_prev.stride(0):
        raise ValueError("mlp_out_layer_bwd: c_prev and s_prev must share their row stride")
    ws = _mlp_workspace("skinny%d" % ((J + 7) // 8), 0, s_prev.device, lib.matpbr_mlp_skinny_workspace_bytes(J))
    with torch.cuda.device(s_prev.device):
        code = lib.matpbr_mlp_out_layer_bwd(_ptr(d_x), d_x.stride(0), _ptr(s_prev), _ptr(c_prev), s_prev.stride(0), _ptr(w_out), w_out.stride(0),
                                            _ptr(g_prev), g_prev.stride(0), _ptr(d_w), d_w.stride(0), 1, _ptr(d_bias), _ptr(d_bias_prev), _ptr(ws),
                                            ws.numel() * 4, M, int(J), int(n_prev), _stream(s_prev))
    _lib.check(code, "matpbr_mlp_out_layer_bwd")


def mlp_tile_max(M: int, device) -> torch.Tensor:
    if M % 128:
        raise ValueError("the block-scaled products take row counts that are multiples of 128")
    return torch.zeros(M // 128, dtype=torch.int32, device=device)


def mlp_out_layer_bwd_tmax(d_x: torch.Tensor, s_prev: torch.Tensor, w_out: torch.Tensor, g_prev: torch.Tensor, g_tile_max: torch.Tensor,
                           d_w: torch.Tensor, d_bias: Optional[torch.Tensor], d_bias_prev: Optional[torch.Tensor], J: int, n_prev: int, defer=None) -> None:
    lib = _lib.load()
    s_prev, g_prev = _mat2(s_prev, "s_prev"), _mat2(g_prev, "g_prev")
    M = s_prev.shape[0]
    ws = _mlp_workspace("skinny%d%s" % ((J + 7) // 8, defer[1] if defer else ""), 0, s_prev.device, lib.matpbr_mlp_skinny_workspace_bytes(J))
    with torch.cuda.device(s_prev.device):
        code = lib.matpbr_mlp_out_layer_bwd_tmax(_ptr(d_x), d_x.stride(0), _ptr(s_prev), None, s_prev.stride(0), _ptr(w_out), w_out.stride(0),
                                                 _ptr(g_prev), g_prev.stride(0), _ptr(g_tile_max), _ptr(d_w), d_w.stride(0), 1, _ptr(d_bias),
                                                 _ptr(d_bias_prev), _ptr(ws), ws.numel() * 4, M, int(J), int(n_prev), defer[0] if defer else None, _stream(s_prev))
    _lib.check(code, "matpbr_mlp_out_layer_bwd_tmax")


def mlp_layer_bwd_input_blk(g: torch.Tensor, g_tile_max: torch.Tensor, wtsplit: torch.Tensor, s_prev: torch.Tensor, g_prev: torch.Tensor, n_prev: int,
                            n_red: int, d_bias_prev: Optional[torch.Tensor], out_tile_max: Optional[torch.Tensor], defer=None) -> None:
    lib = _lib.load()
    g = _mat2(g, "g")
    M = g.shape[0]
    if s_prev.stride(0) != g_prev.stride(0):
        raise ValueError("s_prev and g_prev must share their row stride")
    ws = _mlp_workspace("bwd_input" + (defer[1] if defer else ""), M, g.device, lib.matpbr_mlp_bwd_input_workspace_bytes(M))
    with torch.cuda.device(g.device):
        code = lib.matpbr_mlp_layer_bwd_input_blk(_ptr(g), g.stride(0), _ptr(g_tile_max), _ptr(wtsplit), _ptr(s_prev), _ptr(g_prev), g_prev.stride(0),
                                                  _ptr(out_tile_max) if out_tile_max is not None else None,
                                                  _ptr(d_bias_prev) if d_bias_prev is not None else None, _ptr(ws), ws.numel() * 4, M, n_prev, n_red,
                                                  defer[0] if defer else None, _stream(g))
    _lib.check(code, "matpbr_mlp_layer_bwd_input_blk")


def mlp_first_layer_bwd_blk(g: torch.Tensor, g_tile_max: torch.Tensor, wtsplit: torch.Tensor, s_prev: torch.Tensor, x0: torch.Tensor, d_w0: torch.Tensor,
                            d0: int, n0: int, n_red: int, d_bias0: Optional[torch.Tensor], defer=None) -> None:
    lib = _lib.load()
    g, s_prev, x0 = _mat2(g, "g"), _mat2(s_prev, "s_prev"), _mat2(x0, "x0")
    M = g.shape[0]
    ws = _mlp_workspace("bwd_input" + (defer[1] if defer else ""), M, g.device, lib.matpbr_mlp_bwd_input_workspace_bytes(M))
    ws2 = _mlp_workspace("skinny2" + (defer[1] if defer else ""), 0, g.device, lib.matpbr_mlp_skinny_workspace_bytes(16))
    with torch.cuda.device(g.device):
        code = lib.matpbr_mlp_first_layer_bwd_blk(_ptr(g), g.stride(0), _ptr(g_tile_max), _ptr(wtsplit), _ptr(s_prev), s_prev.stride(0), _ptr(x0), x0.stride(0),
                                                  _ptr(d_w0), 1, d_w0.stride(0), int(d0), _ptr(d_bias0), _ptr(ws), ws.numel() * 4, _ptr(ws2), ws2.numel() * 4,
                                                  M, int(n0), int(n_red), defer[0] if defer else None, _stream(g))
    _lib.check(code, "matpbr_mlp_first_layer_bwd_blk")


def mlp_layer_bwd_weight_blk(g: torch.Tensor, g_tile_max: torch.Tensor, x: torch.Tensor, N: int, K: int, out: Optional[torch.Tensor] = None,
                             defer=None) -> torch.Tensor:
    lib = _lib.load()
    g, x = _mat2(g, "g"), _mat2(x, "x")
    M = g.shape[0]
    ws = _mlp_workspace("bwd_weight" + (defer[1] if defer else ""), M, g.device, lib.matpbr_mlp_bwd_weight_workspace_bytes(M))
    d_w = out if out is not None else torch.empty((N, K), dtype=torch.float32, device=g.device)
    with torch.cuda.device(g.device):
        code = lib.matpbr_mlp_layer_bwd_weight_blk(_ptr(g), g.stride(0), _ptr(g_tile_max), _ptr(x), x.stride(0), _ptr(d_w), d_w.stride(0), _ptr(ws),
                                                   ws.numel() * 4, M, N, K, defer[0] if defer else None, _stream(g))
    _lib.check(code, "matpbr_mlp_layer_bwd_weight_blk")
    return d_w


def mlp_set_wgrad_kernel(kernel: int) -> int:
    return int(_lib.load().matpbr_mlp_set_wgrad_kernel(int(kernel)))


def mlp_reduce_jobs(jobs, n: int, like: torch.Tensor) -> None:
    with torch.cuda.device(like.device):
        code = _lib.load().matpbr_mlp_reduce_jobs(ctypes.byref(jobs), int(n), _stream(like))
    _lib.check(code, "matpbr_mlp_reduce_jobs")


LIGHT_SH9, LIGHT_ENV_TEXELS = 1, 2


class _LightToSh25(torch.autograd.Function):
    @staticmethod
    def forward(ctx, light, kind):
        lib = _lib.load()
        light = _dev(light, "light")
        B, n = light.shape[0], light.shape[1]
        out = torch.empty((B, NSH, 3), dtype=torch.float32, device=light.device)
        with torch.cuda.device(light.device):
            code = lib.matpbr_light_to_sh25(_ptr(light), int(kind), n, _ptr(out), B, _stream(light))
        _lib.check(code, "matpbr_light_to_sh25")
        ctx.kind, ctx.n = int(kind), n
        return out

    @staticmethod
    def backward(ctx, d_out):
        lib = _lib.load()
        d_out = d_out.contiguous()
        B = d_out.shape[0]
        d_light = torch.empty((B, ctx.n, 3), dtype=torch.float32, device=d_out.device)
        with torch.cuda.device(d_out.device):
            code = lib.matpbr_light_to_sh25_bwd(_ptr(d_out), ctx.kind, ctx.n, _ptr(d_light), B, _stream(d_out))
        _lib.check(code, "matpbr_light_to_sh25_bwd")
        return d_light, None


def light_to_sh25(light: torch.Tensor, kind: int) -> torch.Tensor:
    squeeze = light.ndim == 2
    out = _LightToSh25.apply(light.reshape((1,) + tuple(light.shape)) if squeeze else light, kind)
    return out[0] if squeeze else out


def adamw_step_dev(p: torch.Tensor, g: torch.Tensor, m: torch.Tensor, v: torch.Tensor, hyper: torch.Tensor, weight_decay: float = 0.01,
                   beta1: float = 0.9, beta2: float = 0.999, eps: float = 1e-8) -> None:
    lib = _lib.load()
    with torch.cuda.device(p.device):
        code = lib.matpbr_adamw_step_dev(_ptr(p), _ptr(g), _ptr(m), _ptr(v), p.numel(), _ptr(hyper), float(beta1), float(beta2), float(eps),
                                         float(weight_decay), _stream(p))
    _lib.check(code, "matpbr_adamw_step_dev")


def brdf_terms(cos1, cos2, r, f0) -> torch.Tensor:
    lib = _lib.load()
    cos1, cos2, r, f0 = (_dev(t, k).reshape(-1) for t, k in ((cos1, "cos1"), (cos2, "cos2"), (r, "r"), (f0, "f0")))
    N = cos1.numel()
    out = torch.empty((N, 4), dtype=torch.float32, device=cos1.device)
    with torch.cuda.device(cos1.device):
        code = lib.matpbr_brdf_terms(_ptr(cos1), _ptr(cos2), _ptr(r), _ptr(f0), _ptr(out), N, _stream(cos1))
    _lib.check(code, "matpbr_brdf_terms")
    return out
```

Baseline: 652.0 it/s.

## Add cache-residency plan using nontemporal loads/stores for MLP backward tensors

Result: faster. 666.9 it/s, median of 6 (+2.3%).

```diff
diff --git a/include/matpbr_mlp.h b/include/matpbr_mlp.h
--- a/include/matpbr_mlp.h
+++ b/include/matpbr_mlp.h
@@ -83,6 +83,7 @@
 int matpbr_mlp_layer_bwd_weight_blk(const float* g, int ldg, const void* g_tile_max, const float* x, int ldx, float* d_w, int ldw, void* workspace,
                                     size_t workspace_bytes, long M, int N, int K, MatpbrReduceJob* defer, void* stream);
 int matpbr_mlp_set_wgrad_kernel(int kernel);
+int matpbr_mlp_set_cache_plan(int mode, long resident_bytes);
 int matpbr_mlp_split_weights_multi(const float* const* w, const int* ldw, const int* N, const int* K, const int* transposed,
                                    void* const* wsplit, int n_jobs, void* stream);
 int matpbr_mlp_skinny_fwd(const float* x, int ldx, const float* w, int ldw, const float* bias, float* out, int ldo, long M, int J, int K,
diff --git a/materialist_amd/_lib.py b/materialist_amd/_lib.py
--- a/materialist_amd/_lib.py
+++ b/materialist_amd/_lib.py
@@ -127,6 +127,7 @@
     "matpbr_mlp_layer_bwd_weight_blk": (ctypes.c_int, [_c_f, ctypes.c_int, ctypes.c_void_p, _c_f, ctypes.c_int, _c_f, ctypes.c_int, ctypes.c_void_p,
                                                        ctypes.c_size_t, ctypes.c_long, ctypes.c_int, ctypes.c_int, ctypes.c_void_p, ctypes.c_void_p]),
     "matpbr_mlp_set_wgrad_kernel": (ctypes.c_int, [ctypes.c_int]),
+    "matpbr_mlp_set_cache_plan": (ctypes.c_int, [ctypes.c_int, ctypes.c_long]),
     "matpbr_mlp_chain_images_bytes": (ctypes.c_size_t, []),
     "matpbr_mlp_chain_prep": (ctypes.c_int, [ctypes.c_void_p, ctypes.c_void_p, ctypes.c_void_p, ctypes.c_void_p, ctypes.c_int, ctypes.c_void_p, ctypes.c_void_p,
                                              ctypes.c_void_p, ctypes.c_long, ctypes.c_void_p]),
diff --git a/materialist_amd/csrc/posmlp_kernels.hip b/materialist_amd/csrc/posmlp_kernels.hip
--- a/materialist_amd/csrc/posmlp_kernels.hip
+++ b/materialist_amd/csrc/posmlp_kernels.hip
@@ -41,6 +41,37 @@
     if (valid > 0) dst[0] = v.x;
     if (valid > 1) dst[1] = v.y;
     if (valid > 2) dst[2] = v.z;
+  }
+}
+
+typedef float f32x4v __attribute__((ext_vector_type(4)));
+template <bool NT>
+__device__ __forceinline__ void st_f4(float* dst, const float4& v) {
+  if constexpr (NT) {
+    asm volatile("" ::: "memory");
+    __builtin_nontemporal_store(f32x4v{v.x, v.y, v.z, v.w}, reinterpret_cast<f32x4v*>(dst));
+    asm volatile("" ::: "memory");
+  } else {
+    *reinterpret_cast<float4*>(dst) = v;
+  }
+}
+template <bool NT>
+__device__ __forceinline__ void st_f1(float* dst, float v) {
+  if constexpr (NT) {
+    asm volatile("" ::: "memory");
+    __builtin_nontemporal_store(v, dst);
+    asm volatile("" ::: "memory");
+  } else {
+    *dst = v;
+  }
+}
+template <bool NT>
+__device__ __forceinline__ float4 ld_f4(const float* src) {
+  if constexpr (NT) {
+    const f32x4v v = __builtin_nontemporal_load(reinterpret_cast<const f32x4v*>(src));
+    return make_float4(v.x, v.y, v.z, v.w);
+  } else {
+    return *reinterpret_cast<const float4*>(src);
   }
 }
 
@@ -62,6 +93,8 @@
   float* w0_part;
   const unsigned* a_tmax;
   unsigned* o_tmax;
+  int nt_store_below = 0;
+  int nt_load_from = 0x7fffffff;
 };
 
 constexpr int kLd = 36;
@@ -1021,7 +1054,6 @@
 }
 
 constexpr int kBxThreads = 512;
-typedef float f32x4v __attribute__((ext_vector_type(4)));
 constexpr int kGlRows = 128 * 32 * 4;
 constexpr size_t kGlSmem = 2 * kBxStage * sizeof(uint4) + 3 * kGlRows;
 template <int EPI, int NPROD, bool FULL, bool HEAD = false, bool W0 = false, bool GL = false>
@@ -1335,6 +1367,7 @@
   extern __shared__ __align__(16) unsigned char gx_smem[];
   constexpr bool F16 = NPROD == 3;
   constexpr bool BLK = F16 && EPI == EPI_MULC;
+  constexpr bool PLAN = BLK && !HEAD;
   static_assert(!F16 || EPI != EPI_BIAS, "the two-piece f16 form: sine layers forward (sines in, unit scale) and input gradients (block-scaled rows)");
   constexpr int kSlicePitch = F16 ? 384 : 256;
   constexpr size_t kStepBytes = F16 ? 16384 : (size_t)kGxW;
@@ -1483,10 +1516,16 @@
     }
     constexpr int kCvSets = W0 ? 1 : 2;
     float4 cvb[kCvSets][4];
+    const bool nt_c = PLAN && tile >= p.nt_load_from, nt_o = PLAN && !W0 && tile < p.nt_store_below;
     auto cv_load = [&](int b, float4 (&dst)[4]) {
       const float* src = p.cmul + (size_t)(row0 + wm * 64 + (b >> 2) * 32 + t_row) * p.ldo + wn * 128 + (b & 3) * 32 + t_col;
-#pragma unroll
-      for (int ps = 0; ps < 4; ++ps) dst[ps] = *reinterpret_cast<const float4*>(src + (size_t)(8 * ps) * p.ldo);
+      if (PLAN && nt_c) {
+#pragma unroll
+        for (int ps = 0; ps < 4; ++ps) dst[ps] = ld_f4<true>(src + (size_t)(8 * ps) * p.ldo);
+      } else {
+#pragma unroll
+        for (int ps = 0; ps < 4; ++ps) dst[ps] = ld_f4<false>(src + (size_t)(8 * ps) * p.ldo);
+      }
     };
     if (EPI == EPI_MULC) cv_load(0, cvb[0]);
     float hacc[4][5];
@@ -1534,7 +1573,8 @@
             if (col + 3 >= p.N) v.w = tl[col + 3];
         }
         if (W0) *reinterpret_cast<float4*>(scr + (t_row + 8 * ps) * kLd + t_col) = v;
-        else *reinterpret_cast<float4*>(p.out0 + o0 + (size_t)(8 * ps) * p.ldo) = v;
+        else if (PLAN && nt_o) st_f4<true>(p.out0 + o0 + (size_t)(8 * ps) * p.ldo, v);
+        else st_f4<false>(p.out0 + o0 + (size_t)(8 * ps) * p.ldo, v);
         vrow[ps] = v;
       }
       if (W0) {
@@ -1629,7 +1669,8 @@
 __device__ __forceinline__ int wg_perm(int i) { return (i & 16) + 2 * (i & 7) + ((i >> 3) & 1); }
 template <int NPROD, bool EARLY>
 __device__ __forceinline__ void wgrad_bx_body(const float* __restrict__ G, int ldg, const float* __restrict__ X, int ldx,
-                                              float* __restrict__ partial, long M, long rows_per_slab, uint4* sW, const unsigned* __restrict__ g_tmax) {
+                                              float* __restrict__ partial, long M, long rows_per_slab, uint4* sW, const unsigned* __restrict__ g_tmax,
+                                              int stream_partial) {
   constexpr bool F16 = NPROD == 3;
   constexpr int NP = F16 ? 2 : 3;
   const int tid = threadIdx.x, lane = tid & 63, wave = tid >> 6;
@@ -1763,27 +1804,32 @@
     if constexpr (kWgDepth > 3) if (st0 + 2 < steps) step(std::integral_constant<int, 2>{}, st0 + 2);
   }
   float* out = partial + (long)blockIdx.x * 256 * 256;
-#pragma unroll
-  for (int ni = 0; ni < 2; ++ni)
-#pragma unroll
-    for (int ki = 0; ki < 4; ++ki)
-#pragma unroll
-      for (int r = 0; r < 16; ++r) {
-        const int n = nq * 64 + ni * 32 + wg_perm((r & 3) + 8 * (r >> 2) + 4 * lh);
-        const int k = kq * 128 + ki * 32 + wg_perm(li);
-        out[n * 256 + k] = F16 ? acc[ni][ki][r] * g_unscale : acc[ni][ki][r];
-      }
+  auto store_partial = [&](auto nt) {
+#pragma unroll
+    for (int ni = 0; ni < 2; ++ni)
+#pragma unroll
+      for (int ki = 0; ki < 4; ++ki)
+#pragma unroll
+        for (int r = 0; r < 16; ++r) {
+          const int n = nq * 64 + ni * 32 + wg_perm((r & 3) + 8 * (r >> 2) + 4 * lh);
+          const int k = kq * 128 + ki * 32 + wg_perm(li);
+          st_f1<decltype(nt)::value>(out + n * 256 + k, F16 ? acc[ni][ki][r] * g_unscale : acc[ni][ki][r]);
+        }
+  };
+  if (F16 && stream_partial) store_partial(std::true_type{});
+  else store_partial(std::false_type{});
 }
 
 template <int NPROD>
 __global__ __launch_bounds__(kWgThreads, 1) void mlp_wgrad_bx(const float* __restrict__ G, int ldg, const float* __restrict__ X, int ldx,
-                                                              float* __restrict__ partial, long M, long rows_per_slab, const unsigned* __restrict__ g_tmax) {
+                                                              float* __restrict__ partial, long M, long rows_per_slab, const unsigned* __restrict__ g_tmax,
+                                                              int stream_partial) {
   extern __shared__ __align__(16) unsigned char wg_smem[];
   uint4* sW = reinterpret_cast<uint4*>(wg_smem);
   if (threadIdx.x >> 8)
-    wgrad_bx_body<NPROD, true>(G, ldg, X, ldx, partial, M, rows_per_slab, sW, g_tmax);
+    wgrad_bx_body<NPROD, true>(G, ldg, X, ldx, partial, M, rows_per_slab, sW, g_tmax, stream_partial);
   else
-    wgrad_bx_body<NPROD, false>(G, ldg, X, ldx, partial, M, rows_per_slab, sW, g_tmax);
+    wgrad_bx_body<NPROD, false>(G, ldg, X, ldx, partial, M, rows_per_slab, sW, g_tmax, stream_partial);
 }
 
 #ifndef MATPBR_WG_HX
@@ -1794,7 +1840,8 @@
 constexpr size_t kHxSmem = 3 * kHxRaw + 2 * kHxPieces * sizeof(uint4);
 static_assert(kHxSmem <= 160 * 1024, "mlp_wgrad_hx: the LDS of a CU");
 __global__ __launch_bounds__(kWgThreads, 1) void mlp_wgrad_hx(const float* __restrict__ G, int ldg, const float* __restrict__ X, int ldx,
-                                                              float* __restrict__ partial, long M, long rows_per_slab, const unsigned* __restrict__ g_tmax) {
+                                                              float* __restrict__ partial, long M, long rows_per_slab, const unsigned* __restrict__ g_tmax,
+                                                              int stream_partial) {
   extern __shared__ __align__(16) unsigned char hx_smem[];
   uint4* sP = reinterpret_cast<uint4*>(hx_smem + 3 * kHxRaw);
   const int tid = threadIdx.x, lane = tid & 63, wave = tid >> 6;
@@ -1922,16 +1969,20 @@
     asm volatile("s_waitcnt vmcnt(0)" ::: "memory");
   }
   float* out = partial + (long)blockIdx.x * 256 * 256;
-#pragma unroll
-  for (int ni = 0; ni < 2; ++ni)
-#pragma unroll
-    for (int ki = 0; ki < 4; ++ki)
-#pragma unroll
-      for (int r = 0; r < 16; ++r) {
-        const int n = nq * 64 + ni * 32 + wg_perm((r & 3) + 8 * (r >> 2) + 4 * lh);
-        const int k = kq * 128 + ki * 32 + wg_perm(li);
-        out[n * 256 + k] = acc[ni][ki][r] * g_unscale;
-      }
+  auto store_partial = [&](auto nt) {
+#pragma unroll
+    for (int ni = 0; ni < 2; ++ni)
+#pragma unroll
+      for (int ki = 0; ki < 4; ++ki)
+#pragma unroll
+        for (int r = 0; r < 16; ++r) {
+          const int n = nq * 64 + ni * 32 + wg_perm((r & 3) + 8 * (r >> 2) + 4 * lh);
+          const int k = kq * 128 + ki * 32 + wg_perm(li);
+          st_f1<decltype(nt)::value>(out + n * 256 + k, acc[ni][ki][r] * g_unscale);
+        }
+  };
+  if (stream_partial) store_partial(std::true_type{});
+  else store_partial(std::false_type{});
 }
 
 constexpr size_t kBxSmem = 2 * kBxStage * sizeof(uint4) + 8 * 32 * kLd * sizeof(float);
@@ -1939,6 +1990,25 @@
 std::atomic<int> g_nt_gl{2};
 std::atomic<int> g_nt_w0_gx{0};
 std::atomic<int> g_wg_hx{MATPBR_WG_HX};
+#ifndef MATPBR_CACHE_PLAN
+#define MATPBR_CACHE_PLAN 1
+#endif
+#ifndef MATPBR_CACHE_STEPS
+#define MATPBR_CACHE_STEPS 14
+#endif
+#ifndef MATPBR_CACHE_RESIDENT_MIB
+#define MATPBR_CACHE_RESIDENT_MIB 192
+#endif
+std::atomic<int> g_cache_plan{MATPBR_CACHE_PLAN};
+std::atomic<long> g_cache_resident{0};
+constexpr long kTileBytes = (long)kBM * 256 * sizeof(float);
+inline long plan_tiles_kept(int step, long tiles, int matrices, long fixed_bytes) {
+  if (g_cache_plan.load(std::memory_order_relaxed) == 0 || !(MATPBR_CACHE_STEPS & step)) return tiles;
+  long resident = g_cache_resident.load(std::memory_order_relaxed);
+  if (resident <= 0) resident = (long)MATPBR_CACHE_RESIDENT_MIB << 20;
+  const long kept = resident > fixed_bytes ? (resident - fixed_bytes) / (matrices * kTileBytes) : 0;
+  return kept < tiles ? kept : tiles;
+}
 inline bool gl_ok(const NtArgs& p) {
   return g_nt_gl.load(std::memory_order_relaxed) != 0 && p.K > 32 && (long)kBM * p.lda * 4 < (1l << 31);
 }
@@ -2285,6 +2355,7 @@
   int ldg;
   float* gsum_part;
   unsigned* tmax;
+  int stream_b;
 };
 template <int J, bool DGRAD = false, int JV = kOutJ>
 __global__ __launch_bounds__(256) void mlp_skinny_tn_kernel(const float* __restrict__ S, int lds, const float* __restrict__ B, int ldb,
@@ -2314,12 +2385,21 @@
     }
     tmx = 0.f;
   };
+  const bool nt_b = DGRAD && dg.stream_b;
   for (long m0 = m_begin + rs; m0 < m_end; m0 += 4 * U) {
     float4 b[U];
-#pragma unroll
-    for (int u = 0; u < U; ++u) {
-      const long m = m0 + 4 * u;
-      b[u] = m < m_end ? *reinterpret_cast<const float4*>(B + m * ldb + 4 * cq) : make_float4(0.f, 0.f, 0.f, 0.f);
+    if (nt_b) {
+#pragma unroll
+      for (int u = 0; u < U; ++u) {
+        const long m = m0 + 4 * u;
+        b[u] = m < m_end ? ld_f4<true>(B + m * ldb + 4 * cq) : make_float4(0.f, 0.f, 0.f, 0.f);
+      }
+    } else {
+#pragma unroll
+      for (int u = 0; u < U; ++u) {
+        const long m = m0 + 4 * u;
+        b[u] = m < m_end ? ld_f4<false>(B + m * ldb + 4 * cq) : make_float4(0.f, 0.f, 0.f, 0.f);
+      }
     }
 #pragma unroll
     for (int u = 0; u < U; ++u) {
@@ -2487,6 +2567,11 @@
 extern "C" {
 
 int matpbr_mlp_set_wgrad_kernel(int kernel) { return g_wg_hx.exchange(kernel != 0 ? 1 : 0, std::memory_order_relaxed); }
+
+int matpbr_mlp_set_cache_plan(int mode, long resident_bytes) {
+  g_cache_resident.store(resident_bytes > 0 ? resident_bytes : 0, std::memory_order_relaxed);
+  return g_cache_plan.exchange(mode != 0 ? 1 : 0, std::memory_order_relaxed);
+}
 
 int matpbr_mlp_set_lds_dma(int mode) {
   g_nt_w0_gx.store(mode == 3 ? 1 : 0, std::memory_order_relaxed);
@@ -2694,6 +2779,12 @@
   NtArgs p{g, nullptr, nullptr, c_prev, g_prev, nullptr, d_bias_prev ? (float*)workspace : nullptr, (int)M, n_prev, n_red, ldg, 0, ldo};
   p.cmul_sin = sgn;
   p.a_tmax = g_tile_max; p.o_tmax = out_tile_max;
+  if (nprod == 3) {
+    const long tiles = M / kBM;
+    p.nt_store_below = (int)(tiles - plan_tiles_kept(2, tiles, 5, 0));
+    const long kept = plan_tiles_kept(8, tiles, 5, (long)matpbr_mlp_bwd_weight_workspace_bytes(M));
+    if (kept < tiles) p.nt_load_from = (int)kept;
+  }
   const int groups = launch_nt_bx<EPI_MULC>(p, (const uint4*)wtsplit, nprod, (hipStream_t)stream);
   if (groups < 0) return MATPBR_ERR_LAUNCH;
   if (defer) defer->kind = MATPBR_REDUCE_NONE;
@@ -2721,6 +2812,10 @@
   p.x0 = x0; p.ldx0 = ldx0; p.w0_part = (float*)workspace2;
   p.a_tmax = g_tile_max;
   const int tiles = (int)(M / kBM);
+  if (nprod == 3) {
+    const long kept = plan_tiles_kept(8, tiles, 4, (long)matpbr_mlp_bwd_weight_workspace_bytes(M));
+    if (kept < tiles) p.nt_load_from = (int)kept;
+  }
   unsigned grid = (unsigned)(tiles < 256 ? tiles : 256);
   int slabs = (int)grid * 4;
   bool ok;
@@ -2825,18 +2920,20 @@
   int slabs = wgrad_slabs(M);
   long rows = ((M + slabs - 1) / slabs + 15) / 16 * 16;
   slabs = (int)((M + rows - 1) / rows);
+  const long tiles_w = (M + kBM - 1) / kBM;
+  const int stream_partial = nprod == 3 && plan_tiles_kept(4, tiles_w, 2, (long)slabs * 256 * 256 * sizeof(float)) < tiles_w;
   if (nprod == 3 && g_wg_hx.load(std::memory_order_relaxed) != 0 && (long)ldg * 4 >= 1024 && (long)ldx * 4 >= 1024 && (long)3 * ldg * 4 + 1024 < (1l << 31) && (long)3 * ldx * 4 + 1024 < (1l << 31)) {
     if (!lds_opt_in<&mlp_wgrad_hx>(kHxSmem)) return MATPBR_ERR_LAUNCH;
-    hipLaunchKernelGGL(mlp_wgrad_hx, dim3(slabs), dim3(kWgThreads), kHxSmem, (hipStream_t)stream, g, ldg, x, ldx, (float*)workspace, M, rows, g_tile_max);
+    hipLaunchKernelGGL(mlp_wgrad_hx, dim3(slabs), dim3(kWgThreads), kHxSmem, (hipStream_t)stream, g, ldg, x, ldx, (float*)workspace, M, rows, g_tile_max, stream_partial);
   } else if (nprod == 3) {
     if (!lds_opt_in<&mlp_wgrad_bx<3>>(kWgSmem)) return MATPBR_ERR_LAUNCH;
-    hipLaunchKernelGGL(mlp_wgrad_bx<3>, dim3(slabs), dim3(kWgThreads), kWgSmem, (hipStream_t)stream, g, ldg, x, ldx, (float*)workspace, M, rows, g_tile_max);
+    hipLaunchKernelGGL(mlp_wgrad_bx<3>, dim3(slabs), dim3(kWgThreads), kWgSmem, (hipStream_t)stream, g, ldg, x, ldx, (float*)workspace, M, rows, g_tile_max, stream_partial);
   } else if (nprod == 6) {
     if (!lds_opt_in<&mlp_wgrad_bx<6>>(kWgSmem)) return MATPBR_ERR_LAUNCH;
-    hipLaunchKernelGGL(mlp_wgrad_bx<6>, dim3(slabs), dim3(kWgThreads), kWgSmem, (hipStream_t)stream, g, ldg, x, ldx, (float*)workspace, M, rows, (const unsigned*)nullptr);
+    hipLaunchKernelGGL(mlp_wgrad_bx<6>, dim3(slabs), dim3(kWgThreads), kWgSmem, (hipStream_t)stream, g, ldg, x, ldx, (float*)workspace, M, rows, (const unsigned*)nullptr, 0);
   } else {
     if (!lds_opt_in<&mlp_wgrad_bx<9>>(kWgSmem)) return MATPBR_ERR_LAUNCH;
-    hipLaunchKernelGGL(mlp_wgrad_bx<9>, dim3(slabs), dim3(kWgThreads), kWgSmem, (hipStream_t)stream, g, ldg, x, ldx, (float*)workspace, M, rows, (const unsigned*)nullptr);
+    hipLaunchKernelGGL(mlp_wgrad_bx<9>, dim3(slabs), dim3(kWgThreads), kWgSmem, (hipStream_t)stream, g, ldg, x, ldx, (float*)workspace, M, rows, (const unsigned*)nullptr, 0);
   }
   MatpbrReduceJob q{};
   q.kind = MATPBR_REDUCE_WGRAD; q.groups = slabs; q.src = (const float*)workspace; q.dst = d_w; q.n0 = N; q.n1 = K; q.n2 = ldw;
@@ -2916,7 +3013,8 @@
   float* partial = (float*)workspace;
   float* bpart = partial + (size_t)kSkinnySlabs * 8 * 256;
   float* gsum_part = bpart + (size_t)kSkinnySlabs * 8;
-  SkinnyDgrad dg{w_out, ldw, J, c_prev, g_prev, ldg, gsum_part, g_tile_max};
+  const long tiles = (M + kBM - 1) / kBM;
+  SkinnyDgrad dg{w_out, ldw, J, c_prev, g_prev, ldg, gsum_part, g_tile_max, plan_tiles_kept(8, tiles, 4, 0) < tiles};
   if (J <= kOutJ) hipLaunchKernelGGL((mlp_skinny_tn_kernel<8, true>), dim3(slabs), dim3(256), 0, (hipStream_t)stream, d_x, ldd, s_prev, lds, partial, bpart, M, rows, dg);
   else hipLaunchKernelGGL((mlp_skinny_tn_kernel<8, true, 8>), dim3(slabs), dim3(256), 0, (hipStream_t)stream, d_x, ldd, s_prev, lds, partial, bpart, M, rows, dg);
   MatpbrReduceJob q{};
diff --git a/materialist_amd/ops.py b/materialist_amd/ops.py
--- a/materialist_amd/ops.py
+++ b/materialist_amd/ops.py
@@ -837,6 +837,10 @@
     return int(_lib.load().matpbr_mlp_set_wgrad_kernel(int(kernel)))
 
 
+def mlp_set_cache_plan(mode: int, resident_bytes: int = 0) -> int:
+    return int(_lib.load().matpbr_mlp_set_cache_plan(int(mode), int(resident_bytes)))
+
+
 def mlp_reduce_jobs(jobs, n: int, like: torch.Tensor) -> None:
     with torch.cuda.device(like.device):
         code = _lib.load().matpbr_mlp_reduce_jobs(ctypes.byref(jobs), int(n), _stream(like))
```
